# jorgeMFS/VCFX

Hardware: NVIDIA B200
Metric: vcf_input_GB_per_s (higher is better)
Workload: dtype u8

## Files before the change

vcfx_b200/csrc/vcfx_api.cu:

```cuda
#include "vcfx_cuda.h"
#include "vcfx_kernels.cuh"

#include <algorithm>
#include <cctype>
#include <cstdio>
#include <cstdlib>
#include <sched.h>
#include <cstring>
#include <new>
#include <string>
#include <vector>

using namespace vcfx;

#ifndef VCFX_LAUNCH
#define VCFX_LAUNCH(kern, grid, block, smem, stream, arg) (kern)<<<(grid), (block), (smem), (stream)>>>(arg)
#endif

namespace {

constexpr size_t DEFAULT_CHUNK = 64u << 20;
constexpr uint32_t EVENT_CAP = 1u << 20;
constexpr int MAX_SLOTS = 8;

struct Work {
    uint32_t *tile_lines = nullptr;
    unsigned long long *tile_out = nullptr;
    unsigned long long *tile_base = nullptr;
    unsigned long long *line_base = nullptr;
    uint32_t *tail_start = nullptr, *tail_len = nullptr, *tail_off = nullptr;
    uint2 *col_scratch = nullptr;
    unsigned int *ticket = nullptr;
    uint32_t *tile_resume = nullptr;
    Rec *recs = nullptr;
    uint8_t *rec_prefix = nullptr;
    uint64_t rec_cap = 0;
    DevStats *d_stats = nullptr;
    unsigned long long *events = nullptr;
    uint32_t ev_cap = 0;
    uint8_t *ib_codes = nullptr; size_t ib_codes_cap = 0;
    IbMeta *ib_rows = nullptr; uint64_t ib_rows_cap = 0;
    uint8_t *ib_panels = nullptr; uint64_t ib_panel_cap = 0;
    unsigned long long ib_seq = 0; bool ib_first = false;
    DevStats *h_stats = nullptr;
    DevStats *h_init = nullptr;
    uint32_t tiles_cap = 0;
    cudaEvent_t ev_k0 = nullptr, ev_k1 = nullptr;
    cudaEvent_t ev_stats = nullptr;
};

struct Slot {
    char *h_in = nullptr;
    uint8_t *d_in = nullptr;
    uint8_t *d_out = nullptr;
    char *h_out = nullptr;
    cudaStream_t stream = nullptr;
    Work w;
    size_t nbytes = 0;
    size_t out_cap = 0;
    vcfx_chunk_info info = {0, 1, 0, 0};
    bool in_flight = false;
    cudaEvent_t ev_h2d = nullptr;
    cudaEvent_t ev_shared_done = nullptr;
    bool shared_pending = false;
    uint8_t *d_in_used = nullptr;
    bool d2h_issued = false;
    size_t d2h_bytes = 0;
};

}

struct vcfx_ctx {
    vcfx_cfg cfg;
    int device = 0;
    int sm_count = 0;
    int blocks_per_sm = 1;
    size_t chunk_bytes = 0, out_bytes = 0;
    uint32_t tile_bytes = 0;
    size_t line_hint = 0;
    bool line_hint_fixed = false;
    int n_slots = 0;
    Slot slots[MAX_SLOTS];
    int head = 0;
    int tail = 0;
    int n_in_flight = 0;
    int acquired_slot = -1;
    Work dev_work;
    cudaStream_t dev_stream = nullptr;
    bool dev_stream_owned = false;
    bool dev_pending = false;
    size_t dev_nbytes = 0;
    uint8_t *dev_in = nullptr, *dev_out = nullptr;
    size_t dev_out_cap = 0;
    vcfx_chunk_info dev_info = {0, 1, 0, 0};
    uint32_t n_sel = 0, max_col = 0;
    uint32_t *d_sel_col = nullptr, *d_name_off = nullptr;
    uint8_t *d_names = nullptr;
    uint4 *d_names16 = nullptr;
    uint32_t name_len = 0;
    bool ac_bulk = true;
    int ac_fmt = 0;
    bool ac_ident = false;
    bool ac_exact = false;
    bool c4_bulk = false;
    uint8_t gq_query[64] = {0}; uint32_t gq_len = 0; int gq_a = -1, gq_b = -1;
    IbState *d_ib = nullptr; double *d_ib_sum = nullptr; unsigned long long *d_ib_het = nullptr; unsigned int *d_ib_used = nullptr; uint8_t *d_ib_last = nullptr;
    cudaEvent_t ib_event = nullptr;
    bool ib_event_set = false;
    unsigned long long ib_next_seq = 0;
    bool ib_open = false;
    std::vector<uint64_t> last_events;
    uint64_t last_n_events = 0;
    std::string last_error;
};

namespace {

#define CU(call)                                                                         \
    do {                                                                                 \
        cudaError_t _e = (call);                                                         \
        if (_e != cudaSuccess) {                                                         \
            ctx->last_error = std::string(#call) + ": " + cudaGetErrorString(_e);       \
            return (_e == cudaErrorMemoryAllocation) ? VCFX_E_NOMEM : VCFX_E_CUDA;       \
        }                                                                                \
    } while (0)

typedef void (*kernel_fn)(const KParams);

#ifdef VCFX_EMU
struct HweArgs { const int32_t *c; size_t n; double *p; };
void hwe_pvalue_entry(const HweArgs a) { hwe_pvalue_kernel(a.c, a.n, a.p); }
void hwe_pvalue_launch(int grid, const int32_t *c, size_t n, double *p) { HweArgs a = {c, n, p}; emu_launch(hwe_pvalue_entry, dim3(grid), dim3(256), 0, nullptr, a); }
#else
void hwe_pvalue_launch(int grid, const int32_t *c, size_t n, double *p) { hwe_pvalue_kernel<<<grid, 256>>>(c, n, p); }
#endif

bool is_copy_op(int op) {
    return op == VCFX_OP_MISSING_DETECT || op == VCFX_OP_NONREF_FILTER || op == VCFX_OP_PHASE_CHECK || op == VCFX_OP_GENOTYPE_QUERY;
}

kernel_fn kernel_for(int op) {
    switch (op) {
    case VCFX_OP_VARIANT_COUNT: return vcfx_scan_kernel<OP_VC, 0>;
    case VCFX_OP_ALLELE_FREQ:   return vcfx_scan_kernel<OP_AF, 0>;
    case VCFX_OP_HWE:           return vcfx_scan_kernel<OP_HWE, 0>;
    case VCFX_OP_MISSING_DETECT: return vcfx_scan_kernel<OP_MD, 0>;
    case VCFX_OP_NONREF_FILTER: return vcfx_scan_kernel<OP_NR, 0>;
    case VCFX_OP_INDEX: return vcfx_scan_kernel<OP_IX, 0>;
    case VCFX_OP_PHASE_CHECK: return vcfx_scan_kernel<OP_PC, 0>;
    case VCFX_OP_INBREEDING: return vcfx_scan_kernel<OP_IB, 0>;
    case VCFX_OP_GENOTYPE_QUERY: return vcfx_scan_kernel<OP_GQ, 0>;
    case VCFX_OP_DOSAGE: return vcfx_scan_kernel<OP_DS, 0>;
    case VCFX_OP_ALLELE_COUNT:  return vcfx_scan_kernel<OP_AC, 0>;
    default: return nullptr;
    }
}
kernel_fn general_kernel_for(int op) {
    switch (op) {
    case VCFX_OP_ALLELE_FREQ: return vcfx_scan_kernel<OP_AF, 1>;
    case VCFX_OP_HWE:         return vcfx_scan_kernel<OP_HWE, 1>;
    default: return nullptr;
    }
}
kernel_fn format_kernel_for(int op, int ac_fmt = 0) {
    if (op == VCFX_OP_ALLELE_COUNT) return ac_fmt == AC_AGG ? format_rows_kernel<OP_AC> : nullptr;
    switch (op) {
    case VCFX_OP_ALLELE_FREQ: return format_rows_kernel<OP_AF>;
    case VCFX_OP_HWE:         return format_rows_kernel<OP_HWE>;
    case VCFX_OP_MISSING_DETECT: return md_copy_kernel;
    case VCFX_OP_NONREF_FILTER: return md_copy_kernel;
    case VCFX_OP_PHASE_CHECK: return md_copy_kernel;
    case VCFX_OP_GENOTYPE_QUERY: return md_copy_kernel;
    case VCFX_OP_INDEX: return format_rows_kernel<OP_IX>;
    case VCFX_OP_INBREEDING: return ib_rows_kernel;
    case VCFX_OP_DOSAGE: return ds_rows_kernel;
    default: return nullptr;
    }
}

constexpr uint32_t MIN_TILE = 32u << 10, MAX_TILE = 256u << 10;

uint32_t tile_for(const vcfx_ctx *ctx, size_t nbytes) {
    if (ctx->tile_bytes) return ctx->tile_bytes;
    size_t warps = (size_t)ctx->sm_count * ctx->blocks_per_sm * WARPS_PER_CTA;
    size_t t = nbytes / (warps * 4 + 1);
    t = (t + 511) & ~(size_t)511;
    t = std::min<size_t>(MAX_TILE, std::max<size_t>(MIN_TILE, t));
    if (ctx->line_hint) {
        size_t want = std::min<size_t>((ctx->line_hint * 8 + 511) & ~(size_t)511, (size_t)8 << 20);
        size_t room = (nbytes / (warps * 2 + 1)) & ~(size_t)511;
        t = std::max(t, std::min(want, room));
    }
    return (uint32_t)t;
}

size_t measure_line(const char *p, size_t n, size_t from) {
    size_t pos = std::min(from, n), lim = std::min(n, pos + ((size_t)1 << 20));
    for (int tries = 0; pos < lim && tries < 4096; ++tries) {
        const char *nl = static_cast<const char *>(memchr(p + pos, '\n', lim - pos));
        if (!nl) return 0;
        size_t len = (size_t)(nl - (p + pos)) + 1;
        if (p[pos] != '#' && len > 1) return len;
        pos += len;
    }
    return 0;
}

uint32_t tiles_for(const vcfx_ctx *ctx, size_t nbytes, uint32_t tile) {
    (void)ctx;
    return (uint32_t)std::max<size_t>(1, (nbytes + tile - 1) / tile);
}

int grid_for(const vcfx_ctx *ctx, uint32_t n_tiles) {
    int resident = ctx->sm_count * ctx->blocks_per_sm;
    int need = (int)((n_tiles + WARPS_PER_CTA - 1) / WARPS_PER_CTA);
    return std::max(1, std::min(resident, need));
}

uint64_t default_rec_cap(size_t nbytes) { return nbytes / 256 + 65536; }

uint64_t rec_slack(const vcfx_ctx *ctx) {
    return (uint64_t)REC_BLOCK * ctx->sm_count * ctx->blocks_per_sm * WARPS_PER_CTA + 1024;
}

void free_work(Work &w) {
    cudaFree(w.tile_lines); cudaFree(w.tile_out); cudaFree(w.tile_base); cudaFree(w.line_base);
    cudaFree(w.rec_prefix); cudaFree(w.ticket); cudaFree(w.recs); cudaFree(w.d_stats); cudaFree(w.events);
    cudaFree(w.tail_start); cudaFree(w.tail_len); cudaFree(w.tail_off); cudaFree(w.col_scratch); cudaFree(w.tile_resume);
    cudaFree(w.ib_codes); cudaFree(w.ib_rows); cudaFree(w.ib_panels);
    if (w.h_stats) cudaFreeHost(w.h_stats);
    if (w.h_init) cudaFreeHost(w.h_init);
    if (w.ev_k0) cudaEventDestroy(w.ev_k0);
    if (w.ev_k1) cudaEventDestroy(w.ev_k1);
    if (w.ev_stats) cudaEventDestroy(w.ev_stats);
    w = Work();
}

int ensure_work(vcfx_ctx *ctx, Work &w, size_t max_bytes, uint64_t min_recs = 0, uint64_t min_panel_bytes = 0) {
    uint32_t tiles = tiles_for(ctx, max_bytes, ctx->tile_bytes ? ctx->tile_bytes : MIN_TILE);
    if (!w.d_stats) {
        CU(cudaMalloc(&w.d_stats, sizeof(DevStats)));
        CU(cudaMalloc(&w.ticket, 2 * sizeof(unsigned int)));
        CU(cudaMalloc(&w.events, sizeof(unsigned long long) * EVENT_CAP));
        w.ev_cap = EVENT_CAP;
        CU(cudaMallocHost(&w.h_stats, sizeof(DevStats)));
        CU(cudaMallocHost(&w.h_init, sizeof(DevStats)));
        memset(w.h_init, 0, sizeof(DevStats)); w.h_init->first_short_key = ~0ULL;
        memset(w.h_stats, 0, sizeof(DevStats));
        CU(cudaEventCreate(&w.ev_k0));
        CU(cudaEventCreate(&w.ev_k1));
        CU(cudaEventCreateWithFlags(&w.ev_stats, cudaEventDisableTiming));
    }
    if (tiles > w.tiles_cap) {
        cudaFree(w.tile_lines); cudaFree(w.tile_out); cudaFree(w.tile_base); cudaFree(w.line_base);
        w.tile_lines = nullptr; w.tile_out = nullptr; w.tile_base = w.line_base = nullptr;
        CU(cudaMalloc(&w.tile_lines, sizeof(uint32_t) * tiles));
        CU(cudaMalloc(&w.tile_out, sizeof(unsigned long long) * tiles));
        CU(cudaMalloc(&w.tile_base, sizeof(unsigned long long) * tiles));
        CU(cudaMalloc(&w.line_base, sizeof(unsigned long long) * tiles));
        if (general_kernel_for(ctx->cfg.op)) {
            cudaFree(w.tile_resume); w.tile_resume = nullptr;
            CU(cudaMalloc(&w.tile_resume, sizeof(uint32_t) * tiles));
        }
        if (is_copy_op(ctx->cfg.op)) {
            cudaFree(w.tail_start); cudaFree(w.tail_len); cudaFree(w.tail_off);
            w.tail_start = w.tail_len = w.tail_off = nullptr;
            CU(cudaMalloc(&w.tail_start, sizeof(uint32_t) * tiles));
            CU(cudaMalloc(&w.tail_len, sizeof(uint32_t) * tiles));
            CU(cudaMalloc(&w.tail_off, sizeof(uint32_t) * tiles));
        }
        w.tiles_cap = tiles;
    }
    uint64_t recs = 0;
    if (format_kernel_for(ctx->cfg.op, ctx->ac_fmt)) recs = std::max<uint64_t>(default_rec_cap(max_bytes), min_recs);
    if (ctx->cfg.op == VCFX_OP_ALLELE_COUNT && !w.col_scratch) {
        size_t n = (size_t)ctx->sm_count * ctx->blocks_per_sm * WARPS_PER_CTA * std::max<uint32_t>(ctx->max_col, 1);
        CU(cudaMalloc(&w.col_scratch, n * sizeof(uint2)));
    }
    if (ctx->cfg.op == VCFX_OP_DOSAGE && max_bytes + VCFX_DEVICE_PAD > w.ib_codes_cap) {
        cudaFree(w.ib_codes); w.ib_codes = nullptr; w.ib_codes_cap = 0;
        CU(cudaMalloc(&w.ib_codes, max_bytes + VCFX_DEVICE_PAD));
        w.ib_codes_cap = max_bytes + VCFX_DEVICE_PAD;
    }
    if (ctx->cfg.op == VCFX_OP_INBREEDING) {
        const uint64_t want_pan = std::max<uint64_t>(max_bytes + (1u << 20), min_panel_bytes);
        if (want_pan > w.ib_panel_cap) {
            cudaFree(w.ib_panels); w.ib_panels = nullptr; w.ib_panel_cap = 0;
            CU(cudaMalloc(&w.ib_panels, want_pan));
            w.ib_panel_cap = want_pan;
        }
        if (max_bytes + VCFX_DEVICE_PAD > w.ib_codes_cap) {
            cudaFree(w.ib_codes); w.ib_codes = nullptr; w.ib_codes_cap = 0;
            CU(cudaMalloc(&w.ib_codes, max_bytes + VCFX_DEVICE_PAD));
            w.ib_codes_cap = max_bytes + VCFX_DEVICE_PAD;
        }
        if (std::max<uint64_t>(recs, w.rec_cap) > w.ib_rows_cap) {
            const uint64_t want = std::max<uint64_t>(recs, w.rec_cap);
            cudaFree(w.ib_rows); w.ib_rows = nullptr; w.ib_rows_cap = 0;
            CU(cudaMalloc(&w.ib_rows, want * sizeof(IbMeta)));
            w.ib_rows_cap = want;
        }
    }
    if (recs > w.rec_cap) {
        cudaFree(w.recs); w.recs = nullptr; w.rec_cap = 0;
        cudaFree(w.rec_prefix); w.rec_prefix = nullptr;
        CU(cudaMalloc(&w.recs, recs * sizeof(Rec)));
        if (ctx->cfg.op == VCFX_OP_ALLELE_FREQ || ctx->cfg.op == VCFX_OP_HWE) CU(cudaMalloc(&w.rec_prefix, recs * 32));
        w.rec_cap = recs;
    }
    return VCFX_OK;
}

uint64_t ib_panel_need(const vcfx_ctx *ctx, const Work &w) {
    return (uint64_t)w.h_stats->n_recs * 32u * ((ctx->n_sel + 31u) / 32u) + (1u << 20);
}

void ib_begin(vcfx_ctx *ctx, Work &w, const vcfx_chunk_info *info) {
    if (ctx->cfg.op != VCFX_OP_INBREEDING) return;
    w.ib_seq = ctx->ib_next_seq++;
    w.ib_first = !ctx->ib_open;
    ctx->ib_open = !(info ? info->is_final != 0 : true);
}

int launch_chunk(vcfx_ctx *ctx, Work &w, cudaStream_t st, uint8_t *d_in, size_t nbytes,
                 const vcfx_chunk_info *info, uint8_t *d_out, size_t out_cap, bool write_pad = true) {
    kernel_fn fn = kernel_for(ctx->cfg.op);
    if (!fn) return VCFX_E_UNSUPPORTED;
    const uint32_t tile = tile_for(ctx, nbytes);
    uint32_t tiles = tiles_for(ctx, nbytes, tile);
    if (write_pad) CU(cudaMemsetAsync(d_in + nbytes, '\n', 64, st));
    CU(cudaMemsetAsync(w.ticket, 0, 2 * sizeof(unsigned int), st));
    kernel_fn gfn = general_kernel_for(ctx->cfg.op);
    if (gfn) CU(cudaMemsetAsync(w.tile_resume, 0xFF, sizeof(uint32_t) * tiles, st));
    CU(cudaMemcpyAsync(w.d_stats, w.h_init, sizeof(DevStats), cudaMemcpyHostToDevice, st));

    KParams P;
    P.in = d_in; P.n = nbytes;
    P.tile_bytes = tile; P.n_tiles = tiles;
    P.mode = ctx->cfg.mode; P.flags = ctx->cfg.flags;
    P.valid_from = info ? info->data_valid_from : 0;
    P.fmt0_until = info ? info->format_cache_from : 0;
    P.file_offset = info ? info->file_offset : 0;
    P.is_final = info ? info->is_final : 1;
    P.out = d_out; P.out_cap = out_cap;
    P.tile_lines = w.tile_lines; P.tile_out = w.tile_out; P.tile_base = w.tile_base; P.line_base = w.line_base;
    P.tail_start = w.tail_start; P.tail_len = w.tail_len; P.tail_off = w.tail_off;
    P.ac_fmt = ctx->ac_fmt; P.ac_ident = ctx->ac_ident ? 1 : 0; P.ac_pass = 0; P.ac_spec = (ctx->cfg.op == VCFX_OP_ALLELE_COUNT && ctx->ac_fmt == AC_TEXT_MT && !ctx->ac_exact) ? 1 : 0; P.n_sel = ctx->n_sel; P.sel_col = ctx->d_sel_col; P.name_off = ctx->d_name_off;
    P.names = ctx->d_names; P.names16 = ctx->d_names16; P.name_len = ctx->name_len; P.ac_bulk = ctx->ac_bulk ? 1 : 0; P.max_col = ctx->max_col; P.col_scratch = w.col_scratch;
    P.ticket = w.ticket; P.ticket2 = w.ticket + 1; P.tile_resume = w.tile_resume; P.recs = w.recs; P.rec_prefix = w.rec_prefix; P.rec_cap = w.rec_cap;
    P.c4_bulk = ctx->c4_bulk ? 1 : 0;
    memcpy(P.gq_query, ctx->gq_query, sizeof P.gq_query); P.gq_len = ctx->gq_len; P.gq_a = ctx->gq_a; P.gq_b = ctx->gq_b; P.gq_strict = (ctx->cfg.flags & VCFX_F_GQ_STRICT) ? 1 : 0;
    P.ib_codes = w.ib_codes; P.ib_rows = w.ib_rows; P.ib_panels = w.ib_panels; P.ib_panel_cap = w.ib_panel_cap; P.ib = ctx->d_ib; P.ib_seq = w.ib_seq; P.ib_first = w.ib_first ? 1 : 0; P.text_cap = out_cap;
    if (ctx->cfg.op == VCFX_OP_INBREEDING) P.out_cap = ~0ULL;
    P.stats = w.d_stats; P.events = w.events; P.ev_cap = w.ev_cap; P.ev_raw = (ctx->cfg.op == VCFX_OP_PHASE_CHECK || ctx->cfg.op == VCFX_OP_GENOTYPE_QUERY) ? 1 : 0;

    CU(cudaEventRecord(w.ev_k0, st));
    if (nbytes > 0) {
        int grid = grid_for(ctx, tiles);
        VCFX_LAUNCH(fn, grid, WARPS_PER_CTA * 32, 0, st, P);
        CU(cudaGetLastError());
        if (gfn) {
            const int ggrid = std::max(1, std::min(ctx->sm_count * VCFX_GENERAL_CTAS, (int)((tiles + WARPS_PER_CTA - 1) / WARPS_PER_CTA)));
            VCFX_LAUNCH(gfn, ggrid, WARPS_PER_CTA * 32, 0, st, P);
            CU(cudaGetLastError());
        }
        VCFX_LAUNCH(tile_scan_kernel, 1, 1024, SCAN_SMEM_BYTES, st, P);
        CU(cudaGetLastError());
        if (kernel_fn ff = format_kernel_for(ctx->cfg.op, ctx->ac_fmt)) {
            VCFX_LAUNCH(ff, ctx->sm_count * ((is_copy_op(ctx->cfg.op)) ? 8 : 16), 256, 0, st, P);
            CU(cudaGetLastError());
        } else if (ctx->cfg.op == VCFX_OP_ALLELE_COUNT) {
            CU(cudaMemsetAsync(w.ticket, 0, 2 * sizeof(unsigned int), st));
            P.ac_pass = 1;
            VCFX_LAUNCH(fn, grid, WARPS_PER_CTA * 32, 0, st, P);
            CU(cudaGetLastError());
        }
    }
    if (ctx->cfg.op == VCFX_OP_INBREEDING) {
        if (ctx->ib_event_set) CU(cudaStreamWaitEvent(st, ctx->ib_event, 0));
        VCFX_LAUNCH(ib_accumulate_kernel, (int)((ctx->n_sel + 31) / 32), 32, 0, st, P);
        CU(cudaGetLastError());
        VCFX_LAUNCH(ib_finish_kernel, 1, 1024, 0, st, P);
        CU(cudaGetLastError());
        CU(cudaEventRecord(ctx->ib_event, st));
        ctx->ib_event_set = true;
    }
    CU(cudaEventRecord(w.ev_k1, st));
    CU(cudaMemcpyAsync(w.h_stats, w.d_stats, sizeof(DevStats), cudaMemcpyDeviceToHost, st));
    CU(cudaEventRecord(w.ev_stats, st));
    return VCFX_OK;
}

void fill_stats(const Work &w, size_t nbytes, vcfx_chunk_stats *s) {
    if (!s) return;
    memset(s, 0, sizeof *s);
    const DevStats &d = *w.h_stats;
    s->bytes_in = nbytes; s->bytes_out = d.bytes_out;
    s->lines = d.lines; s->data_lines = d.data_lines; s->rows = d.rows; s->flagged = d.flagged;
    s->pre_header = d.pre_header; s->short_lines = d.short_lines;
    s->first_short_line = d.first_short_line; s->n_events = d.n_events;
    s->dots_terminated = d.dots_terminated; s->last_unterminated_flagged = d.last_unterminated_flagged;
    float ms = 0.f;
    if (cudaEventElapsedTime(&ms, w.ev_k0, w.ev_k1) == cudaSuccess) s->kernel_ms = ms;
}

int fetch_events(vcfx_ctx *ctx, const Work &w, cudaStream_t st) {
    uint64_t nev = std::min<uint64_t>(w.h_stats->n_events, w.ev_cap);
    ctx->last_n_events = w.h_stats->n_events;
    ctx->last_events.resize(nev);
    if (nev) {
        CU(cudaMemcpyAsync(ctx->last_events.data(), w.events, nev * sizeof(uint64_t), cudaMemcpyDeviceToHost, st));
        CU(cudaStreamSynchronize(st));
        std::sort(ctx->last_events.begin(), ctx->last_events.end());
    }
    return VCFX_OK;
}

int grow_events(vcfx_ctx *ctx, Work &w) {
    if ((ctx->cfg.op != VCFX_OP_PHASE_CHECK && ctx->cfg.op != VCFX_OP_GENOTYPE_QUERY) || w.h_stats->n_events <= w.ev_cap) return 0;
    const uint64_t want = w.h_stats->n_events + (w.h_stats->n_events >> 3) + 1024;
    if (want > 0xFFFFFFFFull) return VCFX_E_OUTPUT_TOO_BIG;
    cudaFree(w.events); w.events = nullptr; w.ev_cap = 0;
    CU(cudaMalloc(&w.events, sizeof(unsigned long long) * want));
    w.ev_cap = (uint32_t)want;
    return 1;
}

size_t default_out_bytes(int op, unsigned flags, size_t chunk) {
    switch (op) {
    case VCFX_OP_VARIANT_COUNT: return 4096;
    case VCFX_OP_MISSING_DETECT: return chunk + chunk / 4 + 4096;
    case VCFX_OP_NONREF_FILTER: return chunk + 4096;
    case VCFX_OP_PHASE_CHECK: return chunk + 4096;
    case VCFX_OP_GENOTYPE_QUERY: return chunk + 4096;
    case VCFX_OP_DOSAGE: return chunk + 4096;
    case VCFX_OP_INBREEDING: return 1u << 20;
    case VCFX_OP_ALLELE_COUNT:
        if (flags & VCFX_F_AC_AGGREGATE) return chunk / 4 + (1u << 20);
        if (flags & VCFX_F_AC_BINARY) return chunk + 4096;
        return 10 * chunk + 4096;
    default: return chunk / 4 + (1u << 20);
    }
}

void kick_ready(vcfx_ctx *ctx) {
    for (int i = 0, k = ctx->tail; i < ctx->n_in_flight; ++i, k = (k + 1) % ctx->n_slots) {
        Slot &s = ctx->slots[k];
        if (!s.in_flight || s.d2h_issued) continue;
        if (cudaEventQuery(s.w.ev_stats) != cudaSuccess) break;
        if (s.w.h_stats->overflow) continue;
        const size_t nout = (size_t)s.w.h_stats->bytes_out;
        if (nout && cudaMemcpyAsync(s.h_out, s.d_out, nout, cudaMemcpyDeviceToHost, s.stream) != cudaSuccess) { cudaGetLastError(); break; }
        s.d2h_issued = true; s.d2h_bytes = nout;
    }
}

}

extern "C" {

int vcfx_cuda_abi_version(void) { return VCFX_CUDA_ABI_VERSION; }

int vcfx_cuda_device_count(int *n) {
    int c = 0;
    cudaError_t e = cudaGetDeviceCount(&c);
    if (n) *n = (e == cudaSuccess) ? c : 0;
    return (e == cudaSuccess && c > 0) ? VCFX_OK : VCFX_E_NO_DEVICE;
}

const char *vcfx_cuda_strerror(int err) {
    switch (err) {
    case VCFX_OK: return "ok";
    case VCFX_E_INVALID: return "invalid argument or call order";
    case VCFX_E_NO_DEVICE: return "no usable CUDA device (libvcfx_cuda has no CPU fallback)";
    case VCFX_E_CUDA: return "CUDA call failed";
    case VCFX_E_NOMEM: return "out of memory";
    case VCFX_E_BUSY: return "all pipeline slots in flight";
    case VCFX_E_EMPTY: return "nothing in flight";
    case VCFX_E_OUTPUT_TOO_BIG: return "chunk output exceeds the output slot";
    case VCFX_E_UNSUPPORTED: return "operation not supported";
    default: return "unknown error";
    }
}

const char *vcfx_cuda_last_error(const vcfx_ctx *ctx) { return ctx ? ctx->last_error.c_str() : ""; }

int vcfx_cuda_create(const vcfx_cfg *cfg, vcfx_ctx **out) {
    if (!cfg || !out) return VCFX_E_INVALID;
    *out = nullptr;
    if (cfg->op < VCFX_OP_VARIANT_COUNT || cfg->op > VCFX_OP_DOSAGE) return VCFX_E_INVALID;
    if (cfg->mode != VCFX_MODE_FILE && cfg->mode != VCFX_MODE_STDIN) return VCFX_E_INVALID;
    int ndev = 0;
    if (cudaGetDeviceCount(&ndev) != cudaSuccess || ndev <= 0) return VCFX_E_NO_DEVICE;
    if (cfg->device < 0 || cfg->device >= ndev) return VCFX_E_INVALID;
    if (!kernel_for(cfg->op)) return VCFX_E_UNSUPPORTED;
    vcfx_ctx *ctx = new (std::nothrow) vcfx_ctx();
    if (!ctx) return VCFX_E_NOMEM;
    ctx->cfg = *cfg;
    ctx->device = cfg->device;
    ctx->chunk_bytes = cfg->chunk_bytes ? cfg->chunk_bytes : DEFAULT_CHUNK;
    ctx->tile_bytes = cfg->tile_bytes > 0 ? std::max<uint32_t>(512, ((uint32_t)cfg->tile_bytes + 511) & ~511u) : 0;
    ctx->out_bytes = cfg->out_bytes ? cfg->out_bytes : default_out_bytes(cfg->op, cfg->flags, ctx->chunk_bytes);
    ctx->n_slots = cfg->n_slots > 0 ? std::min(cfg->n_slots, MAX_SLOTS) : 3;
    auto fail = [&](int rc) { std::string e = ctx->last_error; vcfx_cuda_destroy(ctx); (void)e; return rc; };
#define CUC(call)                                                                        \
    do {                                                                                 \
        cudaError_t _e = (call);                                                         \
// ... 398 lines not shown
```

vcfx_b200/csrc/vcfx_kernels.cuh:

```cuda
#pragma once
#include <cuda_runtime.h>
#include <stdint.h>
#include <stddef.h>
#include "vcfx_numfmt.cuh"

namespace vcfx {

constexpr unsigned FULL = 0xFFFFFFFFu;
constexpr int WARPS_PER_CTA = 8;
constexpr uint32_t WINDOW = 512;

enum : int { OP_VC = 0, OP_AF = 1, OP_HWE = 2, OP_MD = 3, OP_AC = 4, OP_NR = 5, OP_IX = 6, OP_PC = 7, OP_IB = 8, OP_GQ = 9, OP_DS = 10 };
constexpr uint32_t NR_PLAIN = 0xFFFFFFFFu;
enum : int { MODE_FILE = 0, MODE_STDIN = 1 };
enum : int { AC_TEXT_MT = 0, AC_TEXT_FWD = 1, AC_AGG = 2, AC_BIN = 3 };
constexpr uint32_t AC_STAGE = 2048;

struct Rec {
    uint32_t tile;
    uint32_t ls_rel;
    uint32_t prefix_len;
    uint32_t off_in_tile;
    uint32_t a, b, c, d;
};

struct IbEntry {
    double x;
    uint32_t inc;
    uint32_t flag;
};
struct IbMeta { IbEntry e[4]; };
struct IbState {
    unsigned long long seq;
    unsigned long long variants;
    double *sum;
    unsigned long long *het;
    unsigned int *used;
    uint8_t *last;
};
constexpr uint32_t IB_NONE = 3, IB_ABSENT = 4;
constexpr uint32_t IB_F_GLOBAL = 1, IB_F_SKIP_BOUNDARY = 2, IB_F_COUNT_BOUNDARY = 4;

constexpr unsigned int REC_BLOCK = 32;
constexpr uint32_t RESUME_DONE = 0xFFFFFFFFu;
constexpr uint32_t REC_INVALID = 0xFFFFFFFFu;

struct DevStats {
    unsigned long long lines, data_lines, rows, flagged, pre_header, short_lines;
    unsigned long long first_short_key;
    unsigned long long n_events;
    unsigned long long dots_terminated;
    unsigned long long last_unterminated_flagged;
    unsigned long long bytes_out;
    unsigned long long overflow;
    unsigned long long first_short_line;
    unsigned long long n_recs;
    unsigned long long n_unfinished;
};

enum : int { C_LINES = 0, C_DATA = 1, C_ROWS = 2, C_FLAG = 3, C_PRE = 4, C_SHORT = 5, C_DOTS = 8, CNT_SLOTS = 9 };
static_assert(offsetof(DevStats, lines) == 8 * C_LINES && offsetof(DevStats, data_lines) == 8 * C_DATA && offsetof(DevStats, rows) == 8 * C_ROWS &&
              offsetof(DevStats, flagged) == 8 * C_FLAG && offsetof(DevStats, pre_header) == 8 * C_PRE && offsetof(DevStats, short_lines) == 8 * C_SHORT &&
              offsetof(DevStats, dots_terminated) == 8 * C_DOTS, "counter slots follow DevStats");

struct KParams {
    const uint8_t *in;
    uint64_t n;
    uint32_t tile_bytes;
    uint32_t n_tiles;
    int32_t mode;
    uint32_t flags;
    uint64_t valid_from;
    uint64_t file_offset;
    int32_t is_final;
    uint8_t *out;
    uint64_t out_cap;
    uint32_t *tile_lines;
    unsigned long long *tile_out;
    unsigned long long *tile_base;
    unsigned long long *line_base;
    uint32_t *tail_start;
    uint32_t *tail_len;
    uint32_t *tail_off;
    int32_t ac_fmt;
    int32_t ac_pass;
    int32_t ac_ident;
    int32_t ac_spec;
    uint32_t n_sel;
    const uint32_t *sel_col;
    const uint32_t *name_off;
    const uint8_t *names;
    const uint4 *names16;
    int32_t ac_bulk;
    uint32_t name_len;
    uint32_t max_col;
    uint2 *col_scratch;
    unsigned int *ticket;
    unsigned int *ticket2;
    uint32_t *tile_resume;
    Rec *recs;
    uint8_t *rec_prefix;
    uint64_t rec_cap;
    DevStats *stats;
    unsigned long long *events;
    uint32_t ev_cap;
    unsigned long long fmt0_until;
    int32_t c4_bulk;
    uint8_t gq_query[64];
    uint32_t gq_len;
    int32_t gq_a, gq_b;
    int32_t gq_strict;
    uint8_t *ib_codes;
    IbMeta *ib_rows;
    uint8_t *ib_panels;
    uint64_t ib_panel_cap;
    IbState *ib;
    unsigned long long ib_seq;
    int32_t ib_first;
    uint64_t text_cap;
    int32_t ev_raw;
};

__device__ __forceinline__ uint32_t zero_bytes(uint32_t x) {
    return ~(((x & 0x7F7F7F7Fu) + 0x7F7F7F7Fu) | x) & 0x80808080u;
}
__device__ __forceinline__ uint32_t eq_bytes(uint32_t w, uint32_t c4) { return zero_bytes(w ^ c4); }

constexpr uint32_t C_TAB = 0x09090909u, C_NL = 0x0A0A0A0Au, C_DOT = 0x2E2E2E2Eu;

__device__ __forceinline__ uint32_t range_mask(uint32_t base, uint32_t lo, uint32_t hi) {
    uint32_t m = 0x80808080u;
    if (lo > base) { uint32_t s = lo - base; m = (s >= 4) ? 0u : (m << (8 * s)); }
    if (hi < base + 4) { m = (hi <= base) ? 0u : (m & (0x80808080u >> (8 * (base + 4 - hi)))); }
    return m;
}

__device__ __forceinline__ uint32_t lane_keep16(uint32_t pb, uint32_t lo, uint32_t hi) {
    const uint32_t a = lo > pb ? min(lo - pb, 16u) : 0u;
    const uint32_t b = hi > pb ? min(hi - pb, 16u) : 0u;
    return b > a ? (((1u << b) - 1u) & ~((1u << a) - 1u)) : 0u;
}
__device__ __forceinline__ uint32_t nib80(uint32_t keep16, int j) {
    return ((((keep16 >> (4 * j)) & 0xFu) * 0x00204081u) & 0x01010101u) << 7;
}
__device__ __forceinline__ void clip4(uint32_t &m0, uint32_t &m1, uint32_t &m2, uint32_t &m3, uint32_t pb, uint32_t lo, uint32_t hi) {
    const uint32_t k = lane_keep16(pb, lo, hi);
    m0 &= nib80(k, 0); m1 &= nib80(k, 1); m2 &= nib80(k, 2); m3 &= nib80(k, 3);
}

__device__ __forceinline__ uint4 ld16(const uint8_t *p) { return __ldg(reinterpret_cast<const uint4 *>(p)); }
__device__ __forceinline__ uint32_t ldb(const uint8_t *p) { return (uint32_t)__ldg(p); }
__device__ __forceinline__ uint32_t ldw(const uint8_t *p) { return __ldg(reinterpret_cast<const uint32_t *>(p)); }
#ifdef VCFX_EMU
#define VCFX_GRID_CONSTANT
__device__ __forceinline__ void prefetch_l2(const void *) {}
__device__ __forceinline__ void prefetch_l1(const void *) {}
__device__ __forceinline__ int lane_id() { return (int)(threadIdx.x & 31u); }
#else
#define VCFX_GRID_CONSTANT __grid_constant__
__device__ __forceinline__ void prefetch_l2(const void *p) { asm volatile("prefetch.global.L2 [%0];" ::"l"(p)); }
__device__ __forceinline__ void prefetch_l1(const void *p) { asm volatile("prefetch.global.L1 [%0];" ::"l"(p)); }
__device__ __forceinline__ int lane_id() { int l; asm("mov.u32 %0, %%laneid;" : "=r"(l)); return l; }
#endif

__device__ __forceinline__ bool is_dig(uint32_t b) { return (b - 48u) <= 9u; }
__device__ __forceinline__ bool is_sep(uint32_t b) { return b == '/' || b == '|'; }


__device__ __noinline__ uint2 af_sample_slow(const uint8_t *p, bool strip_cr, int gt_index) {
    uint32_t alt = 0, total = 0;
    const uint8_t *se = p;
    uint32_t c = ldb(se);
    while (c != '\t' && c != '\n') { ++se; c = ldb(se); }
    if (strip_cr && c == '\n' && se > p && ldb(se - 1) == '\r') --se;
    for (int i = 0; i < gt_index && p < se; ++i) {
        while (p < se && ldb(p) != ':') ++p;
        if (p < se) ++p;
    }
    if (p >= se) return make_uint2(0u, 0u);
    const uint8_t *ge = p;
    while (ge < se && ldb(ge) != ':') ++ge;
    while (p < ge) {
        while (p < ge && is_sep(ldb(p))) ++p;
        if (p >= ge) break;
        const uint8_t *q = p; bool numeric = true, zero = true; const uint32_t first = ldb(p);
        while (q < ge) {
            uint32_t d = ldb(q);
            if (is_sep(d)) break;
            if (numeric) { if (!is_dig(d)) numeric = false; else if (d != '0') zero = false; }
            ++q;
        }
        if (first != '.' && numeric) { ++total; if (!zero) ++alt; }
        p = q;
    }
    return make_uint2(alt, total);
}

__device__ __noinline__ int hwe_sample_slow(const uint8_t *p) {
    const uint8_t *e = p;
    for (;;) { uint32_t c = ldb(e); if (c == '\t' || c == ':' || c == '\n') break; ++e; }
    while (p < e) { uint32_t c = ldb(p); if (c == ' ' || c == '\r') ++p; else break; }
    if (p >= e) return -1;
    if (!is_dig(ldb(p))) return -1;
    int a1 = 0, a2 = 0;
    while (p < e && is_dig(ldb(p))) { a1 = (a1 > 1) ? 2 : a1 * 10 + (int)(ldb(p) - 48u); ++p; }
    if (p >= e || !is_sep(ldb(p))) return -1;
    ++p;
    if (p >= e || !is_dig(ldb(p))) return -1;
    while (p < e && is_dig(ldb(p))) { a2 = (a2 > 1) ? 2 : a2 * 10 + (int)(ldb(p) - 48u); ++p; }
    if (a1 > 1 || a2 > 1) return -1;
    if (a1 == 0 && a2 == 0) return 0;
    if (a1 == 1 && a2 == 1) return 2;
    return 1;
}

__device__ __noinline__ int gt_index_of(const uint8_t *p, const uint8_t *e) {
    int idx = 0;
    while (p < e) {
        const uint8_t *q = p;
        while (q < e && ldb(q) != ':') ++q;
        if (q - p == 2 && ldb(p) == 'G' && ldb(p + 1) == 'T') return idx;
        ++idx;
        p = (q < e) ? q + 1 : q;
    }
    return -1;
}

__device__ __noinline__ bool nr_sample_homref(const uint8_t *p, bool file_mode, int gt_index) {
    const uint8_t *se = p;
    uint32_t c = ldb(se);
    while (c != '\t' && c != '\n') { ++se; c = ldb(se); }
    if (file_mode && c == '\n' && ldb(se - 1) == '\r') { if (se - 1 >= p) --se; else return true; }
    if (se == p) return (c == '\n') ? file_mode : false;
    const uint8_t *gs = p, *ge = se;
    if (file_mode && gt_index == 0) { ge = p; while (ge < se && ldb(ge) != ':') ++ge; }
    else {
        int idx = 0; const uint8_t *fs = p; bool got = false;
        for (const uint8_t *q = p; q <= se; ++q) {
            if (q == se || ldb(q) == ':') {
                if (idx == gt_index) { gs = fs; ge = q; got = true; break; }
                ++idx; fs = q + 1;
            }
        }
        if (!got) return false;
        if (!file_mode && ge == se && gs == se && ldb(se - 1) == ':') return false;
    }
    const uint32_t n = (uint32_t)(ge - gs);
    if (n == 0) return false;
    if (file_mode && n == 3) return ldb(gs) == '0' && is_sep(ldb(gs + 1)) && ldb(gs + 2) == '0';
    for (const uint8_t *q = gs; q < ge; ++q) { const uint32_t b = ldb(q); if (b != '0' && !is_sep(b)) return false; }
    return true;
}

__device__ __noinline__ bool pc_sample_phased(const uint8_t *p, bool file_mode, int gt_index) {
    const uint8_t *se = p;
    uint32_t c = ldb(se);
    while (c != '\t' && c != '\n') { ++se; c = ldb(se); }
    if (file_mode && c == '\n' && ldb(se - 1) == '\r') { if (se - 1 >= p) --se; else return true; }
    if (se == p) return (c == '\n') ? file_mode : false;
    const uint8_t *gs = p, *ge = se;
    if (gt_index == 0) { ge = p; while (ge < se && ldb(ge) != ':') ++ge; }
    else {
        int idx = 0; const uint8_t *fs = p; bool got = false;
        for (const uint8_t *q = p; q <= se; ++q) {
            if (q == se || ldb(q) == ':') {
                if (idx == gt_index) { gs = fs; ge = q; got = true; break; }
                ++idx; fs = q + 1;
            }
        }
        if (!got) return false;
    }
    const uint32_t n = (uint32_t)(ge - gs);
    if (n == 0 || n == 1) return false;
    if (n == 3) return ldb(gs + 1) == '|' && ldb(gs) != '.' && ldb(gs + 2) != '.';
    if (ldb(gs) == '.' && is_sep(ldb(gs + 1)) && ldb(gs + 2) == '.') return false;
    bool pipe = false; const uint8_t *as = gs;
    for (const uint8_t *q = gs; q < ge; ++q) {
        const uint32_t b = ldb(q);
        if (b == '|') {
            const uint32_t al = (uint32_t)(q - as);
            if (al == 0 || (al == 1 && ldb(as) == '.')) return false;
            pipe = true; as = q + 1;
        } else if (b == '/') return false;
    }
    const uint32_t al = (uint32_t)(ge - as);
    if (al == 0 || (al == 1 && ldb(as) == '.')) return false;
    return pipe;
}

struct GqQuery { const uint8_t *q; uint32_t len; int a, b; bool strict; };
__device__ __forceinline__ bool gq_match3(uint32_t u, const GqQuery &Q) {
    if (Q.strict) return Q.len == 3u && ((u ^ ((uint32_t)Q.q[0] | ((uint32_t)Q.q[1] << 8) | ((uint32_t)Q.q[2] << 16))) & 0x00FFFFFFu) == 0u;
    const uint32_t b1 = (u >> 8) & 0xFFu, d0 = (u & 0xFFu) - '0', d2 = ((u >> 16) & 0xFFu) - '0';
    if ((b1 != '/' && b1 != '|') || d0 > 9u || d2 > 9u) return false;
    return (int)min(d0, d2) == Q.a && (int)max(d0, d2) == Q.b;
}
__device__ __noinline__ bool gq_sample_match(const uint8_t *p, int gt_index, const GqQuery Q) {
    const uint8_t *se = p;
    uint32_t c = ldb(se);
    while (c != '\t' && c != '\n') { ++se; c = ldb(se); }
    const uint8_t *gs = p, *ge = se;
    {
        int idx = 0; const uint8_t *fs = p; bool got = false;
        for (const uint8_t *q = p; q <= se; ++q) {
            if (q == se || ldb(q) == ':') {
                if (idx == gt_index) { gs = fs; ge = q; got = true; break; }
                ++idx; fs = q + 1;
            }
        }
        if (!got) return false;
    }
    const uint32_t n = (uint32_t)(ge - gs);
    if (n == 0) return false;
    if (Q.strict) {
        if (n != Q.len) return false;
        for (uint32_t i = 0; i < n; ++i) if (ldb(gs + i) != Q.q[i]) return false;
        return true;
    }
    uint32_t sp = 0;
    while (sp < n && ldb(gs + sp) != '|' && ldb(gs + sp) != '/') ++sp;
    if (sp == n || sp == 0 || sp == n - 1) return false;
    uint32_t a1 = 0, a2 = 0;
    for (uint32_t i = 0; i < sp; ++i) { const uint32_t d = ldb(gs + i) - '0'; if (d > 9u) return false; a1 = a1 * 10u + d; }
    for (uint32_t i = sp + 1; i < n; ++i) { const uint32_t d = ldb(gs + i) - '0'; if (d > 9u) return false; a2 = a2 * 10u + d; }
    int x = (int)a1, y = (int)a2;
    if (x > y) { const int t = x; x = y; y = t; }
    return x == Q.a && y == Q.b;
}

__device__ __noinline__ uint32_t ib_sample_code(const uint8_t *p) {
    uint32_t c = ldb(p);
    if (c == '\n' || (c == '\r' && ldb(p + 1) == '\n')) return IB_ABSENT;
    while (c == ' ' || c == '\r') { ++p; c = ldb(p); }
    if (c - '0' > 9u) return IB_NONE;
    uint32_t a1 = 0, a2 = 0;
    while (c - '0' <= 9u) { a1 = a1 * 10u + (c - '0'); ++p; c = ldb(p); }
    if (c != '/' && c != '|') return IB_NONE;
    ++p; c = ldb(p);
    if (c - '0' > 9u) return IB_NONE;
    while (c - '0' <= 9u) { a2 = a2 * 10u + (c - '0'); ++p; c = ldb(p); }
    if (a1 > 1u || a2 > 1u) return IB_NONE;
    return a1 + a2;
}

__device__ __noinline__ uint32_t ds_sample_code(const uint8_t *p, bool file_mode, int gt_index) {
    const uint8_t *se = p;
    uint32_t c = ldb(se);
    while (c != '\t' && c != '\n') { ++se; c = ldb(se); }
    if (file_mode && c == '\n' && se > p && ldb(se - 1) == '\r') --se;
    if (se == p && c == '\n') return IB_ABSENT;
    const uint8_t *gs = p, *ge = se;
    {
        int idx = 0; const uint8_t *fs = p; bool got = false;
        for (const uint8_t *q = p; q <= se; ++q) {
            if (q == se || ldb(q) == ':') {
                if (idx == gt_index) { gs = fs; ge = q; got = true; break; }
                ++idx; fs = q + 1;
            }
        }
        if (!got || ge == gs) return IB_NONE;
    }
    uint32_t dosage = 0, alleles = 0;
    const uint8_t *q = gs;
    while (q < ge) {
        while (q < ge && is_sep(ldb(q))) ++q;
        if (q >= ge) break;
        uint32_t allele = 0; bool digit = false;
        while (q < ge && ldb(q) - '0' <= 9u) { allele = allele * 10u + (ldb(q) - '0'); digit = true; ++q; }
        if (!digit) return IB_NONE;
        if ((int)allele > 0) ++dosage;
        if (++alleles > 2) return IB_NONE;
    }
    return alleles == 2 ? dosage : IB_NONE;
}

__device__ __noinline__ bool ix_parse_line(const uint8_t *s, const uint8_t *e, bool file_mode, uint32_t &c_off, uint32_t &c_len, long long &pos) {
    auto space = [](uint32_t c) { return c == ' ' || (c >= 9u && c <= 13u); };
    const uint8_t *p = s;
    if (file_mode) {
        while (p < e && (ldb(p) == ' ' || ldb(p) == '\t')) ++p;
        if (p >= e || ldb(p) == '#') return false;
        const uint8_t *cs = p;
        while (p < e && ldb(p) != '\t') ++p;
        if (p == cs || p >= e) return false;
        c_off = (uint32_t)(cs - s); c_len = (uint32_t)(p - cs);
        ++p;
        unsigned long long v = 0;
        while (p < e && is_dig(ldb(p))) { v = v * 10ULL + (ldb(p) - 48u); ++p; }
        pos = (long long)v;
        return pos > 0;
    }
    while (p < e && space(ldb(p))) ++p;
    if (p < e && ldb(p) == '#') return false;
    const uint8_t *tab = s;
    while (tab < e && ldb(tab) != '\t') ++tab;
    if (tab >= e) return false;
    c_off = 0; c_len = (uint32_t)(tab - s);
    const uint8_t *q = tab + 1, *pe = q;
    while (pe < e && ldb(pe) != '\t') ++pe;
    while (q < pe && space(ldb(q))) ++q;
    bool neg = false;
    if (q < pe && (ldb(q) == '+' || ldb(q) == '-')) { neg = ldb(q) == '-'; ++q; }
    if (q >= pe || !is_dig(ldb(q))) return false;
    const unsigned long long lim = neg ? 9223372036854775808ULL : 9223372036854775807ULL;
    unsigned long long v = 0;
    while (q < pe && is_dig(ldb(q))) {
        const unsigned long long d = ldb(q) - 48u;
        if (v > (lim - d) / 10ULL) return false;
        v = v * 10ULL + d; ++q;
    }
    pos = neg ? (long long)(0ULL - v) : (long long)v;
    return true;
}
__device__ __forceinline__ uint32_t dec_len64(long long v) {
    unsigned long long u = v < 0 ? 0ULL - (unsigned long long)v : (unsigned long long)v;
    uint32_t n = v < 0 ? 1u : 0u;
    do { ++n; u /= 10ULL; } while (u);
    return n;
}
__device__ __forceinline__ uint8_t *put_dec64(uint8_t *d, long long v) {
    unsigned long long u = v < 0 ? 0ULL - (unsigned long long)v : (unsigned long long)v;
    if (v < 0) *d++ = '-';
    char t[24]; int n = 0;
    do { t[n++] = (char)('0' + (int)(u % 10ULL)); u /= 10ULL; } while (u);
    while (n) *d++ = (uint8_t)t[--n];
    return d;
}

__device__ __forceinline__ int first_byte(uint32_t m0, uint32_t m1, uint32_t m2, uint32_t m3) {
    const uint32_t m = m0 ? m0 : (m1 ? m1 : (m2 ? m2 : m3));
    const int base = m0 ? 0 : (m1 ? 4 : (m2 ? 8 : 12));
    return base + ((__ffs(m) - 1) >> 3);
}

__device__ __forceinline__ int warp_incl_scan(int v, int lane) {
#pragma unroll
    for (int o = 1; o < 32; o <<= 1) { int t = __shfl_up_sync(FULL, v, o); if (lane >= o) v += t; }
    return v;
}

struct Tally { uint32_t a, b, c; };

struct WClass { uint32_t D, Z, P, S, E, O; };
template <int OP>
__device__ __forceinline__ WClass classify_word(uint32_t x) {
    const uint32_t x7 = x & 0x7F7F7F7Fu, ok = ~x & 0x80808080u;
#define VCFX_GE(c) (x7 + (0x80808080u - 0x01010101u * (uint32_t)(c)))
    const uint32_t g2e = VCFX_GE(0x2E), g2f = VCFX_GE(0x2F), g30 = VCFX_GE(0x30), g31 = VCFX_GE(0x31);
    const uint32_t g3a = VCFX_GE(0x3A), g3b = VCFX_GE(0x3B), g7c = VCFX_GE(0x7C), g7d = VCFX_GE(0x7D);
    const uint32_t g09 = VCFX_GE(0x09), g0b = VCFX_GE(0x0B);
    WClass c;
    c.P = g2e & ~g2f & ok;
    c.Z = g30 & ~g31 & ok;
    c.D = g30 & ~g3a & ok;
    c.S = ((g2f & ~g30) | (g7c & ~g7d)) & ok;
    c.E = ((g09 & ~g0b) | (g3a & ~g3b)) & ok;
    c.O = (OP == OP_HWE) ? (g31 & ~VCFX_GE(0x32) & ok) : 0u;
#undef VCFX_GE
    return c;
}
__device__ __forceinline__ uint32_t down(uint32_t lo, uint32_t hi, int k) { return __funnelshift_rc(lo, hi, 8u * (uint32_t)k); }

template <int OP>
__device__ __noinline__ uint4 lane_samples_generic(uint32_t w0, uint32_t w1, uint32_t w2, uint32_t w3, uint32_t la,
                                                   uint32_t m0, uint32_t m1, uint32_t m2, uint32_t m3,
                                                   const uint8_t *lane_ptr, bool strip_cr, int gt_index) {
    const uint32_t ws[5] = {w0, w1, w2, w3, la};
    const uint32_t ms[4] = {m0, m1, m2, m3};
    uint32_t ta = 0, tb = 0, tc = 0, irregular = 0;
    WClass lo = classify_word<OP>(ws[0]);
#pragma unroll
    for (int j = 0; j < 4; ++j) {
        const WClass hi = classify_word<OP>(ws[j + 1]);
        const uint32_t m = ms[j];
        uint32_t rest = m;
        if (m) {
            const uint32_t d1 = down(lo.D, hi.D, 1), d3 = down(lo.D, hi.D, 3), s2 = down(lo.S, hi.S, 2);
            if (OP == OP_AF) {
                if (gt_index == 0) {
                    const uint32_t tokl = lo.D | lo.P, tokh = hi.D | hi.P;
                    const uint32_t t1 = down(tokl, tokh, 1), t3 = down(tokl, tokh, 3);
                    const uint32_t e1 = down(lo.E, hi.E, 1), e2 = down(lo.E, hi.E, 2), e4 = hi.E;
                    const uint32_t z1 = down(lo.Z, hi.Z, 1), z3 = down(lo.Z, hi.Z, 3);
                    const uint32_t A = m & e1, B = m & t1 & e2, C = m & t1 & s2 & t3 & e4, any = B | C;
                    tb += __popc(any & d1) + __popc(C & d3);
                    ta += __popc(any & d1 & ~z1) + __popc(C & d3 & ~z3);
                    rest = m & ~(A | any);
                    irregular |= m & ~(C & d1 & d3);
                } else irregular = 1;
            } else {
                const uint32_t d2 = down(lo.D, hi.D, 2), d4 = hi.D, p1 = down(lo.P, hi.P, 1);
                const uint32_t o1 = down(lo.O, hi.O, 1), o3 = down(lo.O, hi.O, 3);
                const uint32_t l1 = o1 | down(lo.Z, hi.Z, 1), l3 = o3 | down(lo.Z, hi.Z, 3);
                const uint32_t full = m & d1 & s2 & d3 & ~d4;
                const uint32_t rej = m & ((~d1 & p1) | (d1 & ~s2 & ~d2) | (d1 & s2 & ~d3));
                const uint32_t ok = full & l1 & l3;
                ta += __popc(ok & ~o1 & ~o3); tb += __popc(ok & (o1 ^ o3)); tc += __popc(ok & o1 & o3);
                rest = m & ~(full | rej);
                irregular |= m & ~full;
            }
        }
        while (rest) {
            const int k = (__ffs(rest) - 1) >> 3;
            rest &= rest - 1;
            const uint8_t *p = lane_ptr + 4 * j + k + 1;
            if (OP == OP_AF) { const uint2 r = af_sample_slow(p, strip_cr, gt_index); ta += r.x; tb += r.y; }
            else { const int c = hwe_sample_slow(p); ta += (c == 0); tb += (c == 1); tc += (c == 2); }
        }
        lo = hi;
    }
    return make_uint4(ta, tb, tc, irregular);
}

template <int OP>
__device__ __forceinline__ bool lane_lattice(uint32_t w0, uint32_t w1, uint32_t w2, uint32_t w3, uint32_t la,
                                             uint32_t &packed, uint32_t &sh) {
    const uint32_t t0 = eq_bytes(w0, C_TAB);
    sh = (uint32_t)__ffs(t0);
    const uint32_t xs[4] = {__funnelshift_rc(w0, w1, sh), __funnelshift_rc(w1, w2, sh),
                            __funnelshift_rc(w2, w3, sh), __funnelshift_rc(w3, la, sh)};
    uint32_t bad = 0, acc = 0;
#pragma unroll
    for (int j = 0; j < 4; ++j) {
        const uint32_t y = xs[j] ^ 0x09300030u;
        bad |= ((y + 0x00060006u) | y) & 0xFFF000F0u;
        const uint32_t sp = y & 0x0000FF00u;
        bad |= (uint32_t)((sp != 0x00007C00u) & (sp != 0x00002F00u));
        if (OP == OP_AF) {
            acc += (y + 0x000F000Fu) & 0x00100010u;
        } else {
            const uint32_t a = y & 0xFFu, b = (y >> 16) & 0xFFu;
            const uint32_t ok = (uint32_t)((a | b) <= 1u);
            acc += ok + ((ok & (a ^ b)) << 8) + ((ok & a & b) << 16);
        }
    }
    packed = (OP == OP_AF) ? (((acc >> 4) & 0xFFu) + (acc >> 20)) : acc;
    return bad == 0;
}

__device__ __noinline__ bool md_lane_dots(const uint8_t *p, uint32_t d0, uint32_t d1, uint32_t d2, uint32_t d3, bool strip_cr) {
    uint32_t ds[4] = {d0, d1, d2, d3};
#pragma unroll
    for (int j = 0; j < 4; ++j) {
        uint32_t m = ds[j];
        while (m) {
            const int k = (__ffs(m) - 1) >> 3;
            m &= m - 1;
            const uint8_t *q = p + 4 * j + k;
            const uint32_t prev = ldb(q - 1), next = ldb(q + 1);
            const bool a = (prev == '\t') || is_sep(prev);
            const bool b = is_sep(next) || next == ':' || next == '\t' || next == '\n' ||
                           (strip_cr && next == '\r' && ldb(q + 2) == '\n');
            if (!(a || b)) continue;
            if (prev == '\t') return true;
            const uint8_t *r = q - 1;
            for (;;) { const uint32_t c = ldb(r); if (c == '\t') return true; if (c == ':') break; --r; }
        }
    }
    return false;
}

__device__ __noinline__ uint2 ac_sample_slow(const uint8_t *p) {
    uint32_t ref = 0, alt = 0;
    for (;;) {
        uint32_t c = ldb(p);
        if (c == ':' || c == '\t' || c == '\n') break;
        if (is_dig(c)) {
            bool nz = false;
            do { nz |= (c != '0'); ++p; c = ldb(p); } while (is_dig(c));
            if (nz) ++alt; else ++ref;
        } else ++p;
    }
    return make_uint2(ref, alt);
}
__device__ __forceinline__ uint32_t dec_len(int v) {
    if ((uint32_t)v < 10u) return 1u;
    uint32_t n = (v < 0) ? 1u : 0u;
    uint32_t u = (v < 0) ? (uint32_t)(-v) : (uint32_t)v;
    do { ++n; u /= 10u; } while (u);
    return n;
}
__device__ __forceinline__ uint8_t *put_dec(uint8_t *d, int v) {
    if ((uint32_t)v < 10u) { *d = (uint8_t)('0' + v); return d + 1; }
    if (v < 0) { *d++ = '-'; v = -v; }
    char t[12]; int n = 0; uint32_t u = (uint32_t)v;
    do { t[n++] = (char)('0' + u % 10u); u /= 10u; } while (u);
    while (n) *d++ = (uint8_t)t[--n];
    return d;
}
__device__ __forceinline__ void warp_flush_smem(uint8_t *dst, const uint8_t *st, uint32_t n, int lane) {
    const uint32_t head = min(n, (uint32_t)((16 - ((uintptr_t)dst & 15)) & 15));
    if (lane < (int)head) dst[lane] = st[lane];
    const uint32_t nq = (n - head) >> 4;
    uint4 *d16 = reinterpret_cast<uint4 *>(dst + head);
    const uint4 *s16 = reinterpret_cast<const uint4 *>(st + head);
    for (uint32_t i = lane; i < nq; i += 32) d16[i] = s16[i];
    const uint32_t done = head + (nq << 4);
    if (lane < (int)(n - done)) dst[done + lane] = st[done + lane];
}

__device__ __forceinline__ void warp_flush_smem_bulk(uint8_t *dst, const uint8_t *st, uint32_t n, int lane) {
#ifdef VCFX_EMU
    warp_flush_smem(dst, st, n, lane);
#else
    const uint32_t head = min(n, (uint32_t)((16 - ((uintptr_t)dst & 15)) & 15));
    if (lane < (int)head) dst[lane] = st[lane];
    const uint32_t nq = (n - head) >> 4;
    if (lane == 0 && nq) {
        const uint32_t saddr = (uint32_t)__cvta_generic_to_shared(st + head);
        asm volatile("fence.proxy.async.shared::cta;" ::: "memory");
        asm volatile("cp.async.bulk.global.shared::cta.bulk_group [%0], [%1], %2;" :: "l"(dst + head), "r"(saddr), "r"(nq << 4) : "memory");
        asm volatile("cp.async.bulk.commit_group;" ::: "memory");
        asm volatile("cp.async.bulk.wait_group.read 0;" ::: "memory");
    }
    const uint32_t done = head + (nq << 4);
    if (lane < (int)(n - done)) dst[done + lane] = st[done + lane];
#endif
}

template <int OP>
__device__ __forceinline__ bool t1_eval(uint32_t w0, uint32_t w1, uint32_t w2, uint32_t w3, uint32_t la,
                                        uint32_t sh_u, uint32_t pat, uint32_t &accp, uint32_t &hetp, uint32_t &hap) {
    const uint32_t y0 = __funnelshift_rc(w0, w1, sh_u) ^ pat;
    const uint32_t y1 = __funnelshift_rc(w1, w2, sh_u) ^ pat;
    const uint32_t y2 = __funnelshift_rc(w2, w3, sh_u) ^ pat;
    const uint32_t y3 = __funnelshift_rc(w3, la, sh_u) ^ pat;
    const uint32_t bad = (y0 | y1 | y2 | y3) & 0xFFFEFFFEu;
    if (__any_sync(FULL, bad != 0)) return false;
    if (OP == OP_AF) accp += y0 + y1 + y2 + y3;
    else {
        const uint32_t pk = y0 + 2u * y1 + 4u * y2 + 8u * y3;
        const uint32_t ab = pk & 0xFu, bb = (pk >> 16) & 0xFu;
        hetp += __popc(ab ^ bb); hap += __popc(ab & bb);
    }
    return true;
}

template <int OP> struct OutCount { typedef uint32_t type; };
template <> struct OutCount<OP_AC> { typedef unsigned long long type; };

template <int OP>
__device__ __forceinline__ void t1_tally(uint32_t y0, uint32_t y1, uint32_t y2, uint32_t y3, uint32_t &accp, uint32_t &hetp, uint32_t &hap) {
    if (OP == OP_AF) accp += y0 + y1 + y2 + y3;
    else {
        const uint32_t pk = y0 + 2u * y1 + 4u * y2 + 8u * y3;
        const uint32_t ab = pk & 0xFu, bb = (pk >> 16) & 0xFu;
        hetp += __popc(ab ^ bb); hap += __popc(ab & bb);
    }
}

#ifdef VCFX_EMU
__device__ __forceinline__ uint32_t dp4a_u(uint32_t a, uint32_t b, uint32_t c) {
    return c + (a & 0xFFu) * (b & 0xFFu) + ((a >> 8) & 0xFFu) * ((b >> 8) & 0xFFu) + ((a >> 16) & 0xFFu) * ((b >> 16) & 0xFFu) + (a >> 24) * (b >> 24);
}
#else
__device__ __forceinline__ uint32_t dp4a_u(uint32_t a, uint32_t b, uint32_t c) { return __dp4a(a, b, c); }
#endif
constexpr uint32_t M80 = 0x80808080u;
#define VCFX_GE(x, c) ((x) + (0x80808080u - 0x01010101u * (uint32_t)(c)))
__device__ __forceinline__ uint32_t up1(uint32_t prev, uint32_t w) { return __funnelshift_l(prev, w, 8); }

template <int OP> struct DigitClass { uint32_t adjc, D, NZ, SP, TB; };
template <int OP>
__device__ __forceinline__ DigitClass<OP> digit_classes(uint32_t x) {
    DigitClass<OP> c;
    const uint32_t g30 = VCFX_GE(x, 0x30), g31 = VCFX_GE(x, 0x31), g3a = VCFX_GE(x, 0x3A), g3b = VCFX_GE(x, 0x3B);
    const uint32_t g09 = VCFX_GE(x, 0x09), g0a = VCFX_GE(x, 0x0A), g0b = VCFX_GE(x, 0x0B);
    c.D = (g30 ^ g3a) & M80;
    c.NZ = (g31 ^ g3a) & M80;
    c.SP = (g0a ^ g0b ^ g3a ^ g3b) & M80;
    if (OP == OP_AF) {
        const uint32_t g2f = VCFX_GE(x, 0x2F), g7c = VCFX_GE(x, 0x7C), g7d = VCFX_GE(x, 0x7D);
        c.adjc = (g09 ^ g0b ^ g2f ^ g30 ^ g7c ^ g7d) & M80;
        c.TB = 0;
    } else {
        c.adjc = c.D;
        c.TB = (g09 ^ g0a) & M80;
    }
    return c;
}

__device__ __forceinline__ void patch_outside(uint4 &v, uint32_t pb, uint32_t lo, uint32_t hi, uint32_t filler4) {
    const uint32_t keep = lane_keep16(pb, lo, hi);
    const uint32_t k0 = (nib80(keep, 0) >> 7) * 0xFFu, k1 = (nib80(keep, 1) >> 7) * 0xFFu;
    const uint32_t k2 = (nib80(keep, 2) >> 7) * 0xFFu, k3 = (nib80(keep, 3) >> 7) * 0xFFu;
    v.x = (v.x & k0) | (filler4 & ~k0); v.y = (v.y & k1) | (filler4 & ~k1);
    v.z = (v.z & k2) | (filler4 & ~k2); v.w = (v.w & k3) | (filler4 & ~k3);
}

template <int OP>
__device__ __forceinline__ void digits_window(const uint4 cur, const uint32_t carry_in, const int lane,
                                              uint32_t &tB, uint32_t &tA, uint32_t &tT, uint32_t &odd, uint32_t &next_carry) {
    uint32_t pk, adj_first;
    tT = 0;
    {
        const DigitClass<OP> c3 = digit_classes<OP>(cur.w);
        pk = (c3.adjc & 0x80000000u) | ((c3.D >> 1) & 0x40000000u) | ((c3.NZ >> 2) & 0x20000000u);
        const DigitClass<OP> c2 = digit_classes<OP>(cur.z);
        const uint32_t a3 = up1(c2.adjc, c3.adjc);
        odd = ((OP == OP_AF) ? (~(c3.adjc | a3) & M80) : (c3.adjc & a3)) | c3.SP | c2.SP;
        tB = dp4a_u(c3.D, 0x00010101u, dp4a_u(c2.D, 0x01010101u, 0u));
        tA = dp4a_u(c3.NZ, 0x00010101u, dp4a_u(c2.NZ, 0x01010101u, 0u));
        if (OP == OP_AC) tT = dp4a_u(c3.TB, 0x01010101u, dp4a_u(c2.TB, 0x01010101u, 0u));
        const DigitClass<OP> c1 = digit_classes<OP>(cur.y);
        const uint32_t a2 = up1(c1.adjc, c2.adjc);
        odd |= ((OP == OP_AF) ? (~(c2.adjc | a2) & M80) : (c2.adjc & a2)) | c1.SP;
        tB = dp4a_u(c1.D, 0x01010101u, tB); tA = dp4a_u(c1.NZ, 0x01010101u, tA);
        if (OP == OP_AC) tT = dp4a_u(c1.TB, 0x01010101u, tT);
        const DigitClass<OP> c0 = digit_classes<OP>(cur.x);
        const uint32_t a1 = up1(c0.adjc, c1.adjc);
        odd |= ((OP == OP_AF) ? (~(c1.adjc | a1) & M80) : (c1.adjc & a1)) | c0.SP;
        tB = dp4a_u(c0.D, 0x01010101u, tB); tA = dp4a_u(c0.NZ, 0x01010101u, tA);
        if (OP == OP_AC) tT = dp4a_u(c0.TB, 0x01010101u, tT);
        adj_first = c0.adjc;
    }
    uint32_t pv = __shfl_sync(FULL, pk, (lane + 31) & 31);
    next_carry = pv;
    if (lane == 0) pv = carry_in;
    const uint32_t a0 = up1(pv, adj_first);
    odd |= ((OP == OP_AF) ? (~(adj_first | a0) & M80) : (adj_first & a0)) | ((cur.x | cur.y | cur.z | cur.w) & M80);
    tB += (pv >> 23) & 0x80u;
    tA += (pv >> 22) & 0x80u;
}

template <int OP>
__device__ __forceinline__ bool line_digits(const uint8_t *__restrict__ tin, uint32_t wb, const uint32_t lo, const uint32_t nrel,
                                           const bool strip_cr, uint32_t &out_a, uint32_t &out_b, uint32_t &out_tabs, uint32_t &out_e) {
    const int lane = lane_id();
    constexpr uint32_t FILL = (OP == OP_AF) ? 0x09090909u : 0x20202020u;
    uint32_t accA = 0, accB = 0, accT = 0;
    uint32_t carry = (OP == OP_AF) ? 0x80000000u : 0u;
    uint4 cur = ld16(tin + wb + 16 * lane);
    uint4 nxt = ld16(tin + wb + WINDOW + 16 * lane);
    uint4 nx2 = ld16(tin + wb + 2 * WINDOW + 16 * lane);
    patch_outside(cur, wb + 16 * lane, lo, ~0u, FILL);
    bool first = true;
    for (;;) {
        uint32_t tB, tA, tT, odd, nc;
        digits_window<OP>(cur, carry, lane, tB, tA, tT, odd, nc);
        if (__any_sync(FULL, odd != 0)) {
            const uint32_t n0 = eq_bytes(cur.x, C_NL), n1 = eq_bytes(cur.y, C_NL), n2 = eq_bytes(cur.z, C_NL), n3 = eq_bytes(cur.w, C_NL);
            const unsigned ebal = __ballot_sync(FULL, (n0 | n1 | n2 | n3) != 0);
            if (!ebal) return false;
            const int src = __ffs(ebal) - 1;
            int k = first_byte(n0, n1, n2, n3);
            k = __shfl_sync(FULL, k, src);
            const uint32_t e = wb + 16 * src + k;
            uint32_t ee = e;
            if (OP == OP_AF && strip_cr && e > lo && ldb(tin + e - 1) == '\r') ee = e - 1;
            patch_outside(cur, wb + 16 * lane, 0u, ee, FILL);
            digits_window<OP>(cur, carry, lane, tB, tA, tT, odd, nc);
            if (__any_sync(FULL, odd != 0)) return false;
            accB += tB; accA += tA; if (OP == OP_AC && !first) accT += tT;
            out_a = accA >> 7; out_b = accB >> 7; out_tabs = accT >> 7; out_e = e;
            return true;
        }
        accB += tB; accA += tA; if (OP == OP_AC && !first) accT += tT;
        if (lane == 0) carry = nc;
        first = false;
        wb += WINDOW; cur = nxt; nxt = nx2; nx2 = ld16(tin + wb + 2 * WINDOW + 16 * lane);
        if (((wb >> 9) & 7u) == 0) {
            const uint32_t pf = wb + 10 * WINDOW + 128 * lane;
            if (pf < nrel) prefetch_l2(tin + pf);
        }
    }
}

__device__ __forceinline__ unsigned long long alloc_slot(unsigned long long *rec_base, unsigned int *rec_used, DevStats *stats) {
    unsigned int used = *rec_used;
    if (used == REC_BLOCK) { *rec_base = atomicAdd(&stats->n_recs, (unsigned long long)REC_BLOCK); used = 0; }
    *rec_used = used + 1;
    return *rec_base + used;
}

struct WarpShared {
    volatile uint32_t *tp;
    uint8_t *stage0;
    uint32_t *u;
    unsigned int *cnt;
    unsigned long long *rec_base; unsigned int *rec_used;
    volatile unsigned int *odd, *reg, *tag;
    uint8_t *ring;
    unsigned long long *bars;
    uint32_t *ring_par;
};
template <int OP> struct TileState {
    uint32_t ls, nlines;
    typename OutCount<OP>::type out_bytes;
    uint32_t md_prev_end, md_last_end;
    bool md_add_nl;
    uint32_t offlattice_lines;
};

#ifndef VCFX_C4_RING
#define VCFX_C4_RING 0
#endif
constexpr uint32_t C4_PIECE = 1024, C4_STAGES = 4, C4_RING = C4_PIECE * C4_STAGES;
__device__ __forceinline__ void ring_init(unsigned long long *bars, int lane) {
#ifndef VCFX_EMU
    if (lane == 0) {
        const uint32_t b = (uint32_t)__cvta_generic_to_shared(bars);
        for (uint32_t i = 0; i < C4_STAGES; ++i) asm volatile("mbarrier.init.shared::cta.b64 [%0], 1;" :: "r"(b + 8u * i));
        asm volatile("fence.mbarrier_init.release.cluster;" ::: "memory");
    }
    __syncwarp();
#endif
}
__device__ __forceinline__ void ring_issue(uint8_t *ring, unsigned long long *bars, const uint8_t *g0, uint32_t k) {
    const uint32_t st = k % C4_STAGES;
#ifdef VCFX_EMU
    for (uint32_t i = 0; i < C4_PIECE; ++i) ring[st * C4_PIECE + i] = g0[(size_t)k * C4_PIECE + i];
#else
    const uint32_t bar = (uint32_t)__cvta_generic_to_shared(bars + st), dst = (uint32_t)__cvta_generic_to_shared(ring + st * C4_PIECE);
    asm volatile("mbarrier.arrive.expect_tx.shared::cta.b64 _, [%0], %1;" :: "r"(bar), "r"(C4_PIECE) : "memory");
    asm volatile("cp.async.bulk.shared::cluster.global.mbarrier::complete_tx::bytes [%0], [%1], %2, [%3];"
                 :: "r"(dst), "l"(g0 + (size_t)k * C4_PIECE), "r"(C4_PIECE), "r"(bar) : "memory");
#endif
}
__device__ __forceinline__ void ring_wait(unsigned long long *bars, uint32_t st, uint32_t parity) {
#ifndef VCFX_EMU
    const uint32_t bar = (uint32_t)__cvta_generic_to_shared(bars + st);
    uint32_t done = 0;
    while (!done)
        asm volatile("{ .reg .pred p; mbarrier.try_wait.parity.shared::cta.b64 p, [%1], %2; selp.u32 %0, 1, 0, p; }" : "=r"(done) : "r"(bar), "r"(parity) : "memory");
#endif
}

template <int OP, bool RING = false>
__device__ __forceinline__ bool multikey_window(const uint4 v, const uint8_t *__restrict__ p, uint32_t &da, uint32_t &db, uint32_t &dc,
                                                const uint8_t *ring = nullptr, uint32_t x = 0) {
    const uint32_t a0 = VCFX_GE(v.x, 0x09), b0 = VCFX_GE(v.x, 0x0A), c0 = VCFX_GE(v.x, 0x0B);
    const uint32_t a1 = VCFX_GE(v.y, 0x09), b1 = VCFX_GE(v.y, 0x0A), c1 = VCFX_GE(v.y, 0x0B);
    const uint32_t a2 = VCFX_GE(v.z, 0x09), b2 = VCFX_GE(v.z, 0x0A), c2 = VCFX_GE(v.z, 0x0B);
    const uint32_t a3 = VCFX_GE(v.w, 0x09), b3 = VCFX_GE(v.w, 0x0A), c3 = VCFX_GE(v.w, 0x0B);
    const uint32_t tm0 = (a0 ^ b0) & M80, tm1 = (a1 ^ b1) & M80, tm2 = (a2 ^ b2) & M80, tm3 = (a3 ^ b3) & M80;
    bool odd = (((b0 ^ c0) | (b1 ^ c1) | (b2 ^ c2) | (b3 ^ c3) | v.x | v.y | v.z | v.w) & M80) != 0;
    da = 0; db = 0; dc = 0;
    if (tm0 | tm1 | tm2 | tm3) {
        const uint32_t m16 = ((tm0 * 0x00204081u) >> 28) | (((tm1 * 0x00204081u) >> 24) & 0xF0u) |
                             (((tm2 * 0x00204081u) >> 20) & 0xF00u) | (((tm3 * 0x00204081u) >> 16) & 0xF000u);
        if (m16 & (m16 - 1u)) odd = true;
        uint32_t q;
        if (RING) {
            const uint32_t xs = x + (uint32_t)__ffs(m16);
            const uint32_t w0 = *reinterpret_cast<const uint32_t *>(ring + ((xs & ~3u) & (C4_RING - 1u)));
            const uint32_t w1 = *reinterpret_cast<const uint32_t *>(ring + (((xs & ~3u) + 4u) & (C4_RING - 1u)));
            q = __funnelshift_r(w0, w1, 8u * (xs & 3u));
        } else {
            const uint8_t *s = p + __ffs(m16);
            const uint32_t *s4 = reinterpret_cast<const uint32_t *>((uintptr_t)s & ~(uintptr_t)3);
            q = __funnelshift_r(__ldg(s4), __ldg(s4 + 1), 8u * (uint32_t)((uintptr_t)s & 3));
        }
        const uint32_t q1 = (q >> 8) & 0xFFu, q3 = q >> 24;
        const bool sep = (q1 == '/') | (q1 == '|');
        const uint32_t dg = q & 0x00FF00FFu;
        const bool two_digits = ((dg & 0x00F000F0u) == 0x00300030u) & ((((dg & 0x000F000Fu) + 0x00060006u) & 0x00100010u) == 0u);
        if (OP == OP_AF) {
            const bool end = (q3 == ':') | (q3 == '\t');
            if (sep & end & two_digits) { db = 2; da = (uint32_t)((dg & 0x0000000Fu) != 0u) + (uint32_t)((dg & 0x000F0000u) != 0u); }
            else if (!(sep & end & (dg == 0x002E002Eu))) odd = true;
        } else {
            const bool more = (q3 - 48u) <= 9u;
            if (sep & two_digits & !more) {
                const uint32_t al = dg & 0x000F000Fu;
                if ((al & 0x000E000Eu) == 0u) { const uint32_t c = (al & 1u) + (al >> 16); da = (c == 0); db = (c == 1); dc = (c == 2); }
            } else if (!(sep & (dg == 0x002E002Eu))) odd = true;
        }
    }
    return odd;
}

template <int OP, int VAR>
__device__ __forceinline__ bool tile_lines(const KParams &P, const WarpShared ws, const int lane, const bool strip_cr,
                                           const uint32_t tile, const uint64_t a, const uint64_t a0, const uint8_t *__restrict__ tin,
                                           const uint32_t rb, const uint32_t nrel, const uint64_t n, TileState<OP> &st) {
    constexpr bool HAS_VAR = (OP == OP_AF || OP == OP_HWE);
    constexpr int NEED_TABS = (OP == OP_VC) ? 7 : (OP == OP_IX) ? 1 : 9;
    volatile uint32_t *tp = ws.tp;
    const int wid = threadIdx.x >> 5;
    volatile unsigned int *s_odd = ws.odd, *s_reg = ws.reg, *s_tag = ws.tag;
    uint32_t ls = st.ls, nlines = st.nlines;
    typename OutCount<OP>::type out_bytes = st.out_bytes;
    uint32_t md_prev_end = st.md_prev_end, md_last_end = st.md_last_end;
    bool md_add_nl = st.md_add_nl;
#define VCFX_COUNT(slot, v) do { if (lane == 0) atomicAdd(&ws.cnt[slot], (unsigned int)(v)); } while (0)
#define VCFX_SAVE_STATE() do { st.ls = ls; st.nlines = nlines; st.out_bytes = out_bytes; st.md_prev_end = md_prev_end; st.md_last_end = md_last_end; st.md_add_nl = md_add_nl; } while (0)
        while (ls < rb) {
            uint32_t wb = ls & ~15u;
            uint4 cur = ld16(tin + wb + 16 * lane);
            uint4 nxt = ld16(tin + wb + WINDOW + 16 * lane);
            uint4 nx2 = ld16(tin + wb + 2 * WINDOW + 16 * lane);
            const uint32_t first = ldb(tin + ls);
            const bool hash = (first == '#');
            int tabs = 0;
            bool found = false;
            uint32_t e = 0;
            uint32_t ta = 0, tb = 0, tc = 0;
            int gt_index = -1;
            bool do_samples = false;

            uint32_t t0, t1, t2, t3;
            int rank0 = 0;
            for (;;) {
                const uint32_t pb = wb + 16 * lane;
                t0 = eq_bytes(cur.x, C_TAB); t1 = eq_bytes(cur.y, C_TAB);
                t2 = eq_bytes(cur.z, C_TAB); t3 = eq_bytes(cur.w, C_TAB);
                uint32_t n0 = eq_bytes(cur.x, C_NL), n1 = eq_bytes(cur.y, C_NL);
                uint32_t n2 = eq_bytes(cur.z, C_NL), n3 = eq_bytes(cur.w, C_NL);
                if (wb < ls) {
                    const uint32_t k = lane_keep16(pb, ls, ~0u);
                    const uint32_t k0 = nib80(k, 0), k1 = nib80(k, 1), k2 = nib80(k, 2), k3 = nib80(k, 3);
                    t0 &= k0; t1 &= k1; t2 &= k2; t3 &= k3; n0 &= k0; n1 &= k1; n2 &= k2; n3 &= k3;
                }
                unsigned ebal = __ballot_sync(FULL, (n0 | n1 | n2 | n3) != 0);
                if (ebal) {
                    int src = __ffs(ebal) - 1;
                    int k = first_byte(n0, n1, n2, n3);
                    k = __shfl_sync(FULL, k, src);
                    e = wb + 16 * src + k; found = true;
                    clip4(t0, t1, t2, t3, pb, 0, e);
                }
                int total = 0;
                if (!hash) {
                    if (OP == OP_VC) {
                        const int cnt = __popc(t0) + __popc(t1) + __popc(t2) + __popc(t3);
                        total = (int)__reduce_add_sync(FULL, (unsigned)cnt);
                    } else {
                        uint32_t m16 = ((t0 * 0x00204081u) >> 28) | (((t1 * 0x00204081u) >> 24) & 0xF0u) |
                                       (((t2 * 0x00204081u) >> 20) & 0xF00u) | (((t3 * 0x00204081u) >> 16) & 0xF000u);
                        const int cnt = __popc(m16);
                        int incl = warp_incl_scan(cnt, lane);
                        total = __shfl_sync(FULL, incl, 31);
                        rank0 = tabs + incl - cnt;
                        int rank = rank0;
                        while (m16 && rank < 9) {
                            tp[rank++] = pb + (uint32_t)(__ffs(m16) - 1);
                            m16 &= m16 - 1;
                        }
                    }
                }
                tabs += total;
                if (found || tabs >= NEED_TABS) break;
                wb += WINDOW; cur = nxt; nxt = nx2; nx2 = ld16(tin + wb + 2 * WINDOW + 16 * lane);
            }
            __syncwarp();

            if ((OP == OP_AF || OP == OP_HWE) && !hash && tabs >= 9) {
                const uint32_t fs = tp[7] + 1, fe = tp[8];
                if (OP == OP_AF) {
                    if (fe - fs == 2 && ldb(tin + fs) == 'G' && ldb(tin + fs + 1) == 'T') gt_index = 0;
                    else gt_index = gt_index_of(tin + fs, tin + fe);
                    do_samples = gt_index >= 0 && (a0 + ls >= P.valid_from);
                } else {
                    do_samples = (fe - fs >= 2) && ldb(tin + fs) == 'G' && ldb(tin + fs + 1) == 'T';
                    gt_index = 0;
                }
            }

            if ((OP == OP_AF || OP == OP_HWE) && do_samples) {
                bool first_win = true;
                bool digits_tried = false;
                bool prev_ok = false;
                const uint32_t tab8 = tp[8];
                const uint32_t sep0 = ldb(tin + tab8 + 2);
                const bool lat_possible = (gt_index == 0) && (tp[8] - tp[7] == 3);
                const bool t1_on = lat_possible && (sep0 == '|' || sep0 == '/');
                const uint32_t tau = tab8 & 3u;
                const uint32_t sh_u = 8u * (tau + 1u);
                const uint32_t pat = 0x09300030u | (sep0 << 8);
                uint32_t accp = 0;
                uint32_t hetp = 0, hap = 0;
                uint32_t n_real = 0;
                if (t1_on && !found) {
                    const uint32_t la_ = ldw(tin + wb + 16 * lane + 16);
                    uint32_t y0 = __funnelshift_rc(cur.x, cur.y, sh_u) ^ pat, y1 = __funnelshift_rc(cur.y, cur.z, sh_u) ^ pat;
                    uint32_t y2 = __funnelshift_rc(cur.z, cur.w, sh_u) ^ pat, y3 = __funnelshift_rc(cur.w, la_, sh_u) ^ pat;
                    const uint32_t rel = tab8 - wb, Lb = rel >> 4, kb = (rel >> 2) & 3u;
                    const uint32_t kmin = (uint32_t)lane > Lb ? 0u : ((uint32_t)lane == Lb ? kb : 4u);
                    if (kmin > 0) y0 = 0;
                    if (kmin > 1) y1 = 0;
                    if (kmin > 2) y2 = 0;
                    if (kmin > 3) y3 = 0;
                    if (!__any_sync(FULL, ((y0 | y1 | y2 | y3) & 0xFFFEFFFEu) != 0)) {
                        t1_tally<OP>(y0, y1, y2, y3, accp, hetp, hap);
                        n_real += ((wb + WINDOW - 1 - tab8) >> 2) + 1;
                        first_win = false; prev_ok = true;
                        wb += WINDOW; cur = nxt; nxt = nx2; nx2 = ld16(tin + wb + 2 * WINDOW + 16 * lane);
                    }
                }
                if (HAS_VAR && !found && first_win) {
                    if (VAR == 0) { VCFX_SAVE_STATE(); return false; }
                }
                for (;;) {
                    if (VCFX_C4_RING && VAR == 1 && !first_win && !lat_possible && gt_index == 0 && P.c4_bulk) {
                        const uint8_t *g0 = tin + wb;
                        uint8_t *ring = ws.ring; unsigned long long *bars = ws.bars;
                        uint32_t par = *ws.ring_par;
                        if (lane == 0) for (uint32_t q = 0; q < C4_STAGES; ++q) ring_issue(ring, bars, g0, q);
                        uint32_t k = 0;
                        ring_wait(bars, 0, (par >> 0) & 1u); par ^= 1u;
                        for (;;) {
                            const uint32_t st = k % C4_STAGES, st1 = (k + 1) % C4_STAGES;
                            ring_wait(bars, st1, (par >> st1) & 1u); par ^= 1u << st1;
                            const uint8_t *rp = ring + st * C4_PIECE + 16 * lane;
                            const uint4 v0 = *reinterpret_cast<const uint4 *>(rp), v1 = *reinterpret_cast<const uint4 *>(rp + WINDOW);
                            uint32_t da0, db0, dc0, da1, db1, dc1;
                            const uint32_t x0 = k * C4_PIECE + 16u * (uint32_t)lane;
                            const bool o0 = multikey_window<OP, true>(v0, nullptr, da0, db0, dc0, ring, x0);
                            const bool o1 = multikey_window<OP, true>(v1, nullptr, da1, db1, dc1, ring, x0 + WINDOW);
                            if (__any_sync(FULL, o0 | o1)) break;
                            ta += da0 + da1; tb += db0 + db1; tc += dc0 + dc1;
                            __syncwarp();
                            if (lane == 0) {
#ifndef VCFX_EMU
                                asm volatile("fence.proxy.async.shared::cta;" ::: "memory");
#endif
                                ring_issue(ring, bars, g0, k + C4_STAGES);
                            }
                            ++k;
                        }
                        { const uint32_t s2 = (k + 2) % C4_STAGES, s3 = (k + 3) % C4_STAGES;
                          ring_wait(bars, s2, (par >> s2) & 1u); par ^= 1u << s2;
                          ring_wait(bars, s3, (par >> s3) & 1u); par ^= 1u << s3; }
                        *ws.ring_par = par;
                        wb += k * C4_PIECE;
                        cur = ld16(tin + wb + 16 * lane); nxt = ld16(tin + wb + WINDOW + 16 * lane); nx2 = ld16(tin + wb + 2 * WINDOW + 16 * lane);
                    }
                    else if (VAR == 1 && !first_win && !lat_possible && gt_index == 0) {
                        uint4 nx3 = ld16(tin + wb + 3 * WINDOW + 16 * lane);
                        int state = 0;
                        const uint8_t *lp = tin + wb + 16 * lane;
                        uint32_t it = 0;
                        for (;;) {
                            {
                                uint32_t da0, db0, dc0, da1, db1, dc1;
                                const bool o0 = multikey_window<OP>(cur, lp, da0, db0, dc0);
                                const bool o1 = multikey_window<OP>(nxt, lp + WINDOW, da1, db1, dc1);
                                if (__any_sync(FULL, o0 | o1)) { state = 1; break; }
                                ta += da0 + da1; tb += db0 + db1; tc += dc0 + dc1;
                                cur = ld16(lp + 4 * WINDOW); nxt = ld16(lp + 5 * WINDOW);
                            }
                            {
                                uint32_t da0, db0, dc0, da1, db1, dc1;
                                const bool o0 = multikey_window<OP>(nx2, lp + 2 * WINDOW, da0, db0, dc0);
                                const bool o1 = multikey_window<OP>(nx3, lp + 3 * WINDOW, da1, db1, dc1);
                                if (__any_sync(FULL, o0 | o1)) { state = 2; break; }
                                ta += da0 + da1; tb += db0 + db1; tc += dc0 + dc1;
                                nx2 = ld16(lp + 6 * WINDOW); nx3 = ld16(lp + 7 * WINDOW);
                            }
                            if ((++it & 1u) == 0) {
                                const uint8_t *pf = lp - 16 * lane + 16 * WINDOW + 128 * lane;
                                if ((uint32_t)(pf - tin) < nrel) prefetch_l2(pf);
                            }
                            lp += 4 * WINDOW;
                        }
                        wb = (uint32_t)(lp - tin) - 16u * (uint32_t)lane;
                        if (state == 2) { const uint4 t_ = cur; wb += 2 * WINDOW; cur = nx2; nxt = nx3; nx2 = t_; }
                    }
                    if (t1_on && prev_ok) {
                        const uint32_t ITMAX = 64u;
                        uint32_t la_c = 0, la_n = 0;
                        for (;;) {
                            const uint8_t *lp = tin + wb + 16 * lane;
                            uint4 nx3 = ld16(lp + 3 * WINDOW);
                            uint32_t la0 = ldw(lp + 16), la1 = ldw(lp + WINDOW + 16);
                            uint32_t la2 = ldw(lp + 2 * WINDOW + 16), la3 = ldw(lp + 3 * WINDOW + 16);
                            const uint32_t pf_need = wb + 12 * WINDOW;
                            const uint32_t pf_iters = nrel > pf_need ? (nrel - pf_need) / (4 * WINDOW) : 0u;
                            uint32_t it = 0, accf = 0, acc2 = 0;
                            int state = 0;
#define VCFX_T1_ROUND(X, LX, Y, LY)                                                                              \
                                uint32_t bad, sum, sq = 0;                                                       \
                                {                                                                                \
                                    const uint32_t f0 = __funnelshift_rc(X.x, X.y, sh_u), f1 = __funnelshift_rc(X.y, X.z, sh_u); \
                                    const uint32_t f2 = __funnelshift_rc(X.z, X.w, sh_u), f3 = __funnelshift_rc(X.w, LX, sh_u);  \
                                    const uint32_t g0 = __funnelshift_rc(Y.x, Y.y, sh_u), g1 = __funnelshift_rc(Y.y, Y.z, sh_u); \
                                    const uint32_t g2 = __funnelshift_rc(Y.z, Y.w, sh_u), g3 = __funnelshift_rc(Y.w, LY, sh_u);  \
                                    bad = (f0 ^ pat) | (f1 ^ pat); bad |= f2 ^ pat; bad |= f3 ^ pat;             \
                                    bad |= g0 ^ pat; bad |= g1 ^ pat; bad |= g2 ^ pat; bad |= g3 ^ pat;          \
                                    sum = (f0 + f1 + f2) + (f3 + g0 + g1) + (g2 + g3);                           \
                                    if (OP == OP_HWE) sq = f0 * f0 + f1 * f1 + f2 * f2 + f3 * f3 + g0 * g0 + g1 * g1 + g2 * g2 + g3 * g3; \
                                }
                            for (; it < ITMAX; ++it) {
                                {
                                    VCFX_T1_ROUND(cur, la0, nxt, la1)
                                    if (__any_sync(FULL, (bad & 0xFFFEFFFEu) != 0)) { state = 1; break; }
                                    accf += sum; if (OP == OP_HWE) acc2 += sq;
                                    cur = ld16(lp + 4 * WINDOW); la0 = ldw(lp + 4 * WINDOW + 16);
                                    nxt = ld16(lp + 5 * WINDOW); la1 = ldw(lp + 5 * WINDOW + 16);
                                }
                                {
                                    VCFX_T1_ROUND(nx2, la2, nx3, la3)
                                    if (__any_sync(FULL, (bad & 0xFFFEFFFEu) != 0)) { state = 2; break; }
                                    accf += sum; if (OP == OP_HWE) acc2 += sq;
                                    nx2 = ld16(lp + 6 * WINDOW); la2 = ldw(lp + 6 * WINDOW + 16);
                                    nx3 = ld16(lp + 7 * WINDOW); la3 = ldw(lp + 7 * WINDOW + 16);
                                }
                                if (it < pf_iters) {
                                    prefetch_l2(lp + 12 * WINDOW); prefetch_l2(lp + 13 * WINDOW);
                                    prefetch_l2(lp + 14 * WINDOW); prefetch_l2(lp + 15 * WINDOW);
#ifdef VCFX_PF1
                                    prefetch_l1(lp + 8 * WINDOW); prefetch_l1(lp + 9 * WINDOW);
                                    prefetch_l1(lp + 10 * WINDOW); prefetch_l1(lp + 11 * WINDOW);
#endif
                                }
                                lp += 4 * WINDOW;
                            }
#undef VCFX_T1_ROUND
                            const uint32_t rounds = 2u * it + (state == 2 ? 1u : 0u);
                            const uint32_t N = 8u * rounds;
                            const uint32_t ys = accf - N * pat;
                            const uint32_t sa = ys & 0xFFFFu, sb = ys >> 16;
                            if (OP == OP_AF) ta += sa + sb;
                            else {
                                const uint32_t y2 = acc2 - N * (pat * pat) - 2u * pat * ys;
                                const uint32_t sab = (y2 - sa) >> 17;
                                hetp += sa + sb - 2u * sab; hap += sab;
                            }
                            n_real += 256u * rounds; wb += 2 * WINDOW * rounds;
                            if (state == 2) { const uint4 t_ = cur; cur = nx2; nxt = nx3; nx2 = t_; la_c = la2; la_n = la3; }
                            else { la_c = la0; la_n = la1; }
                            if (state != 0) break;
                        }
                        bool finished = false;
#pragma unroll 1
                        for (int k = 0; k < 2; ++k) {
                            uint32_t y0 = __funnelshift_rc(cur.x, cur.y, sh_u) ^ pat, y1 = __funnelshift_rc(cur.y, cur.z, sh_u) ^ pat;
                            uint32_t y2 = __funnelshift_rc(cur.z, cur.w, sh_u) ^ pat, y3 = __funnelshift_rc(cur.w, la_c, sh_u) ^ pat;
                            const uint32_t b0 = y0 & 0xFFFEFFFEu, b1 = y1 & 0xFFFEFFFEu, b2 = y2 & 0xFFFEFFFEu, b3 = y3 & 0xFFFEFFFEu;
                            const unsigned fb = __ballot_sync(FULL, (b0 | b1 | b2 | b3) != 0);
                            if (fb == 0) {
                                t1_tally<OP>(y0, y1, y2, y3, accp, hetp, hap);
                                n_real += 128; wb += WINDOW;
                                cur = nxt; nxt = nx2; nx2 = ld16(tin + wb + 2 * WINDOW + 16 * lane); la_c = la_n;
                                continue;
                            }
                            const int Lf = __ffs(fb) - 1;
                            const uint32_t kf_l = b0 ? 0u : b1 ? 1u : b2 ? 2u : 3u;
                            const uint32_t yf_l = b0 ? y0 : b1 ? y1 : b2 ? y2 : y3;
                            const uint32_t kf = __shfl_sync(FULL, kf_l, Lf), yf = __shfl_sync(FULL, yf_l, Lf);
                            if (((yf ^ 0x03000000u) & 0xFFFEFFFEu) == 0) {
                                const uint32_t keep = lane < Lf ? 4u : (lane == Lf ? kf + 1u : 0u);
                                y0 = keep > 0 ? (y0 & 0x00010001u) : 0u;
                                y1 = keep > 1 ? (y1 & 0x00010001u) : 0u;
                                y2 = keep > 2 ? (y2 & 0x00010001u) : 0u;
                                y3 = keep > 3 ? (y3 & 0x00010001u) : 0u;
                                t1_tally<OP>(y0, y1, y2, y3, accp, hetp, hap);
                                e = wb + 16u * (uint32_t)Lf + 4u * kf + tau + 4u; found = true; finished = true;
                                n_real += (e - wb - tau) >> 2;
                            }
                            break;
                        }
                        if (OP == OP_AF) { ta += (accp & 0xFFFFu) + (accp >> 16); accp = 0; }
                        if (finished) break;
                    }
                    if (VAR == 1 && OP == OP_AF && lat_possible && !digits_tried && !found && (first_win || prev_ok)) {
                        digits_tried = true;
                        uint32_t da = 0, db = 0, dt = 0, de = 0;
                        if (line_digits<OP_AF>(tin, wb, first_win ? tab8 + 1u : wb + tau + 1u, nrel, strip_cr, da, db, dt, de)) {
                            ta += da; tb += db; e = de; found = true;
                            break;
                        }
                        cur = ld16(tin + wb + 16 * lane); nxt = ld16(tin + wb + WINDOW + 16 * lane); nx2 = ld16(tin + wb + 2 * WINDOW + 16 * lane);
                    }
                    const uint32_t pb = wb + 16 * lane;
                    uint32_t la = __shfl_down_sync(FULL, cur.x, 1);
                    const uint32_t nx0 = __shfl_sync(FULL, nxt.x, 0);
                    if (lane == 31) la = nx0;
                    bool done = false, nl_done = false;
                    if (!done && t1_on && (first_win || prev_ok)) {
                        if (!first_win) {
                            const uint32_t n0 = eq_bytes(cur.x, C_NL), n1 = eq_bytes(cur.y, C_NL);
                            const uint32_t n2 = eq_bytes(cur.z, C_NL), n3 = eq_bytes(cur.w, C_NL);
                            const unsigned ebal = __ballot_sync(FULL, (n0 | n1 | n2 | n3) != 0);
                            nl_done = true;
                            if (ebal) {
                                const int src = __ffs(ebal) - 1;
                                int k = first_byte(n0, n1, n2, n3);
                                k = __shfl_sync(FULL, k, src);
                                e = wb + 16 * src + k; found = true;
                            }
                        }
                        if ((first_win || found) && (!found || ((e - tau) & 3u) == 0)) {
                            const uint32_t lo = first_win ? tab8 : 0u, hi = found ? e : ~0u;
                            const uint32_t kk = lane_keep16(pb, lo, hi);
                            const uint32_t k0 = (nib80(kk, 0) >> 7) * 0xFFu, k1 = (nib80(kk, 1) >> 7) * 0xFFu;
                            const uint32_t k2 = (nib80(kk, 2) >> 7) * 0xFFu, k3 = (nib80(kk, 3) >> 7) * 0xFFu;
                            const uint32_t k4 = (range_mask(pb + 16, lo, hi) >> 7) * 0xFFu;
                            const uint32_t fill0 = 0x30003009u | (sep0 << 16);
                            const uint32_t fill = __funnelshift_l(fill0, fill0, 8u * tau);
                            done = t1_eval<OP>((cur.x & k0) | (fill & ~k0), (cur.y & k1) | (fill & ~k1),
                                               (cur.z & k2) | (fill & ~k2), (cur.w & k3) | (fill & ~k3),
                                               (la & k4) | (fill & ~k4), sh_u, pat, accp, hetp, hap);
                            if (done) {
                                const int A = (int)max(lo, wb), B = (int)min(hi, wb + WINDOW);
                                const int t = (int)tau;
                                n_real += (uint32_t)(max(0, (B + 3 - t) >> 2) - max(0, (A + 3 - t) >> 2));
                            }
                        }
                    }
                    unsigned gbal = FULL;
                    if (!done) {
                        uint32_t packed = 0;
                        uint32_t sh_lane = 0;
                        if (s_tag[wid] != ls + 1u) { s_tag[wid] = ls + 1u; s_odd[wid] = 0; s_reg[wid] = 0; }
                        const bool qm = lat_possible && !first_win && s_odd[wid] >= 2;
                        uint32_t irr = 0;
                        const bool lat = lat_possible && !qm && lane_lattice<OP>(cur.x, cur.y, cur.z, cur.w, la, packed, sh_lane);
                        gbal = lat_possible ? __ballot_sync(FULL, lat && sh_lane == sh_u) : 0u;
                        uint32_t m0, m1, m2, m3;
                        const uint32_t n0 = eq_bytes(cur.x, C_NL);
                        m0 = eq_bytes(cur.x, C_TAB); m1 = eq_bytes(cur.y, C_TAB);
                        m2 = eq_bytes(cur.z, C_TAB); m3 = eq_bytes(cur.w, C_TAB);
                        if (first_win) clip4(m0, m1, m2, m3, pb, tab8, found ? e : ~0u);
                        else {
                            if (!nl_done) {
                                const uint32_t n1 = eq_bytes(cur.y, C_NL), n2 = eq_bytes(cur.z, C_NL), n3 = eq_bytes(cur.w, C_NL);
                                const unsigned ebal = __ballot_sync(FULL, (n0 | n1 | n2 | n3) != 0);
                                if (ebal) {
                                    const int src = __ffs(ebal) - 1;
                                    int k = first_byte(n0, n1, n2, n3);
                                    k = __shfl_sync(FULL, k, src);
                                    e = wb + 16 * src + k; found = true;
                                }
                            }
                            if (found) {
                                clip4(m0, m1, m2, m3, pb, 0, e);
                            }
                        }
                        bool pg = false;
                        if (lat_possible) { pg = __shfl_up_sync(FULL, (int)lat, 1) != 0; if (lane == 0) pg = prev_ok; }
                        const bool use_lat = lat && (pg || n0 == 0) && !(first_win && tp[7] >= pb);
                        if (use_lat) {
                            if (!found || pb < e) {
                                if (OP == OP_AF) { ta += packed; tb += 8; }
                                else {
                                    const uint32_t het = (packed >> 8) & 0xFF, ha = packed >> 16;
                                    ta += (packed & 0xFF) - het - ha; tb += het; tc += ha;
                                }
                            }
                        } else {
                            if (m0 | m1 | m2 | m3) {
                                bool handled = false;
                                if (__popc(m0) + __popc(m1) + __popc(m2) + __popc(m3) == 1 && gt_index == 0) {
                                    const int B = first_byte(m0, m1, m2, m3);
                                    const uint32_t lo_ = B < 4 ? cur.x : B < 8 ? cur.y : B < 12 ? cur.z : cur.w;
                                    const uint32_t hi_ = B < 4 ? cur.y : B < 8 ? cur.z : B < 12 ? cur.w : la;
                                    const uint32_t q = __funnelshift_rc(lo_, hi_, 8u * (uint32_t)((B & 3) + 1));
                                    const uint32_t b0 = q & 0xFF, b1 = (q >> 8) & 0xFF, b2 = (q >> 16) & 0xFF, b3 = q >> 24;
                                    if (OP == OP_AF) {
                                        const bool t3 = (b3 == '\t' || b3 == ':' || b3 == '\n');
                                        if (is_dig(b0) && is_sep(b1) && is_dig(b2) && t3) {
                                            tb += 2; ta += (uint32_t)(b0 != '0') + (uint32_t)(b2 != '0'); handled = true;
                                        } else if (b0 == '.' && is_sep(b1) && b2 == '.' && t3) { handled = true; irr = 1; }
                                    } else {
                                        if (is_dig(b0) && is_sep(b1) && is_dig(b2) && !is_dig(b3)) {
                                            if (b0 <= '1' && b2 <= '1') { const uint32_t c = (b0 - '0') + (b2 - '0'); ta += (c == 0); tb += (c == 1); tc += (c == 2); }
                                            handled = true;
                                        } else if (b0 == '.') { handled = true; irr = 1; }
                                    }
                                }
                                if (!handled) {
                                    const uint4 r = lane_samples_generic<OP>(cur.x, cur.y, cur.z, cur.w, la, m0, m1, m2, m3,
                                                                             tin + pb, strip_cr, gt_index);
                                    ta += r.x; tb += r.y; tc += r.z; irr = r.w;
                                }
                            }
                        }
                        if (qm) {
                            const unsigned reg = __any_sync(FULL, irr != 0) ? 0u : s_reg[wid] + 1u;
                            s_reg[wid] = reg;
                            if (reg >= 8) { s_reg[wid] = 0; s_odd[wid] = 0; done = true; }
                        }
                    }
                    if (found) break;
                    s_odd[wid] = done ? 0u : s_odd[wid] + 1u;
                    prev_ok = (gbal >> 31) != 0;
                    first_win = false;
                    wb += WINDOW; cur = nxt; nxt = nx2; nx2 = ld16(tin + wb + 2 * WINDOW + 16 * lane);
                }
                if (OP == OP_AF) { ta += (accp & 0xFFFFu) + (accp >> 16); if (lane == 0) tb += 2u * n_real; }
                else { ta -= hetp + hap; if (lane == 0) ta += n_real; tb += hetp; tc += hap; }
            }
            const bool ac_sizing_only = (OP == OP_AC) && P.ac_spec && P.ac_pass == 0;
            if (OP == OP_AC && !hash && tabs >= 9 && !ac_sizing_only) {
                uint2 *scr = P.col_scratch + (size_t)(blockIdx.x * WARPS_PER_CTA + wid) * P.max_col;
                bool firstw = true;
                bool summed = false;
                if (P.ac_fmt == AC_AGG && P.ac_ident && !found && tp[8] - tp[7] == 3 && ldb(tin + tp[7] + 1) == 'G' && ldb(tin + tp[7] + 2) == 'T') {
                    uint32_t da = 0, db = 0, dt = 0, de = 0;
                    if (line_digits<OP_AC>(tin, wb, tp[8] + 1u, nrel, false, da, db, dt, de) &&
                        (uint32_t)__reduce_add_sync(FULL, dt) + (uint32_t)tabs <= 8u + P.n_sel) {
                        ta = db - da; tb = da; tabs += (int)__reduce_add_sync(FULL, dt); e = de; found = true; summed = true;
                    }
                }
                if (!summed)
                for (;;) {
                    const uint32_t pb = wb + 16 * lane;
                    uint32_t m0, m1, m2, m3;
                    int r0;
                    if (firstw) { m0 = t0; m1 = t1; m2 = t2; m3 = t3; r0 = rank0; }
                    else {
                        m0 = eq_bytes(cur.x, C_TAB); m1 = eq_bytes(cur.y, C_TAB);
                        m2 = eq_bytes(cur.z, C_TAB); m3 = eq_bytes(cur.w, C_TAB);
                        const uint32_t n0 = eq_bytes(cur.x, C_NL), n1 = eq_bytes(cur.y, C_NL);
                        const uint32_t n2 = eq_bytes(cur.z, C_NL), n3 = eq_bytes(cur.w, C_NL);
                        const unsigned ebal = __ballot_sync(FULL, (n0 | n1 | n2 | n3) != 0);
                        if (ebal) {
                            const int src = __ffs(ebal) - 1;
                            int k = first_byte(n0, n1, n2, n3);
                            k = __shfl_sync(FULL, k, src);
                            e = wb + 16 * src + k; found = true;
                            clip4(m0, m1, m2, m3, pb, 0, e);
                        }
                        const int cnt = __popc(m0) + __popc(m1) + __popc(m2) + __popc(m3);
                        const int incl = warp_incl_scan(cnt, lane);
                        r0 = tabs + incl - cnt;
                        tabs += __shfl_sync(FULL, incl, 31);
                    }
                    uint32_t la = __shfl_down_sync(FULL, cur.x, 1);
                    const uint32_t nx0 = __shfl_sync(FULL, nxt.x, 0);
                    if (lane == 31) la = nx0;
                    {
                        const uint32_t ws[5] = {cur.x, cur.y, cur.z, cur.w, la};
                        const uint32_t ms[4] = {m0, m1, m2, m3};
                        int r = r0;
                        WClass lo = classify_word<OP_AC>(ws[0]);
#pragma unroll
                        for (int j = 0; j < 4; ++j) {
                            const WClass hi = classify_word<OP_AC>(ws[j + 1]);
                            uint32_t m = ms[j];
                            if (m) {
                                const bool agg_fast = (P.ac_fmt == AC_AGG) && P.ac_ident;
                                const uint32_t tokl = lo.D | lo.P, tokh = hi.D | hi.P;
                                const uint32_t t1 = down(tokl, tokh, 1), t3 = down(tokl, tokh, 3), s2 = down(lo.S, hi.S, 2);
                                const uint32_t e1 = down(lo.E, hi.E, 1), e2 = down(lo.E, hi.E, 2), e4 = hi.E;
                                const uint32_t d1 = down(lo.D, hi.D, 1), d3 = down(lo.D, hi.D, 3);
                                const uint32_t z1 = down(lo.Z, hi.Z, 1), z3 = down(lo.Z, hi.Z, 3);
                                const uint32_t C = m & t1 & s2 & t3 & e4, any = (m & t1 & e2) | C, quick = (m & e1) | any;
                                const uint32_t R1 = any & z1, R3 = C & z3, A1 = any & d1 & ~z1, A3 = C & d3 & ~z3;
                                const int nm = __popc(m);
                                if (agg_fast && r >= 8 && (uint32_t)(r + nm) <= 8u + P.n_sel) {
                                    ta += __popc(R1) + __popc(R3); tb += __popc(A1) + __popc(A3);
                                    uint32_t rest = m & ~quick;
                                    while (rest) {
                                        const int k = (__ffs(rest) - 1) >> 3;
                                        rest &= rest - 1;
                                        const uint2 v = ac_sample_slow(tin + pb + 4 * j + k + 1);
                                        ta += v.x; tb += v.y;
                                    }
                                    r += nm; m = 0;
                                }
                                while (m) {
                                    const uint32_t bit = m & (0u - m);
                                    const int k = (__ffs(m) - 1) >> 3;
                                    m &= m - 1;
                                    if (r >= 8 && (uint32_t)(r - 8) < P.max_col) {
                                        uint2 v;
                                        if (quick & bit) v = make_uint2(((R1 & bit) ? 1u : 0u) + ((R3 & bit) ? 1u : 0u),
                                                                        ((A1 & bit) ? 1u : 0u) + ((A3 & bit) ? 1u : 0u));
                                        else v = ac_sample_slow(tin + pb + 4 * j + k + 1);
                                        if (agg_fast) { if ((uint32_t)(r - 8) < P.n_sel) { ta += v.x; tb += v.y; } }
                                        else scr[r - 8] = v;
                                    }
                                    ++r;
                                }
                            }
                            lo = hi;
                        }
                    }
                    if (found) break;
                    firstw = false;
                    wb += WINDOW; cur = nxt; nxt = nx2; nx2 = ld16(tin + wb + 2 * WINDOW + 16 * lane);
                }
                __syncwarp();
            }
            uint32_t ib_alt = 0, ib_good = 0; bool ib_line = false;
            if (OP == OP_IB && !hash && tabs >= 9 && (a0 + ls >= P.valid_from)) {
                int ok = 0;
                if (lane == 0) {
                    const uint32_t as = tp[3] + 1, ae = tp[4];
                    ok = (P.mode == MODE_FILE) ? (ae > as) : 1;
                    for (uint32_t q = as; q < ae && ok; ++q) if (ldb(tin + q) == ',') ok = 0;
                }
                ib_line = __shfl_sync(FULL, ok, 0) != 0;
            }
            int ds_gi = -1;
            if (OP == OP_DS && !hash && tabs >= 9) {
                ds_gi = gt_index_of(tin + tp[7] + 1, tin + tp[8]);
                ib_line = ds_gi >= 0;
            }
            if ((OP == OP_IB || OP == OP_DS) && ib_line) {
                const uint32_t first = tp[8] + 1u, tq = tp[8] & 3u;
                uint8_t *codes = P.ib_codes + (((a0 + ls) & ~3ULL) + ((((first + 3u) >> 2) - 1u) & 3u));
                bool firstw = true, lat = true;
                for (;;) {
                    const uint32_t pb = wb + 16 * lane;
                    uint32_t la = __shfl_down_sync(FULL, cur.x, 1);
                    const uint32_t nx0 = __shfl_sync(FULL, nxt.x, 0);
                    if (lane == 31) la = nx0;
                    if (!firstw && lat && (OP == OP_IB || ds_gi == 0)) {
                        const uint32_t nl_any = eq_bytes(cur.x, C_NL) | eq_bytes(cur.y, C_NL) | eq_bytes(cur.z, C_NL) | eq_bytes(cur.w, C_NL);
                        if (!__any_sync(FULL, nl_any != 0)) {
                            const uint32_t sh8 = 8u * (tq + 1u);
                            const uint32_t u0 = __funnelshift_rc(cur.x, cur.y, sh8), u1 = __funnelshift_rc(cur.y, cur.z, sh8);
                            const uint32_t u2 = __funnelshift_rc(cur.z, cur.w, sh8), u3 = __funnelshift_rc(cur.w, la, sh8);
                            const uint32_t uu[4] = {u0, u1, u2, u3};
                            uint32_t bad = 0, pk = 0;
#pragma unroll
                            for (int j = 0; j < 4; ++j) {
                                const uint32_t u = uu[j];
                                bad |= (eq_bytes(u, C_TAB) ^ 0x80000000u) | eq_bytes(u, C_NL);
                                const uint32_t b1 = (u >> 8) & 0xFFu;
                                if (OP == OP_IB) {
                                    const bool quick = ((u & 0x00FE00FEu) == 0x00300030u) && (b1 == '/' || b1 == '|');
                                    pk |= (quick ? ((u & 1u) + ((u >> 16) & 1u)) : IB_NONE) << (8 * j);
                                } else {
                                    const uint32_t d0 = (u & 0xFFu) - '0', d2 = ((u >> 16) & 0xFFu) - '0';
                                    const bool quick = d0 <= 9u && d2 <= 9u && (b1 == '/' || b1 == '|');
                                    pk |= (quick ? ((d0 ? 1u : 0u) + (d2 ? 1u : 0u)) : IB_NONE) << (8 * j);
                                }
                            }
                            const int j0 = tabs - 8;
                            bool okl = bad == 0 && j0 == (int)((wb + tq + 1u - first) >> 2) && (OP == OP_DS || (uint32_t)(j0 + 4 * lane + 4) <= P.n_sel);
                            if (lane == 0) okl = okl && ((eq_bytes(cur.x, C_TAB) & (0xFFFFFFFFu >> (24u - 8u * tq))) == (0x80u << (8u * tq)));
                            if (__all_sync(FULL, okl)) {
                                *reinterpret_cast<uint32_t *>(codes + j0 + 4 * lane) = pk;
                                const uint32_t nn = (uint32_t)__popc(eq_bytes(pk, IB_NONE * 0x01010101u));
                                if (OP == OP_IB) { ib_good += 4u - nn; ib_alt += dp4a_u(pk, 0x01010101u, 0u) - 3u * nn; }
                                else ib_alt += nn;
                                tabs += 128;
                                wb += WINDOW; cur = nxt; nxt = nx2; nx2 = ld16(tin + wb + 2 * WINDOW + 16 * lane);
                                if (((wb >> 9) & 7u) == 0) {
                                    const uint32_t pf = wb + 8 * WINDOW + 128 * lane;
                                    if (pf < nrel) prefetch_l2(tin + pf);
                                }
                                continue;
                            }
                            lat = false;
                        }
                    }
                    uint32_t m0, m1, m2, m3;
                    int r0;
                    if (firstw) { m0 = t0; m1 = t1; m2 = t2; m3 = t3; r0 = rank0; }
                    else {
                        m0 = eq_bytes(cur.x, C_TAB); m1 = eq_bytes(cur.y, C_TAB);
                        m2 = eq_bytes(cur.z, C_TAB); m3 = eq_bytes(cur.w, C_TAB);
                        const uint32_t n0 = eq_bytes(cur.x, C_NL), n1 = eq_bytes(cur.y, C_NL);
                        const uint32_t n2 = eq_bytes(cur.z, C_NL), n3 = eq_bytes(cur.w, C_NL);
                        const unsigned ebal = __ballot_sync(FULL, (n0 | n1 | n2 | n3) != 0);
                        if (ebal) {
                            const int src = __ffs(ebal) - 1;
                            int k = first_byte(n0, n1, n2, n3);
                            k = __shfl_sync(FULL, k, src);
                            e = wb + 16 * src + k; found = true;
                            clip4(m0, m1, m2, m3, pb, 0, e);
                        }
                        const int cnt = __popc(m0) + __popc(m1) + __popc(m2) + __popc(m3);
                        const int incl = warp_incl_scan(cnt, lane);
                        r0 = tabs + incl - cnt;
                        tabs += __shfl_sync(FULL, incl, 31);
                    }
                    {
                        const uint32_t wsd[5] = {cur.x, cur.y, cur.z, cur.w, la};
                        const uint32_t ms[4] = {m0, m1, m2, m3};
                        int r = r0;
#pragma unroll
                        for (int j = 0; j < 4; ++j) {
                            uint32_t m = ms[j];
                            while (m) {
                                const int k = (__ffs(m) - 1) >> 3;
                                m &= m - 1;
                                if (r >= 8 && (OP == OP_DS || (uint32_t)(r - 8) < P.n_sel)) {
                                    const uint32_t q = __funnelshift_rc(wsd[j], wsd[j + 1], 8u * (uint32_t)(k + 1));
                                    const uint32_t b1 = (q >> 8) & 0xFFu, b3 = q >> 24;
                                    uint32_t code;
                                    if (OP == OP_IB) {
                                        if ((q & 0x00FE00FEu) == 0x00300030u && (b1 == '/' || b1 == '|') && (b3 - '0') > 9u) code = (q & 1u) + ((q >> 16) & 1u);
                                        else code = ib_sample_code(tin + pb + 4 * j + k + 1);
                                        if (code < IB_NONE) { ib_alt += code; ++ib_good; }
                                    } else {
                                        const uint32_t d0 = (q & 0xFFu) - '0', d2 = ((q >> 16) & 0xFFu) - '0';
                                        if (ds_gi == 0 && d0 <= 9u && d2 <= 9u && (b1 == '/' || b1 == '|') && (b3 == '\t' || b3 == ':' || b3 == '\n'))
                                            code = (d0 ? 1u : 0u) + (d2 ? 1u : 0u);
                                        else code = ds_sample_code(tin + pb + 4 * j + k + 1, P.mode == MODE_FILE, ds_gi);
                                        if (code == IB_NONE) ++ib_alt;
                                    }
                                    codes[r - 8] = (uint8_t)code;
                                }
                                ++r;
                            }
                        }
                    }
                    if (found) break;
                    firstw = false;
                    wb += WINDOW; cur = nxt; nxt = nx2; nx2 = ld16(tin + wb + 2 * WINDOW + 16 * lane);
                    if (((wb >> 9) & 7u) == 0) {
                        const uint32_t pf = wb + 8 * WINDOW + 128 * lane;
                        if (pf < nrel) prefetch_l2(tin + pf);
                    }
                }
            }
            bool md_flag = false, md_any = false;
            if (OP == OP_MD && !hash && tabs >= 9) {
                const uint32_t lo = tp[8] + 1;
                bool firstw = true;
                for (;;) {
                    const uint32_t pb = wb + 16 * lane;
                    if (!firstw) {
                        const uint32_t n0 = eq_bytes(cur.x, C_NL), n1 = eq_bytes(cur.y, C_NL);
                        const uint32_t n2 = eq_bytes(cur.z, C_NL), n3 = eq_bytes(cur.w, C_NL);
                        const unsigned ebal = __ballot_sync(FULL, (n0 | n1 | n2 | n3) != 0);
                        if (ebal) {
                            const int src = __ffs(ebal) - 1;
                            int k = first_byte(n0, n1, n2, n3);
                            k = __shfl_sync(FULL, k, src);
                            e = wb + 16 * src + k; found = true;
                        }
                    }
                    if (!md_flag) {
                        uint32_t d0 = eq_bytes(cur.x, C_DOT), d1 = eq_bytes(cur.y, C_DOT);
                        uint32_t d2 = eq_bytes(cur.z, C_DOT), d3 = eq_bytes(cur.w, C_DOT);
                        if (firstw || found) {
                            const uint32_t l = firstw ? lo : 0u, h = found ? e : ~0u;
                            clip4(d0, d1, d2, d3, pb, l, h);
                        }
                        const bool any = (d0 | d1 | d2 | d3) != 0;
                        if (__any_sync(FULL, any)) {
                            md_any = true;
                            const bool hit = any && md_lane_dots(tin + pb, d0, d1, d2, d3, strip_cr);
                            md_flag = __any_sync(FULL, hit);
                        }
                    }
                    if (found) break;
                    firstw = false;
                    wb += WINDOW; cur = nxt; nxt = nx2; nx2 = ld16(tin + wb + 2 * WINDOW + 16 * lane);
                    if (((wb >> 9) & 7u) == 0) {
                        const uint32_t pf = wb + 8 * WINDOW + 128 * lane;
                        if (pf < nrel) prefetch_l2(tin + pf);
                    }
                }
            }
            bool nr_all = false;
            if ((OP == OP_NR || OP == OP_PC || OP == OP_GQ) && !hash && tabs >= 9 && (a0 + ls >= P.valid_from)) {
                const int gi_ = gt_index_of(tin + tp[7] + 1, tin + tp[8]);
                const int gi = (OP == OP_PC && gi_ < 0 && P.mode == MODE_FILE && tp[8] == tp[7] + 1 && (a0 + ls) < P.fmt0_until) ? 0 : gi_;
                GqQuery gq; gq.q = P.gq_query; gq.len = P.gq_len; gq.a = P.gq_a; gq.b = P.gq_b; gq.strict = P.gq_strict != 0;
                if (gi >= 0) {
                    nr_all = true;
                    const uint32_t lo = tp[8];
                    const bool file_mode = P.mode == MODE_FILE;
                    bool firstw = true;
                    for (;;) {
                        const uint32_t pb = wb + 16 * lane;
                        if (!firstw) {
                            const uint32_t n0 = eq_bytes(cur.x, C_NL), n1 = eq_bytes(cur.y, C_NL);
                            const uint32_t n2 = eq_bytes(cur.z, C_NL), n3 = eq_bytes(cur.w, C_NL);
                            const unsigned ebal = __ballot_sync(FULL, (n0 | n1 | n2 | n3) != 0);
                            if (ebal) {
                                const int src = __ffs(ebal) - 1;
                                int k = first_byte(n0, n1, n2, n3);
                                k = __shfl_sync(FULL, k, src);
                                e = wb + 16 * src + k; found = true;
                            }
                        }
                        bool lat_pass = false;
                        if (nr_all && !firstw && !found && gi == 0) {
                            const uint32_t tq = lo & 3u, sh8 = 8u * (tq + 1u);
                            uint32_t la = __shfl_down_sync(FULL, cur.x, 1);
                            const uint32_t nx0 = __shfl_sync(FULL, nxt.x, 0);
                            if (lane == 31) la = nx0;
                            const uint32_t uu[4] = {__funnelshift_rc(cur.x, cur.y, sh8), __funnelshift_rc(cur.y, cur.z, sh8),
                                                    __funnelshift_rc(cur.z, cur.w, sh8), __funnelshift_rc(cur.w, la, sh8)};
                            uint32_t badw = 0;
#pragma unroll
                            for (int j = 0; j < 4; ++j) {
                                const uint32_t u = uu[j];
                                if (OP == OP_NR) badw |= (u != 0x09302F30u && u != 0x09307C30u) ? 1u : 0u;
                                else if (OP == OP_GQ) {
                                    badw |= (eq_bytes(u, C_TAB) ^ 0x80000000u) | eq_bytes(u, C_NL) | (eq_bytes(u, 0x3A3A3A3Au) & 0x00808080u);
                                    badw |= gq_match3(u, gq) ? 1u : 0u;
                                }
                                else {
                                    badw |= (eq_bytes(u, C_TAB) ^ 0x80000000u) | eq_bytes(u, C_NL);
                                    badw |= ((eq_bytes(u, C_DOT) | eq_bytes(u, 0x3A3A3A3Au)) & 0x00800080u) | ((u ^ 0x00007C00u) & 0x0000FF00u);
                                }
                            }
                            if (lane == 0) badw |= (eq_bytes(cur.x, C_TAB) & (0xFFFFFFFFu >> (24u - 8u * tq))) ^ (0x80u << (8u * tq));
                            lat_pass = __all_sync(FULL, badw == 0);
                        }
                        if (nr_all && !lat_pass) {
                            uint32_t m0 = eq_bytes(cur.x, C_TAB), m1 = eq_bytes(cur.y, C_TAB);
                            uint32_t m2 = eq_bytes(cur.z, C_TAB), m3 = eq_bytes(cur.w, C_TAB);
                            if (firstw || found) clip4(m0, m1, m2, m3, pb, firstw ? lo : 0u, found ? e : ~0u);
                            uint32_t m16 = ((m0 * 0x00204081u) >> 28) | (((m1 * 0x00204081u) >> 24) & 0xF0u) |
                                           (((m2 * 0x00204081u) >> 20) & 0xF00u) | (((m3 * 0x00204081u) >> 16) & 0xF000u);
                            bool bad = false;
                            while (m16) {
                                const uint8_t *sp = tin + pb + __ffs(m16);
                                m16 &= m16 - 1u;
                                const uint32_t *s4 = reinterpret_cast<const uint32_t *>((uintptr_t)sp & ~(uintptr_t)3);
                                const uint32_t q = __funnelshift_r(__ldg(s4), __ldg(s4 + 1), 8u * (uint32_t)((uintptr_t)sp & 3));
                                const uint32_t g3 = q & 0x00FFFFFFu, b3 = q >> 24;
                                if (OP == OP_NR) {
                                    const bool quick = gi == 0 && (g3 == 0x00302F30u || g3 == 0x00307C30u) && (b3 == '\t' || b3 == ':');
                                    if (!quick && !nr_sample_homref(sp, file_mode, gi)) bad = true;
                                } else if (OP == OP_GQ) {
                                    const uint32_t ends = eq_bytes(q, C_TAB) | eq_bytes(q, C_NL) | eq_bytes(q, 0x3A3A3A3Au);
                                    if (gi == 0 && (ends & 0x00808080u) == 0 && (ends & 0x80000000u)) { if (gq_match3(q, gq)) bad = true; }
                                    else if (gq_sample_match(sp, gi, gq)) bad = true;
                                } else {
                                    const uint32_t b0 = q & 0xFFu, b2 = (q >> 16) & 0xFFu;
                                    const bool e0 = b0 == '.' || b0 == '\t' || b0 == '\n' || b0 == ':' || b0 == '\r';
                                    const bool e2 = b2 == '.' || b2 == '\t' || b2 == '\n' || b2 == ':' || b2 == '\r';
                                    const bool quick = gi == 0 && ((q >> 8) & 0xFFu) == '|' && !e0 && !e2 && (b3 == '\t' || b3 == ':');
                                    if (!quick && !pc_sample_phased(sp, file_mode, gi)) bad = true;
                                }
                            }
                            if (__any_sync(FULL, bad)) nr_all = false;
                        }
                        if (found) break;
                        firstw = false;
                        wb += WINDOW; cur = nxt; nxt = nx2; nx2 = ld16(tin + wb + 2 * WINDOW + 16 * lane);
                        if (((wb >> 9) & 7u) == 0) {
                            const uint32_t pf = wb + 8 * WINDOW + 128 * lane;
                            if (pf < nrel) prefetch_l2(tin + pf);
                        }
                    }
                }
            }
            uint32_t wcount = 0;
            while (!found) {
                wb += WINDOW; cur = nxt; nxt = nx2; nx2 = ld16(tin + wb + 2 * WINDOW + 16 * lane);
                if ((++wcount & 7u) == 0) {
                    const uint32_t pf = wb + 8 * WINDOW + 128 * lane;
                    if (pf < nrel) prefetch_l2(tin + pf);
                }
                uint32_t n0 = eq_bytes(cur.x, C_NL), n1 = eq_bytes(cur.y, C_NL);
                uint32_t n2 = eq_bytes(cur.z, C_NL), n3 = eq_bytes(cur.w, C_NL);
                unsigned ebal = __ballot_sync(FULL, (n0 | n1 | n2 | n3) != 0);
                if (ebal) {
                    int src = __ffs(ebal) - 1;
                    int k = first_byte(n0, n1, n2, n3);
                    k = __shfl_sync(FULL, k, src);
                    e = wb + 16 * src + k; found = true;
                }
            }

            ++nlines;
            uint32_t ee = e;
            if (strip_cr && e > ls && ldb(tin + e - 1) == '\r') ee = e - 1;
            if (OP == OP_VC) {
                if (e != ls && !hash) {
                    if (tabs >= 7) VCFX_COUNT(C_ROWS, 1);
                    else {
                        VCFX_COUNT(C_SHORT, 1);
                        if (lane == 0) {
                            unsigned long long key = ((unsigned long long)tile << 32) | (nlines - 1);
                            atomicMin(&P.stats->first_short_key, key);
                            unsigned long long slot = atomicAdd(&P.stats->n_events, 1ULL);
                            if (slot < P.ev_cap) P.events[slot] = key;
                        }
                    }
                }
            } else if ((OP == OP_AF || OP == OP_HWE) && ee != ls && !hash) {
                uint32_t ra_ = 0, rb_ = 0, rc_ = 0;
                if (do_samples) {
                    ra_ = __reduce_add_sync(FULL, ta); rb_ = __reduce_add_sync(FULL, tb);
                    if (OP == OP_HWE) rc_ = __reduce_add_sync(FULL, tc);
                }
                bool row = false;
                if (OP == OP_AF) {
                    if (a0 + ls < P.valid_from) VCFX_COUNT(C_PRE, 1);
                    else if (P.mode == MODE_FILE) {
                        VCFX_COUNT(C_DATA, 1);
                        if (tabs >= 9) row = gt_index >= 0;
                        else if (tabs == 8 && tp[7] + 1 < ee) row = gt_index_of(tin + tp[7] + 1, tin + ee) >= 0;
                    } else {
                        int nf = tabs + ((ldb(tin + ee - 1) == '\t') ? 0 : 1);
                        if (nf < 9) VCFX_COUNT(C_SHORT, 1);
                        else {
                            VCFX_COUNT(C_DATA, 1);
                            if (tabs >= 9) row = gt_index >= 0;
                            else row = gt_index_of(tin + tp[7] + 1, tin + ee) >= 0;
                        }
                    }
                } else {
                    VCFX_COUNT(C_DATA, 1);
                    if (tabs >= 9 && do_samples) {
                        bool comma = false;
                        for (uint32_t q = tp[3] + 1; q < tp[4]; ++q) comma |= (ldb(tin + q) == ',');
                        row = !comma;
                        if (P.mode == MODE_FILE)
                            row = row && (tp[0] > ls) && (tp[1] > tp[0] + 1) && (tp[4] > tp[3] + 1) && (tp[8] + 1 < ee);
                    }
                }
                if (row) {
                    const uint32_t prefix_len = tp[4] + 1 - ls;
                    const uint32_t row_len = prefix_len + ((OP == OP_AF) ? 7u : 9u);
                    unsigned long long slot = 0;
                    if (lane == 0) slot = alloc_slot(ws.rec_base, ws.rec_used, P.stats);
                    slot = __shfl_sync(FULL, slot, 0);
                    if (slot < P.rec_cap) {
                        if (lane == 0) {
                            Rec r; r.tile = tile; r.ls_rel = (uint32_t)(a0 + ls - a); r.prefix_len = prefix_len;
                            r.off_in_tile = (uint32_t)out_bytes; r.a = ra_; r.b = rb_; r.c = rc_; r.d = 0;
                            P.recs[slot] = r;
                        }
                        if (prefix_len <= 32 && (uint32_t)lane < prefix_len) P.rec_prefix[slot * 32 + lane] = (uint8_t)ldb(tin + ls + lane);
                    }
                    out_bytes += row_len; VCFX_COUNT(C_ROWS, 1);
                }
            }
            else if (OP == OP_AC) {
                if (e != ls && !hash) {
                    if (P.ac_pass == 0) VCFX_COUNT(C_DATA, 1);
                    const uint2 *scr = P.col_scratch + (size_t)(blockIdx.x * WARPS_PER_CTA + wid) * P.max_col;
                    const uint32_t ns_parsed = tabs >= 9 ? (uint32_t)(tabs - 8) : 0u;
                    uint32_t n_rows = P.n_sel;
                    if (P.ac_fmt != AC_TEXT_MT) {
                        uint32_t ns_f = 0;
                        if (tabs >= 9 && tp[8] + 1 < e) ns_f = ns_parsed - ((ldb(tin + e - 1) == '\t') ? 1u : 0u);
                        uint32_t lo_ = 0, hi_ = P.n_sel;
                        while (lo_ < hi_) { const uint32_t mid = (lo_ + hi_) >> 1; if (P.sel_col[mid] < ns_f) lo_ = mid + 1; else hi_ = mid; }
                        n_rows = lo_;
                    }
                    const uint32_t extra_tabs = tabs >= 5 ? 0u : (uint32_t)(5 - tabs);
                    const uint32_t prefix_src = tabs >= 5 ? tp[4] + 1 - ls : e - ls;
                    const uint32_t prefix_len = prefix_src + extra_tabs;
                    if (P.ac_fmt == AC_AGG) {
                        uint32_t sr = ta, sa = tb;
                        if (!P.ac_ident) {
                            sr = 0; sa = 0;
                            for (uint32_t i = lane; i < n_rows; i += 32) {
                                const uint32_t c = P.sel_col[i];
                                if (c < ns_parsed) { const uint2 v = scr[c]; sr += v.x; sa += v.y; }
                            }
                        }
                        sr = __reduce_add_sync(FULL, sr); sa = __reduce_add_sync(FULL, sa);
                        const uint32_t row_len = prefix_len + dec_len((int)sr) + 1 + dec_len((int)sa) + 1 + dec_len((int)n_rows) + 1;
                        if (lane == 0) {
                            unsigned long long slot = alloc_slot(ws.rec_base, ws.rec_used, P.stats);
                            if (slot < P.rec_cap) {
                                Rec r; r.tile = tile; r.ls_rel = (uint32_t)(a0 + ls - a); r.prefix_len = prefix_src;
                                r.off_in_tile = (uint32_t)out_bytes; r.a = sr; r.b = sa; r.c = n_rows; r.d = extra_tabs;
                                P.recs[slot] = r;
                            }
                        }
                        out_bytes += row_len; VCFX_COUNT(C_ROWS, 1);
                    } else {
                        uint8_t *stage0 = ws.stage0;
                        uint32_t n_rows_done = 0;
                        unsigned long long opos = (P.ac_pass ? P.tile_base[tile] : 0ULL) + out_bytes;
                        const bool text = (P.ac_fmt != AC_BIN);
                        if (ac_sizing_only) {
                            out_bytes += (unsigned long long)n_rows * (prefix_len + 4u) + (P.name_off[n_rows] - P.name_off[0]);
                            n_rows_done = n_rows; n_rows = 0;
                        }
                        const unsigned long long out_limit = P.ac_pass ? min((unsigned long long)P.out_cap, P.tile_base[tile] + P.tile_out[tile]) : 0ULL;
                        const uint32_t NL = P.name_len;
                        const bool fast_line = P.ac_pass && text && NL != 0u && extra_tabs == 0u && prefix_src <= 40u && prefix_src >= 1u;
                        const uint32_t L = prefix_src + NL + 4u;
                        if (fast_line) {
                            __syncwarp();
                            if (lane < 20) {
                                uint32_t w = 0;
#pragma unroll
                                for (uint32_t bb = 0; bb < 4; ++bb) {
                                    const uint32_t pp = 4u * (uint32_t)lane + bb;
                                    uint32_t byte = 0;
                                    if (pp >= 3u && pp < 3u + prefix_src) byte = ldb(tin + ls + pp - 3u);
                                    else if (pp >= 3u + L && pp < 6u + L) byte = ldb(tin + ls + pp - 3u - L);
                                    w |= byte << (8u * bb);
                                }
                                ws.u[lane] = w;
                            }
                            __syncwarp();
                        }
                        for (uint32_t i0 = 0; i0 < n_rows; i0 += 32) {
                            const uint32_t i = i0 + lane;
                            int vr = 0, va = 0; uint32_t len = 0, noff = 0, nlen = 0;
                            if (i < n_rows) {
                                const uint32_t c = P.ac_ident ? i : P.sel_col[i];
                                if (c < ns_parsed) { const uint2 v = scr[c]; vr = (int)v.x; va = (int)v.y; }
                                if (P.ac_fmt != AC_TEXT_FWD) { vr = (int)(int8_t)vr; va = (int)(int8_t)va; }
                            }
                            const bool fast = fast_line && __all_sync(FULL, i >= n_rows || ((uint32_t)vr <= 9u && (uint32_t)va <= 9u));
                            uint32_t off, btot;
                            if (fast) { off = (uint32_t)lane * L; btot = min(32u, n_rows - i0) * L; }
                            else {
                                if (i < n_rows) {
                                    if (text) {
                                        noff = P.name_off[i]; nlen = P.name_off[i + 1] - noff;
                                        len = prefix_len + nlen + dec_len(vr) + 1 + dec_len(va) + 1;
                                    } else len = 2;
                                }
                                const int incl = warp_incl_scan((int)len, lane);
                                off = (uint32_t)incl - len;
                                btot = (uint32_t)__shfl_sync(FULL, incl, 31);
                            }
                            if (P.ac_pass && opos + btot > out_limit) {
                                if (lane == 0) atomicOr(&P.stats->overflow, 4ULL);
                            } else
                            if (fast) {
                                uint32_t *sw = reinterpret_cast<uint32_t *>(stage0);
                                const uint32_t o = (uint32_t)((uintptr_t)(P.out + opos) & 15) + (uint32_t)lane * L;
                                const uint32_t sh = 8u * (3u - (o & 3u));
                                const uint32_t a_prev = __shfl_up_sync(FULL, (uint32_t)va, 1);
                                if (i < n_rows) {
                                    const uint32_t tl = 0x000A0009u | ((48u + a_prev) << 8);
                                    const uint4 nm = __ldg(P.names16 + i);
                                    const uint32_t T = (48u + (uint32_t)vr) | (0x09u << 8) | ((48u + (uint32_t)va) << 16) | (0x0Au << 24);
                                    const uint32_t ti = NL >> 2, ts = 8u * (NL & 3u);
                                    const uint32_t Tlo = T << ts, Thi = ts ? (T >> (32u - ts)) : 0u;
                                    const uint32_t v0 = nm.x | (ti == 0 ? Tlo : 0u);
                                    const uint32_t v1 = nm.y | (ti == 1 ? Tlo : 0u) | (ti == 0 ? Thi : 0u);
                                    const uint32_t v2 = nm.z | (ti == 2 ? Tlo : 0u) | (ti == 1 ? Thi : 0u);
                                    const uint32_t v3 = nm.w | (ti == 3 ? Tlo : 0u) | (ti == 2 ? Thi : 0u);
                                    const uint32_t q = (3u + prefix_src) >> 2, sv = 8u * ((3u + prefix_src) & 3u);
                                    const uint32_t s0 = __funnelshift_l(0u, v0, sv), s1 = __funnelshift_l(v0, v1, sv), s2 = __funnelshift_l(v1, v2, sv);
                                    const uint32_t s3 = __funnelshift_l(v2, v3, sv), s4 = __funnelshift_l(v3, 0u, sv);
                                    const uint32_t nw = ((o & 3u) + L + 3u) >> 2;
                                    uint32_t *dw = sw + (o >> 2);
                                    for (uint32_t k = 0; k + 1u < q; ++k) {
                                        const uint32_t lo_ = ws.u[k] | (k == 0u ? tl : 0u), hi_ = ws.u[k + 1];
                                        dw[k] = __funnelshift_r(lo_, hi_, sh);
                                    }
                                    const uint32_t c_1 = ws.u[q - 1] | (q == 1u ? tl : 0u);
                                    const uint32_t c0 = ws.u[q] | s0, c1 = ws.u[q + 1] | s1, c2 = ws.u[q + 2] | s2, c3 = ws.u[q + 3] | s3, c4 = ws.u[q + 4] | s4, c5 = ws.u[q + 5];
                                    if (q - 1u < nw) dw[q - 1] = __funnelshift_r(c_1, c0, sh);
                                    if (q < nw) dw[q] = __funnelshift_r(c0, c1, sh);
                                    if (q + 1u < nw) dw[q + 1] = __funnelshift_r(c1, c2, sh);
                                    if (q + 2u < nw) dw[q + 2] = __funnelshift_r(c2, c3, sh);
                                    if (q + 3u < nw) dw[q + 3] = __funnelshift_r(c3, c4, sh);
                                    if (q + 4u < nw) dw[q + 4] = __funnelshift_r(c4, c5, sh);
                                }
                                __syncwarp();
                                if (P.ac_bulk) warp_flush_smem_bulk(P.out + opos, stage0 + (uint32_t)((uintptr_t)(P.out + opos) & 15), btot, lane);
                                else warp_flush_smem(P.out + opos, stage0 + (uint32_t)((uintptr_t)(P.out + opos) & 15), btot, lane);
                                __syncwarp();
                            } else
                            if (P.ac_pass) {
                                const bool staged = btot <= AC_STAGE;
                                uint8_t *stage = stage0 + (uint32_t)((uintptr_t)(P.out + opos) & 15);
                                uint8_t *d = staged ? stage + off : P.out + opos + off;
                                if (i < n_rows) {
                                    if (text) {
                                        const uint8_t *src = tin + ls;
                                        for (uint32_t k = 0; k < prefix_src; ++k) d[k] = (uint8_t)ldb(src + k);
                                        d += prefix_src;
                                        for (uint32_t k = 0; k < extra_tabs; ++k) *d++ = '\t';
                                        const uint8_t *nm = P.names + noff;
                                        for (uint32_t k = 0; k < nlen; ++k) d[k] = (uint8_t)ldb(nm + k);
                                        d += nlen;
                                        d = put_dec(d, vr); *d++ = '\t'; d = put_dec(d, va); *d++ = '\n';
                                    } else { d[0] = (uint8_t)vr; d[1] = (uint8_t)va; }
                                }
                                if (staged) { __syncwarp(); warp_flush_smem(P.out + opos, stage, btot, lane); __syncwarp(); }
                            }
                            opos += btot; out_bytes += btot;
                        }
                        if (P.ac_pass == 0) VCFX_COUNT(C_ROWS, ac_sizing_only ? n_rows_done : n_rows);
                    }
                }
            }
            else if (OP == OP_IX) {
                if (ee != ls && (a0 + ls >= P.valid_from)) {
                    uint32_t c_off = 0, c_len = 0; long long pos = 0; bool ok = false;
                    if (lane == 0) ok = ix_parse_line(tin + ls, tin + ee, P.mode == MODE_FILE, c_off, c_len, pos);
                    ok = __shfl_sync(FULL, (int)ok, 0) != 0;
                    if (ok) {
                        uint32_t row_len = 0;
                        if (lane == 0) {
                            row_len = c_len + 1u + dec_len64(pos) + 1u + dec_len64((long long)(P.file_offset + a0 + ls)) + 1u;
                            unsigned long long slot = alloc_slot(ws.rec_base, ws.rec_used, P.stats);
                            if (slot < P.rec_cap) {
                                Rec r; r.tile = tile; r.ls_rel = (uint32_t)(a0 + ls - a); r.prefix_len = c_len;
                                r.off_in_tile = (uint32_t)out_bytes; r.a = c_off; r.b = 0;
                                r.c = (uint32_t)((unsigned long long)pos & 0xFFFFFFFFULL); r.d = (uint32_t)((unsigned long long)pos >> 32);
                                P.recs[slot] = r;
                            }
                        }
                        out_bytes += __shfl_sync(FULL, row_len, 0); VCFX_COUNT(C_ROWS, 1);
                    }
                }
            }
            else if (OP == OP_IB) {
                if (ib_line) {
                    const uint32_t alt = __reduce_add_sync(FULL, ib_alt), good = __reduce_add_sync(FULL, ib_good);
                    if (P.mode != MODE_FILE || tp[8] + 1 < ee) {
                        VCFX_COUNT(C_DATA, 1);
                        if (good >= 2) VCFX_COUNT(C_ROWS, 1);
                        if (lane == 0) {
                            const unsigned long long slot = alloc_slot(ws.rec_base, ws.rec_used, P.stats);
                            if (slot < P.rec_cap) {
                                Rec r; r.tile = tile; r.ls_rel = (uint32_t)(a0 + ls - a); r.prefix_len = 0;
                                r.off_in_tile = (uint32_t)out_bytes; r.a = alt; r.b = good;
                                r.c = min((uint32_t)(tabs - 8), P.n_sel); r.d = (((tp[8] + 4u) >> 2) - 1u) & 3u;
                                P.recs[slot] = r;
                            }
                        }
                        out_bytes += 1;
                    }
                }
            }
            else if (OP == OP_PC) {
                const bool term = (a0 + e) < n;
                const uint32_t raw_end = term ? e + 1 : e;
                const bool file_mode = P.mode == MODE_FILE;
                const uint32_t cend = file_mode ? ee : e;
                const bool data = (cend != ls) && !hash;
                bool drop = false; uint32_t why = 0;
                if (data) {
                    VCFX_COUNT(C_DATA, 1);
                    if (a0 + ls < P.valid_from) { drop = true; why = 1; VCFX_COUNT(C_PRE, 1); }
                    else if (file_mode) {
                        if (tabs < 8 || tp[7] + 1 >= cend) { drop = true; why = 2; }
                        else if (tabs == 8) { drop = true; why = gt_index_of(tin + tp[7] + 1, tin + cend) < 0 ? 0u : 2u; }
                        else if (!nr_all) drop = true;
                    } else {
                        if (tabs < 9) { drop = true; why = 2; }
                        else if (gt_index_of(tin + tp[7] + 1, tin + tp[8]) < 0) { drop = true; why = 3; }
                        else if (!nr_all) drop = true;
                    }
                }
                if (data && !drop) VCFX_COUNT(C_ROWS, 1);
                if (drop) {
                    VCFX_COUNT(C_FLAG, 1);
                    if (lane == 0) {
                        const unsigned long long slot = atomicAdd(&P.stats->n_events, 1ULL);
                        if (slot < P.ev_cap) P.events[slot] = ((unsigned long long)(a0 + ls) << 2) | why;
                    }
                }
                if (drop || cend != e || !term) {
                    const uint32_t content_len = drop ? 0u : cend - ls, mod_len = drop ? 0u : content_len + 1u;
                    if (lane == 0) {
                        unsigned long long slot = alloc_slot(ws.rec_base, ws.rec_used, P.stats);
                        if (slot < P.rec_cap) {
                            Rec r; r.tile = tile; r.ls_rel = (uint32_t)(a0 + ls - a); r.prefix_len = (uint32_t)(a0 + md_prev_end - a);
                            r.off_in_tile = (uint32_t)out_bytes; r.a = 0; r.b = NR_PLAIN; r.c = content_len; r.d = mod_len;
                            P.recs[slot] = r;
                        }
                    }
                    out_bytes += (ls - md_prev_end) + mod_len;
                    md_prev_end = raw_end;
                }
                md_add_nl = false;
                md_last_end = raw_end;
            }
            else if (OP == OP_DS) {
                if (ee != ls && !hash) {
                    VCFX_COUNT(C_DATA, 1);
                    if (tabs < 9) {
                        VCFX_COUNT(C_SHORT, 1);
                    } else {
                        const uint32_t nna = __reduce_add_sync(FULL, ib_alt);
                        const uint32_t prefix_len = tp[4] + 1 - ls;
                        uint32_t ncols = (uint32_t)(tabs - 8);
                        if (ldb(tin + ee - 1) == '\t') --ncols;
                        const uint32_t dlen = ds_gi < 0 ? 2u : (ncols ? 2u * ncols - 1u + nna : 0u);
                        if (lane == 0) {
                            const unsigned long long slot = alloc_slot(ws.rec_base, ws.rec_used, P.stats);
                            if (slot < P.rec_cap) {
                                Rec r; r.tile = tile; r.ls_rel = (uint32_t)(a0 + ls - a); r.prefix_len = prefix_len;
                                r.off_in_tile = (uint32_t)out_bytes; r.a = ncols; r.b = dlen; r.c = ds_gi < 0 ? 1u : 0u;
                                r.d = (((tp[8] + 4u) >> 2) - 1u) & 3u;
                                P.recs[slot] = r;
                            }
                        }
                        out_bytes += prefix_len + dlen + 1u; VCFX_COUNT(C_ROWS, 1);
                    }
                }
            }
            else if (OP == OP_GQ) {
                const bool term = (a0 + e) < n;
                const uint32_t raw_end = term ? e + 1 : e;
                const bool data = (e != ls) && !hash;
                bool drop = (e == ls);
                if (data) {
                    VCFX_COUNT(C_DATA, 1);
                    if (tabs < 8) {
                        drop = true;
                        if (ldb(tin + e - 1) != '\t') {
                            VCFX_COUNT(C_SHORT, 1);
                            if (lane == 0) {
                                const unsigned long long slot = atomicAdd(&P.stats->n_events, 1ULL);
                                if (slot < P.ev_cap) P.events[slot] = ((unsigned long long)(a0 + ls) << 2) | 2ULL;
                            }
                        }
                    }
                    else if (gt_index_of(tin + tp[7] + 1, tin + (tabs >= 9 ? tp[8] : e)) < 0) drop = true;
                    else drop = (tabs < 9) || nr_all;
                }
                if (data && !drop) VCFX_COUNT(C_ROWS, 1);
                if (drop || !term) {
                    const uint32_t content_len = drop ? 0u : e - ls, mod_len = drop ? 0u : content_len + 1u;
                    if (lane == 0) {
                        unsigned long long slot = alloc_slot(ws.rec_base, ws.rec_used, P.stats);
                        if (slot < P.rec_cap) {
                            Rec r; r.tile = tile; r.ls_rel = (uint32_t)(a0 + ls - a); r.prefix_len = (uint32_t)(a0 + md_prev_end - a);
                            r.off_in_tile = (uint32_t)out_bytes; r.a = 0; r.b = NR_PLAIN; r.c = content_len; r.d = mod_len;
                            P.recs[slot] = r;
                        }
                    }
                    out_bytes += (ls - md_prev_end) + mod_len;
                    md_prev_end = raw_end;
                }
                md_add_nl = false;
                md_last_end = raw_end;
            }
            else if (OP == OP_NR) {
                const bool term = (a0 + e) < n;
                const uint32_t raw_end = term ? e + 1 : e;
                const bool data = (ee != ls) && !hash;
                if (data) {
                    VCFX_COUNT(C_DATA, 1);
                    if (a0 + ls < P.valid_from) VCFX_COUNT(C_PRE, 1);
                }
                const bool drop = data && nr_all;
                if (data && !drop) VCFX_COUNT(C_ROWS, 1);
                if (drop || ee != e || !term) {
                    const uint32_t content_len = drop ? 0u : ee - ls, mod_len = drop ? 0u : content_len + 1u;
                    if (lane == 0) {
                        unsigned long long slot = alloc_slot(ws.rec_base, ws.rec_used, P.stats);
                        if (slot < P.rec_cap) {
                            Rec r; r.tile = tile; r.ls_rel = (uint32_t)(a0 + ls - a); r.prefix_len = (uint32_t)(a0 + md_prev_end - a);
                            r.off_in_tile = (uint32_t)out_bytes; r.a = 0; r.b = NR_PLAIN; r.c = content_len; r.d = mod_len;
                            P.recs[slot] = r;
                        }
                    }
                    out_bytes += (ls - md_prev_end) + mod_len;
                    md_prev_end = raw_end;
                    if (drop) VCFX_COUNT(C_FLAG, 1);
                }
                md_add_nl = false;
                md_last_end = raw_end;
            }
            else if (OP == OP_MD) {
                const bool term = (a0 + e) < n;
                const uint32_t raw_end = term ? e + 1 : e;
                const bool data = (ee != ls) && !hash;
                if (data) VCFX_COUNT(C_DATA, 1);
                const bool has_samples = data && tabs >= 9;
                if (term && has_samples && md_any && tp[8] + 1 < e && (a0 + ls >= P.valid_from)) VCFX_COUNT(C_DOTS, 1);
                md_add_nl = false;
                if (has_samples && md_flag && tp[8] + 1 < ee) {
                    const uint32_t info_off = tp[6] + 1 - ls, info_len = tp[7] - tp[6] - 1, content_len = ee - ls;
                    uint32_t mod_len;
                    if (info_len == 0 || (info_len == 1 && ldb(tin + tp[6] + 1) == '.')) mod_len = content_len - info_len + 19;
                    else mod_len = content_len + 19 + ((ldb(tin + tp[7] - 1) != ';') ? 1u : 0u);
                    mod_len += 1;
                    if (lane == 0) {
                        unsigned long long slot = alloc_slot(ws.rec_base, ws.rec_used, P.stats);
                        if (slot < P.rec_cap) {
                            Rec r; r.tile = tile; r.ls_rel = (uint32_t)(a0 + ls - a); r.prefix_len = (uint32_t)(a0 + md_prev_end - a);
                            r.off_in_tile = (uint32_t)out_bytes; r.a = info_off; r.b = info_len; r.c = content_len; r.d = mod_len;
                            P.recs[slot] = r;
                        }
                        if (!term) P.stats->last_unterminated_flagged = mod_len;
                    }
                    out_bytes += (ls - md_prev_end) + mod_len;
                    md_prev_end = raw_end;
                    VCFX_COUNT(C_FLAG, 1);
                } else if (!term && P.mode == MODE_STDIN) md_add_nl = true;
                md_last_end = raw_end;
            }
            __syncwarp();
            ls = e + 1;
        }
    VCFX_SAVE_STATE();
    return true;
#undef VCFX_COUNT
#undef VCFX_SAVE_STATE
}

#ifndef VCFX_PARSE_CTAS
#define VCFX_PARSE_CTAS 4
#endif
#ifndef VCFX_AC_CTAS
#define VCFX_AC_CTAS 4
#endif
#ifndef VCFX_GENERAL_CTAS
#define VCFX_GENERAL_CTAS 3
#endif
template <int OP, int VAR>
__global__ void __launch_bounds__(WARPS_PER_CTA * 32, (OP == OP_VC) ? 5 : (VAR == 1 ? VCFX_GENERAL_CTAS : (OP == OP_AC ? VCFX_AC_CTAS : VCFX_PARSE_CTAS)))
vcfx_scan_kernel(const VCFX_GRID_CONSTANT KParams P) {
    __shared__ uint32_t s_tp[WARPS_PER_CTA][12];
    __shared__ __align__(128) uint8_t s_ring[(VCFX_C4_RING && VAR == 1) ? WARPS_PER_CTA * C4_RING : 16];
    __shared__ __align__(8) unsigned long long s_bars[(VCFX_C4_RING && VAR == 1) ? WARPS_PER_CTA * C4_STAGES : 1];
    __shared__ uint32_t s_ring_par[WARPS_PER_CTA];
    __shared__ __align__(16) uint8_t s_stage[(OP == OP_AC) ? WARPS_PER_CTA * (AC_STAGE + 32) : 16];
    __shared__ uint32_t s_u[(OP == OP_AC) ? WARPS_PER_CTA : 1][20];
    const int lane = lane_id();
    const int wid = threadIdx.x >> 5;
    const uint64_t n = P.n;
    const bool strip_cr = (OP == OP_HWE) || (P.mode == MODE_FILE && (OP == OP_AF || OP == OP_VC || OP == OP_MD || OP == OP_NR || OP == OP_PC)) || OP == OP_IX || OP == OP_IB || (OP == OP_DS && P.mode == MODE_FILE);
    if (OP == OP_AC && P.ac_pass && P.stats->overflow) return;
    if (VAR == 1 && P.stats->n_unfinished == 0) return;

    __shared__ unsigned int s_cnt[WARPS_PER_CTA][CNT_SLOTS];
    if (lane < CNT_SLOTS) s_cnt[wid][lane] = 0;
    __syncwarp();
#define VCFX_COUNT(slot, v) do { if (lane == 0) atomicAdd(&s_cnt[wid][slot], (unsigned int)(v)); } while (0)
    __shared__ unsigned long long s_rec_base[WARPS_PER_CTA];
    __shared__ unsigned int s_rec_used[WARPS_PER_CTA];
    __shared__ volatile unsigned int s_odd[WARPS_PER_CTA], s_reg[WARPS_PER_CTA], s_tag[WARPS_PER_CTA];
    if (lane == 0) s_tag[wid] = 0;
    if (lane == 0) { s_rec_base[wid] = 0; s_rec_used[wid] = REC_BLOCK; }
    __syncwarp();
    WarpShared ws;
    ws.tp = s_tp[wid]; ws.stage0 = s_stage + ((OP == OP_AC) ? wid * (AC_STAGE + 32) : 0); ws.cnt = s_cnt[wid]; ws.u = s_u[(OP == OP_AC) ? wid : 0];
    ws.ring = s_ring + ((VCFX_C4_RING && VAR == 1) ? wid * C4_RING : 0); ws.bars = s_bars + ((VCFX_C4_RING && VAR == 1) ? wid * C4_STAGES : 0); ws.ring_par = &s_ring_par[wid];
    if (VCFX_C4_RING && VAR == 1) { if ((threadIdx.x & 31) == 0) s_ring_par[wid] = 0; ring_init(ws.bars, threadIdx.x & 31); }
    ws.rec_base = &s_rec_base[wid]; ws.rec_used = &s_rec_used[wid]; ws.odd = s_odd; ws.reg = s_reg; ws.tag = s_tag;

    for (;;) {
        uint32_t tile = 0;
        if (lane == 0) tile = atomicAdd(VAR == 1 ? P.ticket2 : P.ticket, 1u);
        tile = __shfl_sync(FULL, tile, 0);
        if (tile >= P.n_tiles) break;
        uint32_t resume = RESUME_DONE;
        if (VAR == 1) { resume = P.tile_resume[tile]; if (resume == RESUME_DONE) continue; }

        const uint64_t a = (uint64_t)tile * P.tile_bytes;
        const uint64_t b = min(a + (uint64_t)P.tile_bytes, n);
        const uint64_t a0 = a - (tile ? 16u : 0u);
        const uint8_t *__restrict__ tin = P.in + a0;
        const uint32_t ra = (uint32_t)(a - a0), rb = (uint32_t)(b - a0);
        const uint32_t nrel = (uint32_t)min(n - a0, (uint64_t)0xFFFFFFFFu);

        uint32_t ls = rb;
        if (VAR == 1) ls = resume;
        else if (a == 0) ls = 0;
        else {
            const uint32_t from = ra - 1, to = rb - 1;
            uint32_t wb = from & ~15u;
            while (wb < to) {
                const uint32_t pb = wb + 16 * lane;
                uint4 v = ld16(tin + pb);
                uint32_t m0 = eq_bytes(v.x, C_NL), m1 = eq_bytes(v.y, C_NL), m2 = eq_bytes(v.z, C_NL), m3 = eq_bytes(v.w, C_NL);
                clip4(m0, m1, m2, m3, pb, from, to);
                unsigned bal = __ballot_sync(FULL, (m0 | m1 | m2 | m3) != 0);
                if (bal) {
                    int src = __ffs(bal) - 1;
                    int k = first_byte(m0, m1, m2, m3);
                    k = __shfl_sync(FULL, k, src);
                    ls = wb + 16 * src + k + 1;
                    break;
                }
                wb += WINDOW;
            }
        }

        s_tag[wid] = 0;
        TileState<OP> st;
        st.ls = ls; st.nlines = 0; st.out_bytes = 0; st.md_prev_end = ls; st.md_last_end = ls; st.md_add_nl = false; st.offlattice_lines = 0;
        if (VAR == 1) { st.nlines = P.tile_lines[tile]; st.out_bytes = (typename OutCount<OP>::type)P.tile_out[tile]; }
        const uint32_t lines_before = st.nlines;
        const bool finished = tile_lines<OP, VAR>(P, ws, lane, strip_cr, tile, a, a0, tin, rb, nrel, n, st);
        if (!finished) {
            if (lane == 0) { P.tile_lines[tile] = st.nlines; P.tile_out[tile] = st.out_bytes; P.tile_resume[tile] = st.ls; atomicAdd(&P.stats->n_unfinished, 1ULL); }
            VCFX_COUNT(C_LINES, st.nlines);
            __syncwarp();
            if (lane < CNT_SLOTS) {
                const unsigned int v = s_cnt[wid][lane];
                if (v) { s_cnt[wid][lane] = 0; atomicAdd(reinterpret_cast<unsigned long long *>(P.stats) + lane, (unsigned long long)v); }
            }
            __syncwarp();
            continue;
        }
        const uint32_t nlines = st.nlines;
        typename OutCount<OP>::type out_bytes = st.out_bytes;
        const uint32_t md_prev_end = st.md_prev_end, md_last_end = st.md_last_end;
        const bool md_add_nl = st.md_add_nl;

        if (!(OP == OP_AC && P.ac_pass)) VCFX_COUNT(C_LINES, VAR == 1 ? nlines - lines_before : nlines);
        if (OP == OP_MD || OP == OP_NR || OP == OP_PC || OP == OP_GQ) {
            const uint32_t tail = md_last_end - md_prev_end;
            if (lane == 0) {
                P.tail_start[tile] = (uint32_t)(a0 + md_prev_end - a);
                P.tail_len[tile] = tail | (md_add_nl ? 0x80000000u : 0u);
                P.tail_off[tile] = (uint32_t)out_bytes;
            }
            out_bytes += tail + (md_add_nl ? 1u : 0u);
        }
        if (lane == 0 && !(OP == OP_AC && P.ac_pass)) { P.tile_lines[tile] = nlines; P.tile_out[tile] = out_bytes; }
        if (OP == OP_AC && P.ac_pass && P.ac_spec && lane == 0 && (unsigned long long)out_bytes != P.tile_out[tile]) atomicOr(&P.stats->overflow, 4ULL);
        __syncwarp();
        if (lane < CNT_SLOTS) {
            const unsigned int v = s_cnt[wid][lane];
            if (v) { s_cnt[wid][lane] = 0; atomicAdd(reinterpret_cast<unsigned long long *>(P.stats) + lane, (unsigned long long)v); }
        }
        __syncwarp();
    }
#undef VCFX_COUNT
    __syncwarp();
    {
        const unsigned int used = s_rec_used[wid];
        const unsigned long long slot = s_rec_base[wid] + lane;
        if ((unsigned int)lane >= used && (unsigned int)lane < REC_BLOCK && slot < P.rec_cap) P.recs[slot].tile = REC_INVALID;
    }
}

constexpr uint32_t SCAN_BATCH = 8192;
constexpr uint32_t SCAN_SMEM_WORDS = SCAN_BATCH + SCAN_BATCH / 8;
constexpr size_t SCAN_SMEM_BYTES = 2 * SCAN_SMEM_WORDS * sizeof(unsigned long long);
__device__ __forceinline__ uint32_t scan_pad(uint32_t i) { return i + (i >> 3); }

__global__ void __launch_bounds__(1024)
tile_scan_kernel(const KParams P) {
#ifdef VCFX_EMU
    unsigned long long *scan_smem = static_cast<unsigned long long *>(emu::dyn_smem());
#else
    extern __shared__ unsigned long long scan_smem[];
#endif
    unsigned long long *so = scan_smem, *sl = scan_smem + SCAN_SMEM_WORDS;
    __shared__ unsigned long long ws_o[32], ws_l[32];
    __shared__ unsigned long long carry_o, carry_l;
    const uint32_t tid = threadIdx.x, lane = tid & 31, w = tid >> 5, n_tiles = P.n_tiles;
    if (tid == 0) { carry_o = 0; carry_l = 0; }
    for (uint32_t base = 0; base < n_tiles; base += SCAN_BATCH) {
        const uint32_t cnt = min(SCAN_BATCH, n_tiles - base);
#pragma unroll
        for (uint32_t j = 0; j < SCAN_BATCH / 1024; ++j) {
            const uint32_t i = j * 1024 + tid;
            so[scan_pad(i)] = i < cnt ? P.tile_out[base + i] : 0ULL;
            sl[scan_pad(i)] = i < cnt ? (unsigned long long)P.tile_lines[base + i] : 0ULL;
        }
        __syncthreads();
        unsigned long long vo = 0, vl = 0;
#pragma unroll
        for (uint32_t j = 0; j < 8; ++j) { vo += so[scan_pad(tid * 8 + j)]; vl += sl[scan_pad(tid * 8 + j)]; }
        unsigned long long io = vo, il = vl;
#pragma unroll
        for (int o = 1; o < 32; o <<= 1) {
            const unsigned long long to = __shfl_up_sync(FULL, io, o), tl2 = __shfl_up_sync(FULL, il, o);
            if ((int)lane >= o) { io += to; il += tl2; }
        }
        if (lane == 31) { ws_o[w] = io; ws_l[w] = il; }
        const unsigned long long c_o = carry_o, c_l = carry_l;
        __syncthreads();
        if (w == 0) {
            unsigned long long s_o = ws_o[lane], s_l = ws_l[lane];
            const unsigned long long so0 = s_o, sl0 = s_l;
#pragma unroll
            for (int o = 1; o < 32; o <<= 1) {
                const unsigned long long to = __shfl_up_sync(FULL, s_o, o), tl2 = __shfl_up_sync(FULL, s_l, o);
                if ((int)lane >= o) { s_o += to; s_l += tl2; }
            }
            ws_o[lane] = s_o - so0; ws_l[lane] = s_l - sl0;
            if (lane == 31) { carry_o = c_o + s_o; carry_l = c_l + s_l; }
        }
        __syncthreads();
        unsigned long long ro = c_o + ws_o[w] + (io - vo), rl = c_l + ws_l[w] + (il - vl);
#pragma unroll
        for (uint32_t j = 0; j < 8; ++j) {
            const uint32_t k = scan_pad(tid * 8 + j);
            const unsigned long long a = so[k], b = sl[k];
            so[k] = ro; sl[k] = rl;
            ro += a; rl += b;
        }
        __syncthreads();
#pragma unroll
        for (uint32_t j = 0; j < SCAN_BATCH / 1024; ++j) {
            const uint32_t i = j * 1024 + tid;
            if (i < cnt) { P.tile_base[base + i] = so[scan_pad(i)]; P.line_base[base + i] = sl[scan_pad(i)]; }
        }
        __syncthreads();
    }
    __syncthreads();
    if (tid == 0) P.stats->bytes_out = carry_o;
    __syncthreads();
    unsigned long long nev = P.stats->n_events;
    if (nev > P.ev_cap) nev = P.ev_cap;
    for (unsigned long long i = tid; i < nev && !P.ev_raw; i += 1024) {
        unsigned long long k = P.events[i];
        P.events[i] = P.line_base[k >> 32] + (k & 0xFFFFFFFFULL) + 1ULL;
    }
    if (tid == 0) {
        unsigned long long k = P.stats->first_short_key;
        P.stats->first_short_line = (k == ~0ULL) ? 0ULL : P.line_base[k >> 32] + (k & 0xFFFFFFFFULL) + 1ULL;
        unsigned long long ov = 0;
        if (P.stats->n_recs > P.rec_cap) ov |= 1;
        if (P.stats->bytes_out > P.out_cap) ov |= 2;
        P.stats->overflow = ov;
    }
}

template <int OP>
__global__ void __launch_bounds__(256)
format_rows_kernel(const KParams P) {
    if (P.stats->overflow) return;
    const unsigned long long nrec = P.stats->n_recs;
    if (OP == OP_IX) {
        for (unsigned long long i = blockIdx.x * (unsigned long long)blockDim.x + threadIdx.x; i < nrec;
             i += (unsigned long long)gridDim.x * blockDim.x) {
            const Rec r = P.recs[i];
            if (r.tile == REC_INVALID) continue;
            uint8_t *o = P.out + P.tile_base[r.tile] + r.off_in_tile;
            const uint64_t line_off = (uint64_t)r.tile * P.tile_bytes + r.ls_rel;
            const uint8_t *src = P.in + line_off + r.a;
            for (uint32_t k = 0; k < r.prefix_len; ++k) o[k] = __ldg(src + k);
            o += r.prefix_len;
            *o++ = '\t'; o = put_dec64(o, (long long)(((unsigned long long)r.d << 32) | r.c));
            *o++ = '\t'; o = put_dec64(o, (long long)(P.file_offset + line_off)); *o = '\n';
        }
        return;
    }
    if (OP == OP_AC) {
        for (unsigned long long i = blockIdx.x * (unsigned long long)blockDim.x + threadIdx.x; i < nrec;
             i += (unsigned long long)gridDim.x * blockDim.x) {
            const Rec r = P.recs[i];
            if (r.tile == REC_INVALID) continue;
            uint8_t *o = P.out + P.tile_base[r.tile] + r.off_in_tile;
            const uint8_t *src = P.in + (uint64_t)r.tile * P.tile_bytes + r.ls_rel;
            for (uint32_t k = 0; k < r.prefix_len; ++k) o[k] = __ldg(src + k);
            o += r.prefix_len;
            for (uint32_t k = 0; k < r.d; ++k) *o++ = '\t';
            o = put_dec(o, (int)r.a); *o++ = '\t'; o = put_dec(o, (int)r.b); *o++ = '\t'; o = put_dec(o, (int)r.c); *o = '\n';
        }
        return;
    }
    __shared__ __align__(16) uint8_t rows_sm[8][32][64];
    const int lane = threadIdx.x & 31, wi = threadIdx.x >> 5;
    const unsigned long long warp0 = (blockIdx.x * (unsigned long long)blockDim.x + threadIdx.x) >> 5;
    const unsigned long long nwarps = ((unsigned long long)gridDim.x * blockDim.x) >> 5;
    for (unsigned long long base = warp0 * 32; base < nrec; base += nwarps * 32) {
        const unsigned long long i = base + lane;
        uint8_t *dst = nullptr; const uint8_t *src = nullptr;
        uint32_t plen = 0, tlen = 0;
        bool gather = false;
        Rec r; r.tile = REC_INVALID;
        if (i < nrec) r = P.recs[i];
        if (r.tile != REC_INVALID) {
            dst = P.out + P.tile_base[r.tile] + r.off_in_tile;
            plen = r.prefix_len;
            uint8_t *slot = rows_sm[wi][lane];
            uint32_t at = 0;
            if (plen <= 32) {
                *reinterpret_cast<uint4 *>(slot) = *reinterpret_cast<const uint4 *>(P.rec_prefix + i * 32);
                *reinterpret_cast<uint4 *>(slot + 16) = *reinterpret_cast<const uint4 *>(P.rec_prefix + i * 32 + 16);
                at = plen;
            } else {
                gather = true;
                src = P.in + (uint64_t)r.tile * P.tile_bytes + r.ls_rel;
            }
            char num[24]; int nl;
            if (OP == OP_AF) {
                double v = af_value(r.a, r.b);
                nl = (P.mode == MODE_FILE) ? fmt_af_file(v, num) : fmt_af_stdin(v, num);
            } else {
                double pv = hwe_pvalue((int)r.a, (int)r.b, (int)r.c);
                nl = (P.mode == MODE_FILE) ? fmt_p_file(pv, num) : fmt_p_stdin(pv, num);
            }
            for (int k = 0; k < nl; ++k) slot[at + k] = (uint8_t)num[k];
            slot[at + nl] = '\n';
            tlen = at + nl + 1;
        }
        __syncwarp();
        const unsigned gm = __ballot_sync(FULL, gather);
#pragma unroll 4
        for (int j = 0; j < 32; ++j) {
            uint8_t *d = reinterpret_cast<uint8_t *>(__shfl_sync(FULL, (unsigned long long)dst, j));
            const uint32_t tl = __shfl_sync(FULL, tlen, j);
            if ((gm >> j) & 1u) {
                const uint8_t *sj = reinterpret_cast<const uint8_t *>(__shfl_sync(FULL, (unsigned long long)src, j));
                const uint32_t pl = __shfl_sync(FULL, plen, j);
                for (uint32_t k = lane; k < pl; k += 32) d[k] = __ldg(sj + k);
                d += pl;
            }
            if ((uint32_t)lane < tl) d[lane] = rows_sm[wi][j][lane];
            if ((uint32_t)lane + 32 < tl) d[lane + 32] = rows_sm[wi][j][lane + 32];
        }
        __syncwarp();
    }
}

__device__ __forceinline__ void warp_copy_words(uint8_t *dst, const uint8_t *src, uint32_t n, int lane) {
    if (n == 0) return;
    const uint32_t head = min(n, (uint32_t)((4 - ((uintptr_t)dst & 3)) & 3));
    if (lane < (int)head) dst[lane] = __ldg(src + lane);
    dst += head; src += head; n -= head;
    const uint32_t nw = n >> 2;
    const uint32_t sh = 8u * (uint32_t)((uintptr_t)src & 3);
    const uint32_t *s4 = reinterpret_cast<const uint32_t *>(src - (sh >> 3));
    uint32_t *d4 = reinterpret_cast<uint32_t *>(dst);
    if (sh == 0) { for (uint32_t i = lane; i < nw; i += 32) d4[i] = __ldg(s4 + i); }
    else { for (uint32_t i = lane; i < nw; i += 32) d4[i] = __funnelshift_r(__ldg(s4 + i), __ldg(s4 + i + 1), sh); }
    const uint32_t done = nw << 2, rem = n - done;
    if (lane < (int)rem) dst[done + lane] = __ldg(src + done + lane);
}

template <int WS>
__device__ __forceinline__ uint4 realign16(const uint4 A, const uint4 B, uint32_t bs) {
    const uint32_t w[8] = {A.x, A.y, A.z, A.w, B.x, B.y, B.z, B.w};
    uint4 o;
    o.x = __funnelshift_r(w[WS], w[WS + 1], bs); o.y = __funnelshift_r(w[WS + 1], w[WS + 2], bs);
    o.z = __funnelshift_r(w[WS + 2], w[WS + 3], bs); o.w = __funnelshift_r(w[WS + 3], w[WS + 4], bs);
    return o;
}
template <int WS>
__device__ __forceinline__ void copy16_loop(uint4 *__restrict__ d16, const uint4 *__restrict__ s16, uint32_t nq, uint32_t bs, int lane) {
    uint32_t i = lane;
    for (; i + 96 < nq; i += 128) {
        const uint4 A0 = __ldg(s16 + i), B0 = __ldg(s16 + i + 1), A1 = __ldg(s16 + i + 32), B1 = __ldg(s16 + i + 33);
        const uint4 A2 = __ldg(s16 + i + 64), B2 = __ldg(s16 + i + 65), A3 = __ldg(s16 + i + 96), B3 = __ldg(s16 + i + 97);
        d16[i] = realign16<WS>(A0, B0, bs); d16[i + 32] = realign16<WS>(A1, B1, bs);
        d16[i + 64] = realign16<WS>(A2, B2, bs); d16[i + 96] = realign16<WS>(A3, B3, bs);
    }
    for (; i < nq; i += 32) d16[i] = realign16<WS>(__ldg(s16 + i), __ldg(s16 + i + 1), bs);
}

__device__ __forceinline__ void warp_copy(uint8_t *dst, const uint8_t *src, uint32_t n, int lane) {
    if (n < 256) { warp_copy_words(dst, src, n, lane); return; }
    const uint32_t head = (uint32_t)((16 - ((uintptr_t)dst & 15)) & 15);
    warp_copy_words(dst, src, head, lane);
    dst += head; src += head; n -= head;
    const uint32_t nq = n >> 4;
    const uint32_t mis = (uint32_t)((uintptr_t)src & 15);
    const uint4 *__restrict__ s16 = reinterpret_cast<const uint4 *>(src - mis);
    uint4 *__restrict__ d16 = reinterpret_cast<uint4 *>(dst);
    const uint32_t bs = 8u * (mis & 3u);
    if (mis == 0) {
        uint32_t i = lane;
        for (; i + 96 < nq; i += 128) {
            const uint4 a = __ldg(s16 + i), b = __ldg(s16 + i + 32), c = __ldg(s16 + i + 64), d = __ldg(s16 + i + 96);
            d16[i] = a; d16[i + 32] = b; d16[i + 64] = c; d16[i + 96] = d;
        }
        for (; i < nq; i += 32) d16[i] = __ldg(s16 + i);
    }
    else switch (mis >> 2) {
        case 0: copy16_loop<0>(d16, s16, nq, bs, lane); break;
        case 1: copy16_loop<1>(d16, s16, nq, bs, lane); break;
        case 2: copy16_loop<2>(d16, s16, nq, bs, lane); break;
        default: copy16_loop<3>(d16, s16, nq, bs, lane); break;
    }
    warp_copy_words(dst + (nq << 4), src + (nq << 4), n - (nq << 4), lane);
}

__global__ void __launch_bounds__(256)
md_copy_kernel(const KParams P) {
    if (P.stats->overflow) return;
    const int lane = threadIdx.x & 31;
    const unsigned long long nrec = P.stats->n_recs, items = nrec + P.n_tiles;
    const unsigned long long nwarps = (unsigned long long)gridDim.x * (blockDim.x >> 5);
    for (unsigned long long it = (unsigned long long)blockIdx.x * (blockDim.x >> 5) + (threadIdx.x >> 5); it < items; it += nwarps) {
        if (it < nrec) {
            const Rec r = P.recs[it];
            if (r.tile == REC_INVALID) continue;
            const uint8_t *base = P.in + (uint64_t)r.tile * P.tile_bytes;
            uint8_t *o = P.out + P.tile_base[r.tile] + r.off_in_tile;
            const uint32_t gap = r.ls_rel - r.prefix_len;
            warp_copy(o, base + r.prefix_len, gap, lane);
            o += gap;
            const uint8_t *ln = base + r.ls_rel;
            if (r.b == NR_PLAIN) {
                warp_copy(o, ln, r.c, lane);
                if (r.d > r.c && lane == 0) o[r.c] = '\n';
                continue;
            }
            warp_copy(o, ln, r.a, lane);
            o += r.a;
            const uint8_t *info = ln + r.a;
            const bool replace = (r.b == 0) || (r.b == 1 && __ldg(info) == '.');
            uint32_t w = 0;
            if (!replace) {
                warp_copy(o, info, r.b, lane);
                w = r.b;
                if (__ldg(info + r.b - 1) != ';') { if (lane == 0) o[w] = ';'; ++w; }
            }
            if (lane < 19) o[w + lane] = (uint8_t)"MISSING_GENOTYPES=1"[lane];
            w += 19;
            o += w;
            const uint32_t rest = r.c - r.a - r.b;
            warp_copy(o, info + r.b, rest, lane);
            if (lane == 0) o[rest] = '\n';
        } else {
            const uint32_t t = (uint32_t)(it - nrec);
            const uint32_t len = P.tail_len[t] & 0x7FFFFFFFu;
            uint8_t *o = P.out + P.tile_base[t] + P.tail_off[t];
            warp_copy(o, P.in + (uint64_t)t * P.tile_bytes + P.tail_start[t], len, lane);
            if ((P.tail_len[t] >> 31) && lane == 0) o[len] = '\n';
        }
    }
}

__global__ void __launch_bounds__(256)
ib_rows_kernel(const KParams P) {
    if (P.stats->overflow) return;
    const unsigned long long R = P.stats->bytes_out;
    const uint32_t npan = (P.n_sel + 31u) >> 5;
    if (R * 32ULL * npan > P.ib_panel_cap) {
        if (blockIdx.x == 0 && threadIdx.x == 0) atomicOr(&P.stats->overflow, 16ULL);
        return;
    }
    const int lane = threadIdx.x & 31;
    const bool file_mode = P.mode == MODE_FILE;
    const unsigned long long nrec = P.stats->n_recs;
    const unsigned long long nwarps = (unsigned long long)gridDim.x * (blockDim.x >> 5);
    for (unsigned long long i = (unsigned long long)blockIdx.x * (blockDim.x >> 5) + (threadIdx.x >> 5); i < nrec; i += nwarps) {
        const Rec r = P.recs[i];
        if (r.tile == REC_INVALID) continue;
        const unsigned long long rank = P.tile_base[r.tile] + r.off_in_tile;
        const uint8_t *src = P.ib_codes + ((((unsigned long long)r.tile * P.tile_bytes + r.ls_rel) & ~3ULL) + r.d);
        const uint32_t mis = (uint32_t)((uintptr_t)src & 3u), sh = 8u * mis;
        const uint32_t *s4 = reinterpret_cast<const uint32_t *>(src - mis);
        const uint32_t fill = file_mode ? IB_ABSENT : IB_NONE;
        uint32_t absent = (file_mode && r.c < P.n_sel) ? 1u : 0u;
        for (uint32_t s0 = 16u * (uint32_t)lane; s0 < (npan << 5); s0 += 512u) {
            uint32_t w[4];
            if (s0 + 16u <= r.c) {
                const uint32_t *q = s4 + (s0 >> 2);
                const uint32_t a0 = q[0], a1 = q[1], a2 = q[2], a3 = q[3], a4 = mis ? q[4] : 0u;
                w[0] = __funnelshift_r(a0, a1, sh); w[1] = __funnelshift_r(a1, a2, sh); w[2] = __funnelshift_r(a2, a3, sh); w[3] = __funnelshift_r(a3, a4, sh);
            } else {
#pragma unroll
                for (int j = 0; j < 4; ++j) {
                    uint32_t v = 0;
#pragma unroll
                    for (int b = 0; b < 4; ++b) {
                        const uint32_t sidx = s0 + 4u * j + b;
                        const uint32_t c = sidx < r.c ? (uint32_t)src[sidx] : (sidx < P.n_sel ? fill : IB_NONE);
                        v |= c << (8 * b);
                    }
                    w[j] = v;
                }
            }
#pragma unroll
            for (int j = 0; j < 4; ++j) {
                const uint32_t ab = eq_bytes(w[j], IB_ABSENT * 0x01010101u) >> 7;
                if (file_mode) absent |= ab; else w[j] -= ab;
                w[j] <<= 4;
            }
            *reinterpret_cast<uint4 *>(P.ib_panels + ((unsigned long long)(s0 >> 5) * R + rank) * 32ULL + (s0 & 31u)) = make_uint4(w[0], w[1], w[2], w[3]);
        }
        const bool any_absent = __any_sync(FULL, absent != 0);
        if (lane == 0) {
            IbMeta m;
            for (int c = 0; c < 4; ++c) { m.e[c].x = 0.0; m.e[c].inc = 0; m.e[c].flag = 0; }
            m.e[IB_NONE].flag = any_absent ? 1u : 0u;
            const int alt_sum = (int)r.a, n_good = (int)r.b;
            if (n_good >= 2) {
                const double global_p = ddiv((double)alt_sum, dmul(2.0, (double)n_good));
                for (int c = 0; c < 3; ++c) {
                    const double freq = (P.flags & IB_F_GLOBAL) ? global_p : ddiv((double)(alt_sum - c), dmul(2.0, (double)(n_good - 1)));
                    if ((P.flags & IB_F_SKIP_BOUNDARY) && (freq <= 0.0 || freq >= 1.0)) { if (P.flags & IB_F_COUNT_BOUNDARY) m.e[c].inc = 1u; }
                    else { m.e[c].inc = (c == 1) ? 0x10001u : 1u; m.e[c].x = dmul(dmul(2.0, freq), dsub(1.0, freq)); }
                }
            }
            P.ib_rows[rank] = m;
        }
    }
}

__global__ void __launch_bounds__(256)
ds_rows_kernel(const KParams P) {
    __shared__ __align__(16) uint8_t s_stage[8][AC_STAGE + 32];
    if (P.stats->overflow) return;
    const int lane = threadIdx.x & 31;
    uint8_t *stage = s_stage[threadIdx.x >> 5];
    const unsigned long long nrec = P.stats->n_recs;
    const unsigned long long nwarps = (unsigned long long)gridDim.x * (blockDim.x >> 5);
    for (unsigned long long i = (unsigned long long)blockIdx.x * (blockDim.x >> 5) + (threadIdx.x >> 5); i < nrec; i += nwarps) {
        const Rec r = P.recs[i];
        if (r.tile == REC_INVALID) continue;
        const unsigned long long line = (unsigned long long)r.tile * P.tile_bytes + r.ls_rel;
        uint8_t *o = P.out + P.tile_base[r.tile] + r.off_in_tile;
        if (P.tile_base[r.tile] + r.off_in_tile + r.prefix_len + r.b + 1u > P.out_cap) continue;
        warp_copy(o, P.in + line, r.prefix_len, lane);
        o += r.prefix_len;
        if (r.c) { if (lane == 0) { o[0] = 'N'; o[1] = 'A'; o[2] = '\n'; } continue; }
        const uint8_t *codes = P.ib_codes + ((line & ~3ULL) + r.d);
        uint32_t na_before = 0, flushed = 0;
        uint32_t base = (uint32_t)((uintptr_t)o & 15u);
        for (uint32_t sb = 0; sb < r.a; sb += 128) {
          uint32_t c4[4];
#pragma unroll
          for (int u = 0; u < 4; ++u) { const uint32_t sx = sb + 32u * u + (uint32_t)lane; c4[u] = sx < r.a ? (uint32_t)codes[sx] : 0u; }
#pragma unroll
          for (int u = 0; u < 4; ++u) {
            const uint32_t s0 = sb + 32u * u;
            if (s0 >= r.a) break;
            const uint32_t s = s0 + (uint32_t)lane;
            const bool in = s < r.a;
            const uint32_t c = c4[u];
            const bool na = in && c >= IB_NONE;
            const unsigned nb = __ballot_sync(FULL, na);
            if (in) {
                uint8_t *w = stage + base + (2u * s + na_before + (uint32_t)__popc(nb & ((1u << lane) - 1u)) - flushed);
                if (s) w[-1] = ',';
                if (na) { w[0] = 'N'; w[1] = 'A'; } else w[0] = (uint8_t)('0' + c);
            }
            na_before += (uint32_t)__popc(nb);
            const uint32_t s_end = min(s0 + 32u, r.a);
            const uint32_t written = 2u * s_end - 1u + na_before;
            if (written - flushed + 96u + 16u > AC_STAGE) {
                __syncwarp();
                warp_flush_smem(o + flushed, stage + base, written - flushed, lane);
                __syncwarp();
                flushed = written; base = (uint32_t)((uintptr_t)(o + flushed) & 15u);
            }
          }
        }
        if (lane == 0) stage[base + (r.b - flushed)] = '\n';
        __syncwarp();
        warp_flush_smem(o + flushed, stage + base, r.b + 1u - flushed, lane);
// ... 181 lines not shown
```

Baseline: 2640.

## Fuse launch memsets into prologue kernel and redefine tile ownership by line starts

Replaces the per-launch memsets and the host-to-device stats copy with a single small prologue kernel that writes the pad, resets tickets and initializes DevStats. Tile ownership now begins at the line start before the tile boundary, found by a backward warp search, instead of a forward newline scan. Resume state becomes a uint4 and record offsets become signed so they can point before the tile start. The scan kernel also exits early for variant-count runs with no events. The change cuts small launch-prologue operations and gaps, at the cost of touching many offset computations across kernels.

```diff
diff --git a/profiles/step_timeline.py b/profiles/step_timeline.py
--- /dev/null
+++ b/profiles/step_timeline.py
@@ -0,0 +1,77 @@
+from __future__ import annotations
+
+import argparse
+import json
+import sys
+from pathlib import Path
+
+ROOT = Path(__file__).resolve().parent.parent
+sys.path.insert(0, str(ROOT))
+
+
+def main():
+    ap = argparse.ArgumentParser()
+    ap.add_argument("out_dir")
+    ap.add_argument("--tile", type=int, default=0)
+    ap.add_argument("--steps", type=int, default=3, help="profiled steps; the last one is printed")
+    args = ap.parse_args()
+    out = Path(args.out_dir); out.mkdir(parents=True, exist_ok=True)
+
+    import numpy as np
+    import torch
+    from torch.profiler import ProfilerActivity, profile
+
+    import bench
+    from vcfx_b200 import api, synth
+
+    dev = torch.device("cuda", 0)
+    torch.cuda.set_device(0)
+    sh = bench.Shard(torch, np, synth, api, dev, 2, 0, bench.C2_VARIANTS, True, 16)
+    out_cap = 64 << 20
+    d_out = torch.empty(out_cap, dtype=torch.uint8, device=dev)
+    tstream = torch.cuda.Stream(device=dev)
+    torch.cuda.set_stream(tstream)
+    stream = tstream.cuda_stream
+    ctx_af = api.Context(api.OP_ALLELE_FREQ, api.FILE, device=0, stream=stream, chunk_bytes=bench.CHUNK, tile_bytes=args.tile)
+    ctx_vc = api.Context(api.OP_VARIANT_COUNT, api.FILE, device=0, stream=stream, chunk_bytes=bench.CHUNK, tile_bytes=args.tile)
+    valid_from = api.find_chrom_header(sh.hdr)
+
+    def step():
+        ctx_af.run_device(sh.d_in.data_ptr(), sh.nbytes, d_out.data_ptr(), out_cap, valid_from=valid_from)
+        ctx_vc.run_device(sh.d_in.data_ptr(), sh.nbytes, 0, 0)
+
+    for _ in range(5):
+        step()
+    torch.cuda.synchronize()
+    with profile(activities=[ProfilerActivity.CPU, ProfilerActivity.CUDA]) as prof:
+        for _ in range(args.steps):
+            step()
+        torch.cuda.synchronize()
+    trace = out / "step_timeline.pt.trace.json"
+    prof.export_chrome_trace(str(trace))
+
+    ev = json.loads(trace.read_text())["traceEvents"]
+    dev_ops = [e for e in ev if e.get("ph") == "X" and e.get("cat") in ("kernel", "gpu_memset", "gpu_memcpy")]
+    dev_ops.sort(key=lambda e: e["ts"])
+    per_step = len(dev_ops) // args.steps
+    last = dev_ops[-per_step:]
+    t0 = last[0]["ts"]
+    rows, prev_end = [], None
+    for e in last:
+        gap = 0.0 if prev_end is None else e["ts"] - prev_end
+        rows.append({"name": e["name"][:90], "cat": e["cat"], "start_us": round(e["ts"] - t0, 2), "dur_us": round(e["dur"], 2), "gap_us": round(gap, 2)})
+        prev_end = e["ts"] + e["dur"]
+    span = last[-1]["ts"] + last[-1]["dur"] - t0
+    busy = sum(e["dur"] for e in last)
+    lines = [f"{'start us':>10} {'dur us':>9} {'gap us':>8}  {'cat':<11} name"]
+    lines += [f"{r['start_us']:10.1f} {r['dur_us']:9.1f} {r['gap_us']:8.1f}  {r['cat']:<11} {r['name']}" for r in rows]
+    lines.append(f"step span {span:.1f} us, device ops {busy:.1f} us, gaps {span - busy:.1f} us, {len(last)} ops "
+                 f"({sum(r['cat'] != 'kernel' for r in rows)} memsets/memcpys)")
+    text = "\n".join(lines)
+    print(text)
+    (out / "step_timeline.txt").write_text(text + "\n")
+    (out / "step_timeline.json").write_text(json.dumps({"tile": args.tile, "span_us": span, "ops": rows}, indent=1))
+
+
+if __name__ == "__main__":
+    main()
diff --git a/vcfx_b200/csrc/vcfx_api.cu b/vcfx_b200/csrc/vcfx_api.cu
--- a/vcfx_b200/csrc/vcfx_api.cu
+++ b/vcfx_b200/csrc/vcfx_api.cu
@@ -28,10 +28,10 @@
     unsigned long long *tile_out = nullptr;
     unsigned long long *tile_base = nullptr;
     unsigned long long *line_base = nullptr;
-    uint32_t *tail_start = nullptr, *tail_len = nullptr, *tail_off = nullptr;
+    int32_t *tail_start = nullptr; uint32_t *tail_len = nullptr, *tail_off = nullptr;
     uint2 *col_scratch = nullptr;
     unsigned int *ticket = nullptr;
-    uint32_t *tile_resume = nullptr;
+    uint4 *tile_resume = nullptr;
     Rec *recs = nullptr;
     uint8_t *rec_prefix = nullptr;
     uint64_t rec_cap = 0;
@@ -43,7 +43,6 @@
     uint8_t *ib_panels = nullptr; uint64_t ib_panel_cap = 0;
     unsigned long long ib_seq = 0; bool ib_first = false;
     DevStats *h_stats = nullptr;
-    DevStats *h_init = nullptr;
     uint32_t tiles_cap = 0;
     cudaEvent_t ev_k0 = nullptr, ev_k1 = nullptr;
     cudaEvent_t ev_stats = nullptr;
@@ -229,7 +228,6 @@
     cudaFree(w.tail_start); cudaFree(w.tail_len); cudaFree(w.tail_off); cudaFree(w.col_scratch); cudaFree(w.tile_resume);
     cudaFree(w.ib_codes); cudaFree(w.ib_rows); cudaFree(w.ib_panels);
     if (w.h_stats) cudaFreeHost(w.h_stats);
-    if (w.h_init) cudaFreeHost(w.h_init);
     if (w.ev_k0) cudaEventDestroy(w.ev_k0);
     if (w.ev_k1) cudaEventDestroy(w.ev_k1);
     if (w.ev_stats) cudaEventDestroy(w.ev_stats);
@@ -244,8 +242,6 @@
         CU(cudaMalloc(&w.events, sizeof(unsigned long long) * EVENT_CAP));
         w.ev_cap = EVENT_CAP;
         CU(cudaMallocHost(&w.h_stats, sizeof(DevStats)));
-        CU(cudaMallocHost(&w.h_init, sizeof(DevStats)));
-        memset(w.h_init, 0, sizeof(DevStats)); w.h_init->first_short_key = ~0ULL;
         memset(w.h_stats, 0, sizeof(DevStats));
         CU(cudaEventCreate(&w.ev_k0));
         CU(cudaEventCreate(&w.ev_k1));
@@ -260,12 +256,12 @@
         CU(cudaMalloc(&w.line_base, sizeof(unsigned long long) * tiles));
         if (general_kernel_for(ctx->cfg.op)) {
             cudaFree(w.tile_resume); w.tile_resume = nullptr;
-            CU(cudaMalloc(&w.tile_resume, sizeof(uint32_t) * tiles));
+            CU(cudaMalloc(&w.tile_resume, sizeof(uint4) * tiles));
         }
         if (is_copy_op(ctx->cfg.op)) {
             cudaFree(w.tail_start); cudaFree(w.tail_len); cudaFree(w.tail_off);
-            w.tail_start = w.tail_len = w.tail_off = nullptr;
-            CU(cudaMalloc(&w.tail_start, sizeof(uint32_t) * tiles));
+            w.tail_start = nullptr; w.tail_len = w.tail_off = nullptr;
+            CU(cudaMalloc(&w.tail_start, sizeof(int32_t) * tiles));
             CU(cudaMalloc(&w.tail_len, sizeof(uint32_t) * tiles));
             CU(cudaMalloc(&w.tail_off, sizeof(uint32_t) * tiles));
         }
@@ -328,11 +324,7 @@
     if (!fn) return VCFX_E_UNSUPPORTED;
     const uint32_t tile = tile_for(ctx, nbytes);
     uint32_t tiles = tiles_for(ctx, nbytes, tile);
-    if (write_pad) CU(cudaMemsetAsync(d_in + nbytes, '\n', 64, st));
-    CU(cudaMemsetAsync(w.ticket, 0, 2 * sizeof(unsigned int), st));
     kernel_fn gfn = general_kernel_for(ctx->cfg.op);
-    if (gfn) CU(cudaMemsetAsync(w.tile_resume, 0xFF, sizeof(uint32_t) * tiles, st));
-    CU(cudaMemcpyAsync(w.d_stats, w.h_init, sizeof(DevStats), cudaMemcpyHostToDevice, st));
 
     KParams P;
     P.in = d_in; P.n = nbytes;
@@ -353,6 +345,11 @@
     P.ib_codes = w.ib_codes; P.ib_rows = w.ib_rows; P.ib_panels = w.ib_panels; P.ib_panel_cap = w.ib_panel_cap; P.ib = ctx->d_ib; P.ib_seq = w.ib_seq; P.ib_first = w.ib_first ? 1 : 0; P.text_cap = out_cap;
     if (ctx->cfg.op == VCFX_OP_INBREEDING) P.out_cap = ~0ULL;
     P.stats = w.d_stats; P.events = w.events; P.ev_cap = w.ev_cap; P.ev_raw = (ctx->cfg.op == VCFX_OP_PHASE_CHECK || ctx->cfg.op == VCFX_OP_GENOTYPE_QUERY) ? 1 : 0;
+    P.pad = write_pad ? d_in + nbytes : nullptr;
+    P.lines_only = (ctx->cfg.op == VCFX_OP_VARIANT_COUNT) ? 1 : 0;
+
+    VCFX_LAUNCH(launch_prologue_kernel, 1, 64, 0, st, P);
+    CU(cudaGetLastError());
 
     CU(cudaEventRecord(w.ev_k0, st));
     if (nbytes > 0) {
diff --git a/vcfx_b200/csrc/vcfx_kernels.cuh b/vcfx_b200/csrc/vcfx_kernels.cuh
--- a/vcfx_b200/csrc/vcfx_kernels.cuh
+++ b/vcfx_b200/csrc/vcfx_kernels.cuh
@@ -3,6 +3,9 @@
 #include <stdint.h>
 #include <stddef.h>
 #include "vcfx_numfmt.cuh"
+#ifdef VCFX_EMU
+#include "load_counter.h"
+#endif
 
 namespace vcfx {
 
@@ -18,7 +21,7 @@
 
 struct Rec {
     uint32_t tile;
-    uint32_t ls_rel;
+    int32_t ls_rel;
     uint32_t prefix_len;
     uint32_t off_in_tile;
     uint32_t a, b, c, d;
@@ -79,7 +82,7 @@
     unsigned long long *tile_out;
     unsigned long long *tile_base;
     unsigned long long *line_base;
-    uint32_t *tail_start;
+    int32_t *tail_start;
     uint32_t *tail_len;
     uint32_t *tail_off;
     int32_t ac_fmt;
@@ -97,13 +100,15 @@
     uint2 *col_scratch;
     unsigned int *ticket;
     unsigned int *ticket2;
-    uint32_t *tile_resume;
+    uint4 *tile_resume;
     Rec *recs;
     uint8_t *rec_prefix;
     uint64_t rec_cap;
     DevStats *stats;
     unsigned long long *events;
     uint32_t ev_cap;
+    uint8_t *pad;
+    int32_t lines_only;
     unsigned long long fmt0_until;
     int32_t c4_bulk;
     uint8_t gq_query[64];
@@ -148,9 +153,14 @@
     m0 &= nib80(k, 0); m1 &= nib80(k, 1); m2 &= nib80(k, 2); m3 &= nib80(k, 3);
 }
 
-__device__ __forceinline__ uint4 ld16(const uint8_t *p) { return __ldg(reinterpret_cast<const uint4 *>(p)); }
-__device__ __forceinline__ uint32_t ldb(const uint8_t *p) { return (uint32_t)__ldg(p); }
-__device__ __forceinline__ uint32_t ldw(const uint8_t *p) { return __ldg(reinterpret_cast<const uint32_t *>(p)); }
+#ifdef VCFX_EMU
+#define VCFX_NOTE_LOAD(p, n) emu_loads::note((p), (n))
+#else
+#define VCFX_NOTE_LOAD(p, n) ((void)0)
+#endif
+__device__ __forceinline__ uint4 ld16(const uint8_t *p) { VCFX_NOTE_LOAD(p, 16); return __ldg(reinterpret_cast<const uint4 *>(p)); }
+__device__ __forceinline__ uint32_t ldb(const uint8_t *p) { VCFX_NOTE_LOAD(p, 1); return (uint32_t)__ldg(p); }
+__device__ __forceinline__ uint32_t ldw(const uint8_t *p) { VCFX_NOTE_LOAD(p, 4); return __ldg(reinterpret_cast<const uint32_t *>(p)); }
 #ifdef VCFX_EMU
 #define VCFX_GRID_CONSTANT
 __device__ __forceinline__ void prefetch_l2(const void *) {}
@@ -431,6 +441,35 @@
     const uint32_t m = m0 ? m0 : (m1 ? m1 : (m2 ? m2 : m3));
     const int base = m0 ? 0 : (m1 ? 4 : (m2 ? 8 : 12));
     return base + ((__ffs(m) - 1) >> 3);
+}
+__device__ __forceinline__ int last_byte(uint32_t m0, uint32_t m1, uint32_t m2, uint32_t m3) {
+    const uint32_t m = m3 ? m3 : (m2 ? m2 : (m1 ? m1 : m0));
+    const int base = m3 ? 12 : (m2 ? 8 : (m1 ? 4 : 0));
+    return base + ((31 - __clz((int)m)) >> 3);
+}
+
+__device__ __forceinline__ uint64_t line_start_before(const uint8_t *__restrict__ in, const uint64_t x, const int lane) {
+    constexpr uint32_t PER_LANE = 4, SPAN = 32 * 16 * PER_LANE;
+    const uint32_t pl = 16u * PER_LANE * (uint32_t)lane;
+    uint64_t hi = (x + 15) & ~15ULL;
+    while (hi > 0) {
+        const uint64_t lo = hi > SPAN ? hi - SPAN : 0;
+        const uint32_t lim = (uint32_t)(x - lo);
+        uint4 v[PER_LANE];
+#pragma unroll
+        for (uint32_t j = 0; j < PER_LANE; ++j) v[j] = (lo + pl + 16u * j < hi) ? ld16(in + lo + pl + 16u * j) : uint4{0u, 0u, 0u, 0u};
+        int last = -1;
+#pragma unroll
+        for (uint32_t j = 0; j < PER_LANE; ++j) {
+            uint32_t m0 = eq_bytes(v[j].x, C_NL), m1 = eq_bytes(v[j].y, C_NL), m2 = eq_bytes(v[j].z, C_NL), m3 = eq_bytes(v[j].w, C_NL);
+            clip4(m0, m1, m2, m3, pl + 16u * j, 0u, lim);
+            if (m0 | m1 | m2 | m3) last = (int)(pl + 16u * j) + last_byte(m0, m1, m2, m3);
+        }
+        const unsigned bal = __ballot_sync(FULL, last >= 0);
+        if (bal) return lo + (uint64_t)__shfl_sync(FULL, last, 31 - __clz((int)bal)) + 1u;
+        hi = lo;
+    }
+    return 0;
 }
 
 __device__ __forceinline__ int warp_incl_scan(int v, int lane) {
@@ -724,7 +763,7 @@
 }
 
 template <int OP>
-__device__ __forceinline__ bool line_digits(const uint8_t *__restrict__ tin, uint32_t wb, const uint32_t lo, const uint32_t nrel,
+__device__ __forceinline__ bool line_digits(const uint8_t *__restrict__ tin, uint32_t wb, const uint32_t lo, const uint32_t end,
                                            const bool strip_cr, uint32_t &out_a, uint32_t &out_b, uint32_t &out_tabs, uint32_t &out_e) {
     const int lane = lane_id();
     constexpr uint32_t FILL = (OP == OP_AF) ? 0x09090909u : 0x20202020u;
@@ -761,7 +800,7 @@
         wb += WINDOW; cur = nxt; nxt = nx2; nx2 = ld16(tin + wb + 2 * WINDOW + 16 * lane);
         if (((wb >> 9) & 7u) == 0) {
             const uint32_t pf = wb + 10 * WINDOW + 128 * lane;
-            if (pf < nrel) prefetch_l2(tin + pf);
+            if (pf < end) prefetch_l2(tin + pf);
         }
     }
 }
@@ -872,9 +911,10 @@
 
 template <int OP, int VAR>
 __device__ __forceinline__ bool tile_lines(const KParams &P, const WarpShared ws, const int lane, const bool strip_cr,
-                                           const uint32_t tile, const uint64_t a, const uint64_t a0, const uint8_t *__restrict__ tin,
-                                           const uint32_t rb, const uint32_t nrel, const uint64_t n, TileState<OP> &st) {
+                                           const uint32_t tile, const int32_t tile_rel, const uint8_t *__restrict__ tin,
+                                           const uint32_t rb, const uint64_t n, TileState<OP> &st) {
     constexpr bool HAS_VAR = (OP == OP_AF || OP == OP_HWE);
+    const uint64_t a0 = (uint64_t)tile * P.tile_bytes + (int64_t)tile_rel;
     constexpr int NEED_TABS = (OP == OP_VC) ? 7 : (OP == OP_IX) ? 1 : 9;
     volatile uint32_t *tp = ws.tp;
     const int wid = threadIdx.x >> 5;
@@ -1050,7 +1090,7 @@
                             }
                             if ((++it & 1u) == 0) {
                                 const uint8_t *pf = lp - 16 * lane + 16 * WINDOW + 128 * lane;
-                                if ((uint32_t)(pf - tin) < nrel) prefetch_l2(pf);
+                                if ((uint32_t)(pf - tin) < rb) prefetch_l2(pf);
                             }
                             lp += 4 * WINDOW;
                         }
@@ -1066,7 +1106,7 @@
                             uint32_t la0 = ldw(lp + 16), la1 = ldw(lp + WINDOW + 16);
                             uint32_t la2 = ldw(lp + 2 * WINDOW + 16), la3 = ldw(lp + 3 * WINDOW + 16);
                             const uint32_t pf_need = wb + 12 * WINDOW;
-                            const uint32_t pf_iters = nrel > pf_need ? (nrel - pf_need) / (4 * WINDOW) : 0u;
+                            const uint32_t pf_iters = rb > pf_need ? (rb - pf_need) / (4 * WINDOW) : 0u;
                             uint32_t it = 0, accf = 0, acc2 = 0;
                             int state = 0;
 #define VCFX_T1_ROUND(X, LX, Y, LY)                                                                              \
@@ -1157,7 +1197,7 @@
                     if (VAR == 1 && OP == OP_AF && lat_possible && !digits_tried && !found && (first_win || prev_ok)) {
                         digits_tried = true;
                         uint32_t da = 0, db = 0, dt = 0, de = 0;
-                        if (line_digits<OP_AF>(tin, wb, first_win ? tab8 + 1u : wb + tau + 1u, nrel, strip_cr, da, db, dt, de)) {
+                        if (line_digits<OP_AF>(tin, wb, first_win ? tab8 + 1u : wb + tau + 1u, rb, strip_cr, da, db, dt, de)) {
                             ta += da; tb += db; e = de; found = true;
                             break;
                         }
@@ -1289,7 +1329,7 @@
                 bool summed = false;
                 if (P.ac_fmt == AC_AGG && P.ac_ident && !found && tp[8] - tp[7] == 3 && ldb(tin + tp[7] + 1) == 'G' && ldb(tin + tp[7] + 2) == 'T') {
                     uint32_t da = 0, db = 0, dt = 0, de = 0;
-                    if (line_digits<OP_AC>(tin, wb, tp[8] + 1u, nrel, false, da, db, dt, de) &&
+                    if (line_digits<OP_AC>(tin, wb, tp[8] + 1u, rb, false, da, db, dt, de) &&
                         (uint32_t)__reduce_add_sync(FULL, dt) + (uint32_t)tabs <= 8u + P.n_sel) {
                         ta = db - da; tb = da; tabs += (int)__reduce_add_sync(FULL, dt); e = de; found = true; summed = true;
                     }
@@ -1433,7 +1473,7 @@
                                 wb += WINDOW; cur = nxt; nxt = nx2; nx2 = ld16(tin + wb + 2 * WINDOW + 16 * lane);
                                 if (((wb >> 9) & 7u) == 0) {
                                     const uint32_t pf = wb + 8 * WINDOW + 128 * lane;
-                                    if (pf < nrel) prefetch_l2(tin + pf);
+                                    if (pf < rb) prefetch_l2(tin + pf);
                                 }
                                 continue;
                             }
@@ -1497,7 +1537,7 @@
                     wb += WINDOW; cur = nxt; nxt = nx2; nx2 = ld16(tin + wb + 2 * WINDOW + 16 * lane);
                     if (((wb >> 9) & 7u) == 0) {
                         const uint32_t pf = wb + 8 * WINDOW + 128 * lane;
-                        if (pf < nrel) prefetch_l2(tin + pf);
+                        if (pf < rb) prefetch_l2(tin + pf);
                     }
                 }
             }
@@ -1537,7 +1577,7 @@
                     wb += WINDOW; cur = nxt; nxt = nx2; nx2 = ld16(tin + wb + 2 * WINDOW + 16 * lane);
                     if (((wb >> 9) & 7u) == 0) {
                         const uint32_t pf = wb + 8 * WINDOW + 128 * lane;
-                        if (pf < nrel) prefetch_l2(tin + pf);
+                        if (pf < rb) prefetch_l2(tin + pf);
                     }
                 }
             }
@@ -1600,7 +1640,7 @@
                                 const uint8_t *sp = tin + pb + __ffs(m16);
                                 m16 &= m16 - 1u;
                                 const uint32_t *s4 = reinterpret_cast<const uint32_t *>((uintptr_t)sp & ~(uintptr_t)3);
-                                const uint32_t q = __funnelshift_r(__ldg(s4), __ldg(s4 + 1), 8u * (uint32_t)((uintptr_t)sp & 3));
+                                const uint32_t q = __funnelshift_r(ldw(reinterpret_cast<const uint8_t *>(s4)), ldw(reinterpret_cast<const uint8_t *>(s4 + 1)), 8u * (uint32_t)((uintptr_t)sp & 3));
                                 const uint32_t g3 = q & 0x00FFFFFFu, b3 = q >> 24;
                                 if (OP == OP_NR) {
                                     const bool quick = gi == 0 && (g3 == 0x00302F30u || g3 == 0x00307C30u) && (b3 == '\t' || b3 == ':');
@@ -1624,7 +1664,7 @@
                         wb += WINDOW; cur = nxt; nxt = nx2; nx2 = ld16(tin + wb + 2 * WINDOW + 16 * lane);
                         if (((wb >> 9) & 7u) == 0) {
                             const uint32_t pf = wb + 8 * WINDOW + 128 * lane;
-                            if (pf < nrel) prefetch_l2(tin + pf);
+                            if (pf < rb) prefetch_l2(tin + pf);
                         }
                     }
                 }
@@ -1634,7 +1674,7 @@
                 wb += WINDOW; cur = nxt; nxt = nx2; nx2 = ld16(tin + wb + 2 * WINDOW + 16 * lane);
                 if ((++wcount & 7u) == 0) {
                     const uint32_t pf = wb + 8 * WINDOW + 128 * lane;
-                    if (pf < nrel) prefetch_l2(tin + pf);
+                    if (pf < rb) prefetch_l2(tin + pf);
                 }
                 uint32_t n0 = eq_bytes(cur.x, C_NL), n1 = eq_bytes(cur.y, C_NL);
                 uint32_t n2 = eq_bytes(cur.z, C_NL), n3 = eq_bytes(cur.w, C_NL);
@@ -1703,7 +1743,7 @@
                     slot = __shfl_sync(FULL, slot, 0);
                     if (slot < P.rec_cap) {
                         if (lane == 0) {
-                            Rec r; r.tile = tile; r.ls_rel = (uint32_t)(a0 + ls - a); r.prefix_len = prefix_len;
+                            Rec r; r.tile = tile; r.ls_rel = (int32_t)ls + tile_rel; r.prefix_len = prefix_len;
                             r.off_in_tile = (uint32_t)out_bytes; r.a = ra_; r.b = rb_; r.c = rc_; r.d = 0;
                             P.recs[slot] = r;
                         }
@@ -1742,7 +1782,7 @@
                         if (lane == 0) {
                             unsigned long long slot = alloc_slot(ws.rec_base, ws.rec_used, P.stats);
                             if (slot < P.rec_cap) {
-                                Rec r; r.tile = tile; r.ls_rel = (uint32_t)(a0 + ls - a); r.prefix_len = prefix_src;
+                                Rec r; r.tile = tile; r.ls_rel = (int32_t)ls + tile_rel; r.prefix_len = prefix_src;
                                 r.off_in_tile = (uint32_t)out_bytes; r.a = sr; r.b = sa; r.c = n_rows; r.d = extra_tabs;
                                 P.recs[slot] = r;
                             }
@@ -1875,7 +1915,7 @@
                             row_len = c_len + 1u + dec_len64(pos) + 1u + dec_len64((long long)(P.file_offset + a0 + ls)) + 1u;
                             unsigned long long slot = alloc_slot(ws.rec_base, ws.rec_used, P.stats);
                             if (slot < P.rec_cap) {
-                                Rec r; r.tile = tile; r.ls_rel = (uint32_t)(a0 + ls - a); r.prefix_len = c_len;
+                                Rec r; r.tile = tile; r.ls_rel = (int32_t)ls + tile_rel; r.prefix_len = c_len;
                                 r.off_in_tile = (uint32_t)out_bytes; r.a = c_off; r.b = 0;
                                 r.c = (uint32_t)((unsigned long long)pos & 0xFFFFFFFFULL); r.d = (uint32_t)((unsigned long long)pos >> 32);
                                 P.recs[slot] = r;
@@ -1894,7 +1934,7 @@
                         if (lane == 0) {
                             const unsigned long long slot = alloc_slot(ws.rec_base, ws.rec_used, P.stats);
                             if (slot < P.rec_cap) {
-                                Rec r; r.tile = tile; r.ls_rel = (uint32_t)(a0 + ls - a); r.prefix_len = 0;
+                                Rec r; r.tile = tile; r.ls_rel = (int32_t)ls + tile_rel; r.prefix_len = 0;
                                 r.off_in_tile = (uint32_t)out_bytes; r.a = alt; r.b = good;
                                 r.c = min((uint32_t)(tabs - 8), P.n_sel); r.d = (((tp[8] + 4u) >> 2) - 1u) & 3u;
                                 P.recs[slot] = r;
@@ -1937,7 +1977,7 @@
                     if (lane == 0) {
                         unsigned long long slot = alloc_slot(ws.rec_base, ws.rec_used, P.stats);
                         if (slot < P.rec_cap) {
-                            Rec r; r.tile = tile; r.ls_rel = (uint32_t)(a0 + ls - a); r.prefix_len = (uint32_t)(a0 + md_prev_end - a);
+                            Rec r; r.tile = tile; r.ls_rel = (int32_t)ls + tile_rel; r.prefix_len = (uint32_t)((int32_t)md_prev_end + tile_rel);
                             r.off_in_tile = (uint32_t)out_bytes; r.a = 0; r.b = NR_PLAIN; r.c = content_len; r.d = mod_len;
                             P.recs[slot] = r;
                         }
@@ -1962,7 +2002,7 @@
                         if (lane == 0) {
                             const unsigned long long slot = alloc_slot(ws.rec_base, ws.rec_used, P.stats);
                             if (slot < P.rec_cap) {
-                                Rec r; r.tile = tile; r.ls_rel = (uint32_t)(a0 + ls - a); r.prefix_len = prefix_len;
+                                Rec r; r.tile = tile; r.ls_rel = (int32_t)ls + tile_rel; r.prefix_len = prefix_len;
                                 r.off_in_tile = (uint32_t)out_bytes; r.a = ncols; r.b = dlen; r.c = ds_gi < 0 ? 1u : 0u;
                                 r.d = (((tp[8] + 4u) >> 2) - 1u) & 3u;
                                 P.recs[slot] = r;
@@ -1998,7 +2038,7 @@
                     if (lane == 0) {
                         unsigned long long slot = alloc_slot(ws.rec_base, ws.rec_used, P.stats);
                         if (slot < P.rec_cap) {
-                            Rec r; r.tile = tile; r.ls_rel = (uint32_t)(a0 + ls - a); r.prefix_len = (uint32_t)(a0 + md_prev_end - a);
+                            Rec r; r.tile = tile; r.ls_rel = (int32_t)ls + tile_rel; r.prefix_len = (uint32_t)((int32_t)md_prev_end + tile_rel);
                             r.off_in_tile = (uint32_t)out_bytes; r.a = 0; r.b = NR_PLAIN; r.c = content_len; r.d = mod_len;
                             P.recs[slot] = r;
                         }
@@ -2024,7 +2064,7 @@
                     if (lane == 0) {
                         unsigned long long slot = alloc_slot(ws.rec_base, ws.rec_used, P.stats);
                         if (slot < P.rec_cap) {
-                            Rec r; r.tile = tile; r.ls_rel = (uint32_t)(a0 + ls - a); r.prefix_len = (uint32_t)(a0 + md_prev_end - a);
+                            Rec r; r.tile = tile; r.ls_rel = (int32_t)ls + tile_rel; r.prefix_len = (uint32_t)((int32_t)md_prev_end + tile_rel);
                             r.off_in_tile = (uint32_t)out_bytes; r.a = 0; r.b = NR_PLAIN; r.c = content_len; r.d = mod_len;
                             P.recs[slot] = r;
                         }
@@ -2053,7 +2093,7 @@
                     if (lane == 0) {
                         unsigned long long slot = alloc_slot(ws.rec_base, ws.rec_used, P.stats);
                         if (slot < P.rec_cap) {
-                            Rec r; r.tile = tile; r.ls_rel = (uint32_t)(a0 + ls - a); r.prefix_len = (uint32_t)(a0 + md_prev_end - a);
+                            Rec r; r.tile = tile; r.ls_rel = (int32_t)ls + tile_rel; r.prefix_len = (uint32_t)((int32_t)md_prev_end + tile_rel);
                             r.off_in_tile = (uint32_t)out_bytes; r.a = info_off; r.b = info_len; r.c = content_len; r.d = mod_len;
                             P.recs[slot] = r;
                         }
@@ -2120,47 +2160,39 @@
         if (lane == 0) tile = atomicAdd(VAR == 1 ? P.ticket2 : P.ticket, 1u);
         tile = __shfl_sync(FULL, tile, 0);
         if (tile >= P.n_tiles) break;
-        uint32_t resume = RESUME_DONE;
-        if (VAR == 1) { resume = P.tile_resume[tile]; if (resume == RESUME_DONE) continue; }
+        uint4 resume = make_uint4(RESUME_DONE, 0u, 0u, 0u);
+        if (VAR == 1) { resume = P.tile_resume[tile]; if (resume.x == RESUME_DONE) continue; }
 
         const uint64_t a = (uint64_t)tile * P.tile_bytes;
         const uint64_t b = min(a + (uint64_t)P.tile_bytes, n);
-        const uint64_t a0 = a - (tile ? 16u : 0u);
+        uint64_t a0;
+        uint32_t rb, ls, own0_rel;
+        if (VAR == 1) {
+            a0 = a - resume.y; rb = resume.z; ls = resume.x; own0_rel = resume.w;
+        } else {
+            const uint64_t own0 = a ? line_start_before(P.in, a, lane) : 0;
+            const uint64_t own1 = b < n ? line_start_before(P.in, b, lane) : n;
+            a0 = own0 & ~15ULL;
+            own0_rel = (uint32_t)(own0 - a0);
+            rb = (uint32_t)min(own1 - a0, (uint64_t)0xFFFFFFFFu);
+            ls = own0_rel;
+        }
         const uint8_t *__restrict__ tin = P.in + a0;
-        const uint32_t ra = (uint32_t)(a - a0), rb = (uint32_t)(b - a0);
-        const uint32_t nrel = (uint32_t)min(n - a0, (uint64_t)0xFFFFFFFFu);
-
-        uint32_t ls = rb;
-        if (VAR == 1) ls = resume;
-        else if (a == 0) ls = 0;
-        else {
-            const uint32_t from = ra - 1, to = rb - 1;
-            uint32_t wb = from & ~15u;
-            while (wb < to) {
-                const uint32_t pb = wb + 16 * lane;
-                uint4 v = ld16(tin + pb);
-                uint32_t m0 = eq_bytes(v.x, C_NL), m1 = eq_bytes(v.y, C_NL), m2 = eq_bytes(v.z, C_NL), m3 = eq_bytes(v.w, C_NL);
-                clip4(m0, m1, m2, m3, pb, from, to);
-                unsigned bal = __ballot_sync(FULL, (m0 | m1 | m2 | m3) != 0);
-                if (bal) {
-                    int src = __ffs(bal) - 1;
-                    int k = first_byte(m0, m1, m2, m3);
-                    k = __shfl_sync(FULL, k, src);
-                    ls = wb + 16 * src + k + 1;
-                    break;
-                }
-                wb += WINDOW;
-            }
-        }
+#ifdef VCFX_EMU
+        emu_loads::tile_owns(P.in, P.in + n, tin + own0_rel, tin + rb);
+#endif
 
         s_tag[wid] = 0;
         TileState<OP> st;
         st.ls = ls; st.nlines = 0; st.out_bytes = 0; st.md_prev_end = ls; st.md_last_end = ls; st.md_add_nl = false; st.offlattice_lines = 0;
         if (VAR == 1) { st.nlines = P.tile_lines[tile]; st.out_bytes = (typename OutCount<OP>::type)P.tile_out[tile]; }
         const uint32_t lines_before = st.nlines;
-        const bool finished = tile_lines<OP, VAR>(P, ws, lane, strip_cr, tile, a, a0, tin, rb, nrel, n, st);
+        const bool finished = tile_lines<OP, VAR>(P, ws, lane, strip_cr, tile, (int32_t)(a0 - a), tin, rb, n, st);
+#ifdef VCFX_EMU
+        emu_loads::tile_owns(nullptr, nullptr, nullptr, nullptr);
+#endif
         if (!finished) {
-            if (lane == 0) { P.tile_lines[tile] = st.nlines; P.tile_out[tile] = st.out_bytes; P.tile_resume[tile] = st.ls; atomicAdd(&P.stats->n_unfinished, 1ULL); }
+            if (lane == 0) { P.tile_lines[tile] = st.nlines; P.tile_out[tile] = st.out_bytes; P.tile_resume[tile] = make_uint4(st.ls, (uint32_t)(a - a0), rb, own0_rel); atomicAdd(&P.stats->n_unfinished, 1ULL); }
             VCFX_COUNT(C_LINES, st.nlines);
             __syncwarp();
             if (lane < CNT_SLOTS) {
@@ -2179,13 +2211,14 @@
         if (OP == OP_MD || OP == OP_NR || OP == OP_PC || OP == OP_GQ) {
             const uint32_t tail = md_last_end - md_prev_end;
             if (lane == 0) {
-                P.tail_start[tile] = (uint32_t)(a0 + md_prev_end - a);
+                P.tail_start[tile] = (int32_t)(a0 + md_prev_end - a);
                 P.tail_len[tile] = tail | (md_add_nl ? 0x80000000u : 0u);
                 P.tail_off[tile] = (uint32_t)out_bytes;
             }
             out_bytes += tail + (md_add_nl ? 1u : 0u);
         }
         if (lane == 0 && !(OP == OP_AC && P.ac_pass)) { P.tile_lines[tile] = nlines; P.tile_out[tile] = out_bytes; }
+        if ((OP == OP_AF || OP == OP_HWE) && VAR == 0 && lane == 0) P.tile_resume[tile].x = RESUME_DONE;
         if (OP == OP_AC && P.ac_pass && P.ac_spec && lane == 0 && (unsigned long long)out_bytes != P.tile_out[tile]) atomicOr(&P.stats->overflow, 4ULL);
         __syncwarp();
         if (lane < CNT_SLOTS) {
@@ -2201,6 +2234,17 @@
         const unsigned long long slot = s_rec_base[wid] + lane;
         if ((unsigned int)lane >= used && (unsigned int)lane < REC_BLOCK && slot < P.rec_cap) P.recs[slot].tile = REC_INVALID;
     }
+}
+
+static_assert(sizeof(DevStats) % 8 == 0 && sizeof(DevStats) / 8 <= 64, "launch_prologue_kernel: one thread per DevStats word");
+__global__ void __launch_bounds__(64)
+launch_prologue_kernel(const KParams P) {
+    const uint32_t t = threadIdx.x;
+    if (P.pad) P.pad[t] = '\n';
+    if (t == 0) *P.ticket = 0;
+    if (t == 1) *P.ticket2 = 0;
+    if (t < sizeof(DevStats) / 8)
+        reinterpret_cast<unsigned long long *>(P.stats)[t] = (t == offsetof(DevStats, first_short_key) / 8) ? ~0ULL : 0ULL;
 }
 
 constexpr uint32_t SCAN_BATCH = 8192;
@@ -2215,6 +2259,10 @@
 #else
     extern __shared__ unsigned long long scan_smem[];
 #endif
+    if (P.lines_only && P.stats->n_events == 0 && P.stats->first_short_key == ~0ULL) {
+        if (threadIdx.x == 0) { P.stats->bytes_out = 0; P.stats->first_short_line = 0; P.stats->overflow = (P.stats->n_recs > P.rec_cap) ? 1ULL : 0ULL; }
+        return;
+    }
     unsigned long long *so = scan_smem, *sl = scan_smem + SCAN_SMEM_WORDS;
     __shared__ unsigned long long ws_o[32], ws_l[32];
     __shared__ unsigned long long carry_o, carry_l;
@@ -2452,7 +2500,7 @@
             const uint8_t *base = P.in + (uint64_t)r.tile * P.tile_bytes;
             uint8_t *o = P.out + P.tile_base[r.tile] + r.off_in_tile;
             const uint32_t gap = r.ls_rel - r.prefix_len;
-            warp_copy(o, base + r.prefix_len, gap, lane);
+            warp_copy(o, base + (int32_t)r.prefix_len, gap, lane);
             o += gap;
             const uint8_t *ln = base + r.ls_rel;
             if (r.b == NR_PLAIN) {
```

New measurement: 2684, median of 6. +1.7%, better.
